# WeChatCV/WeDetect

Measured on AMD Instinct MI355X. Metric: images/s at 640x640 (WeDetect-Base image tower + 80-class similarity + top-k/NMS), higher is better.
Workload: dtype f32-equivalent: fp32 operands carried as fp16 hi+lo pairs, 3 fp16-MFMA passes per product, fp32 accumulate (fp16x3); similarity GEMM, dwconv, LN, post-process native f32

## Files before the change

__graft_entry__.py:

```python
import os
import sys

ROOT = os.path.dirname(os.path.abspath(__file__))
if ROOT not in sys.path:
    sys.path.insert(0, ROOT)


def build() -> None:
    from wedetect_amd import build as wb
    wb.build()
    import wedetect_amd.lib as lib
    import wedetect_amd.feed
    import wedetect_amd.tile
    import wedetect_amd.views
    import wedetect_amd.detector
    import oracle.postprocess
    import oracle.ref_cpu
    print("built and loaded", lib.LIB_PATH)


def smoke() -> None:
    import numpy as np
    import torch
    from oracle import postprocess as opp
    from oracle import ref_cpu as orc
    from wedetect_amd import weights as W
    from wedetect_amd.arch import get_arch
    from wedetect_amd.engine import ImageTower
    from wedetect_amd.pack import pack

    assert torch.cuda.is_available(), "smoke() needs a HIP device"
    torch.cuda.set_device(0)
    arch, b, hw, npr = "tiny", 2, 128, 64
    sd_np = W.make_state_dict(arch, num_prompts=npr)
    tower = ImageTower(arch, pack(sd_np, arch), b, hw, hw)
    imgs = W.make_images(b, hw, hw)
    embed, boxes = tower.features(torch.from_numpy(imgs).cuda())
    scores = tower.similarity(tower.P["prompts"], normalize=False)
    res = tower.postprocess(scores, 0.0, tower.identity_meta(), nms="torchvision")
    torch.cuda.synchronize()
    sd = orc.to_torch(sd_np)
    with torch.no_grad():
        _, p = orc.forward_features(sd, get_arch(arch), imgs)
        flat = orc.head_flat(sd, p, sd["embeddings"], normalize_text=False)
    e_err = float((embed.cpu() - flat["embed"]).abs().max())
    s_err = float((scores.cpu() - flat["scores"]).abs().max())
    b_err = float((boxes.cpu() - flat["boxes"]).abs().max())
    assert e_err < 1e-3 and s_err < 1e-3 and b_err < 1e-2, (e_err, s_err, b_err)
    lvl = np.concatenate([np.full(n, l) for l, n in enumerate(tower.nl)])
    for i in range(b):
        o = opp.uni_predict_image(boxes[i].cpu().numpy(), embed[i].cpu().numpy(), scores[i].cpu().numpy(), lvl,
                                  np.asarray(tower.lvl_logit_scale, np.float32), np.asarray(tower.lvl_bias, np.float32))
        n = int(res["count"][i])
        assert n == o["scores"].shape[0]
        assert np.array_equal(res["anchors"][i, :n].cpu().numpy(), o["anchors"])
        assert np.array_equal(res["labels"][i, :n].cpu().numpy(), o["labels"])
    print(f"smoke OK: max|d| embeddings {e_err:.2e} scores {s_err:.2e} boxes {b_err:.2e}; kept indices exact")


if __name__ == "__main__":
    build()
    if "--smoke" in sys.argv:
        smoke()
```

wedetect_amd/build.py:

```python
from __future__ import annotations

import os
import subprocess
import sys

HERE = os.path.dirname(os.path.abspath(__file__))
ROOT = os.path.dirname(HERE)
CSRC = os.path.join(HERE, "csrc")
LIB = os.path.join(HERE, "libwedetect_hip.so")
SOURCES = ["abi.hip", "conv_gemm.hip", "similarity_grouped.hip", "split_gemm.hip", "split_gemm_pre.hip", "split_gemm_p8.hip", "split_gemm_p4.hip", "split_gemm_conv.hip", "split_gemm_conv3.hip", "split_gemm_mlp.hip", "split_gemm_mlpw.hip", "probe.hip", "stem.hip", "elementwise.hip", "preprocess.hip", "text.hip", "bricks.hip", "evaluate.hip", "det_eval.hip", "postprocess.hip", "feed.hip", "tile.hip", "views.hip"]
PUBLIC_HEADERS = ["wedetect_hip.h", "wedetect_hip_feed.h", "wedetect_hip_tile.h", "wedetect_hip_views.h"]
HIPCC = os.environ.get("HIPCC", "/opt/rocm/bin/hipcc")
FLAGS = ["--offload-arch=gfx950", "-O3", "-std=c++17", "-fPIC", "-Wall", "-Wno-unused-function", "-Wno-inline-asm",
         "-I", os.path.join(ROOT, "include"), "-I", CSRC]
for _d in os.environ.get("WD_EXTRA_DEFINES", "").split():
    FLAGS.append("-D" + _d)
if os.environ.get("WD_DEBUG_ABLATIONS") == "1":
    FLAGS.append("-DWD_DEBUG_ABLATIONS")


def _headers():
    return [os.path.join(CSRC, f) for f in os.listdir(CSRC) if f.endswith(".h")] + [os.path.join(ROOT, "include", h) for h in PUBLIC_HEADERS]


def source_hash() -> str:
    import hashlib
    h = hashlib.sha256()
    files = sorted(os.path.join(CSRC, f) for f in os.listdir(CSRC) if f.endswith((".hip", ".h")))
    for f in files + [os.path.join(ROOT, "include", h) for h in PUBLIC_HEADERS]:
        h.update(os.path.basename(f).encode())
        h.update(open(f, "rb").read())
    return h.hexdigest()


NO_SCRATCH = {"stem.hip": ["stem_fused_kernel"], "split_gemm_mlpw.hip": ["fused_mlp_wide_kernel"],
              "split_gemm_mlp.hip": ["fused_mlp128_kernel"], "split_gemm_p8.hip": ["split_gemm_p8_kernel"],
              "split_gemm_p4.hip": ["split_gemm_p4_kernel"], "split_gemm_conv.hip": ["split_conv_pp_kernel"],
              "split_gemm_conv3.hip": ["split_conv3_kernel", "split_conv3w_kernel"],
              "split_gemm_pre.hip": ["split_gemm_pingpong_kernel", "split_gemm_glds_kernel"],
              "elementwise.hip": ["dwconv7_dma_kernel", "dwconv7_ln_reg4_dma_kernel"],
              "similarity_grouped.hip": ["similarity_grouped_kernel"],
              "feed.hip": ["feed_resample_h_kernel", "feed_canvas_kernel"],
              "tile.hip": ["tile_cut_kernel", "merge_keys_kernel"],
              "views.hip": ["flip_u8_kernel", "views_sort_kernel"]}
ASM_VMEM_SOURCES = {"split_gemm_mlpw.hip": ["fused_mlp_wide_kernel"], "split_gemm_mlp.hip": [], "split_gemm_p8.hip": [],
                    "split_gemm_p4.hip": [], "split_gemm_pre.hip": [], "split_gemm_conv.hip": [], "split_gemm_conv3.hip": [], "stem.hip": [], "elementwise.hip": [], "similarity_grouped.hip": [],
                    "feed.hip": [], "tile.hip": [], "views.hip": []}


ASM_DS_READ_SOURCES = {"split_gemm_conv3.hip": ["split_conv3w_kernel"]}


def check_isa(src: str, verbose: bool = True) -> None:
    asm = _obj(src).replace(".o", ".s")
    cmd = [HIPCC, *[f for f in FLAGS if f != "-fPIC"], "-S", "--cuda-device-only", os.path.join(CSRC, src), "-o", asm]
    subprocess.check_call(cmd, stderr=subprocess.DEVNULL)
    scripts = os.path.join(ROOT, "scripts")
    r = subprocess.run([sys.executable, os.path.join(scripts, "check_sgpr_vmem_hazard.py"), asm], capture_output=True, text=True)
    if r.returncode != 0:
        raise RuntimeError(f"SGPR -> VMEM hazard in the ISA of {src}:\n{r.stdout[-2000:]}")
    syms = ASM_VMEM_SOURCES[src]
    if syms:
        r = subprocess.run([sys.executable, os.path.join(scripts, "check_asm_loads.py"), asm, *syms], capture_output=True, text=True)
        if r.returncode != 0:
            raise RuntimeError(f"pending asm load touched in the ISA of {src}:\n{r.stdout[-2000:]}")
    if src in ASM_DS_READ_SOURCES:
        r = subprocess.run([sys.executable, os.path.join(scripts, "check_asm_ds_reads.py"), asm, *ASM_DS_READ_SOURCES[src]], capture_output=True, text=True)
        if r.returncode != 0:
            raise RuntimeError(f"pending asm ds_read touched in the ISA of {src}:\n{r.stdout[-2000:]}")
    if src in NO_SCRATCH:
        import re
        meta = open(asm).read()
        meta = meta[meta.index("amdhsa.kernels"):] if "amdhsa.kernels" in meta else ""
        seen = set()
        for blk in meta.split("- .agpr_count")[1:]:
            name = re.search(r"\.name:\s+(\S+)", blk).group(1)
            scratch = int(re.search(r"\.private_segment_fixed_size:\s+(\d+)", blk).group(1))
            for k in NO_SCRATCH[src]:
                if k in name:
                    seen.add(k)
                    if scratch != 0:
                        raise RuntimeError(f"{src}: kernel {name} uses {scratch} bytes of scratch — its counted vmcnt waits assume none")
        missing = [k for k in NO_SCRATCH[src] if k not in seen]
        if missing:
            raise RuntimeError(f"{src}: NO_SCRATCH names no kernel of this source: {missing}")
    os.remove(asm)
    if verbose:
        print(f"ISA checks passed: {src}", flush=True)


def _obj(src: str) -> str:
    return os.path.join(CSRC, src.replace(".hip", ".o"))


def _obj_stale(src: str) -> bool:
    obj = _obj(src)
    if not os.path.exists(obj):
        return True
    t = os.path.getmtime(obj)
    return any(os.path.getmtime(d) > t for d in [os.path.join(CSRC, src)] + _headers())


def _stale() -> bool:
    if not os.path.exists(LIB):
        return True
    t = os.path.getmtime(LIB)
    return any(_obj_stale(s) or os.path.getmtime(_obj(s)) > t for s in SOURCES)


def build(force: bool = False, verbose: bool = True) -> str:
    if not force and not _stale():
        return LIB
    procs = []
    for src in SOURCES:
        if not force and not _obj_stale(src):
            continue
        cmd = [HIPCC, *FLAGS, "-c", os.path.join(CSRC, src), "-o", _obj(src)]
        if verbose:
            print(" ".join(cmd), flush=True)
        procs.append((src, subprocess.Popen(cmd)))
    import concurrent.futures as cf
    with cf.ThreadPoolExecutor(max_workers=4) as ex:
        checks = [ex.submit(check_isa, src, verbose) for src, _ in procs if src in ASM_VMEM_SOURCES]
        for src, p in procs:
            if p.wait() != 0:
                raise RuntimeError(f"hipcc failed on {src}")
        for c in checks:
            c.result()
    cmd = [HIPCC, "--offload-arch=gfx950", "-shared", "-fPIC", *[_obj(s) for s in SOURCES], "-o", LIB]
    if verbose:
        print(" ".join(cmd), flush=True)
    subprocess.check_call(cmd)
    return LIB


if __name__ == "__main__":
    print(build(force="--force" in sys.argv))
```

wedetect_amd/csrc/split_epi_oct.h:

```cpp
#pragma once
#include "split_gemm_impl.h"

namespace {

template <int ACT, bool SPECIAL, bool CSPLIT>
__device__ __forceinline__ void epi_oct_core(const WdConvGemm& p, float unscale, int m, int n, const f32x4 v0, const f32x4 v1,
                                             const f32x4 b0, const f32x4 b1, const f32x4 r0, const f32x4 r1) {
  if (p.range_flag) {
    if (wd_any_nonfinite4(v0[0] + v0[1], v0[2] + v0[3], v1[0] + v1[1], v1[2] + v1[3])) *p.range_flag = 1u;
  }
  const EpiRow er = epi_row<SPECIAL>(p, m);
  f32x4 o0, o1;
#pragma unroll
  for (int r = 0; r < 4; ++r) {
    float x0 = sact<ACT>(fmaf(v0[r], unscale, b0[r]));
    float x1 = sact<ACT>(fmaf(v1[r], unscale, b1[r]));
    if (SPECIAL) {
      x0 = fmaf(x0, er.oscale, er.obias);
      x1 = fmaf(x1, er.oscale, er.obias);
      if (p.sigmoid) { x0 = wd_sigmoid_fast(x0); x1 = wd_sigmoid_fast(x1); }
    }
    o0[r] = x0;
    o1[r] = x1;
  }
  if (p.res != nullptr) {
#pragma unroll
    for (int r = 0; r < 4; ++r) {
      o0[r] = fmaf(p.res_alpha, r0[r], o0[r]);
      o1[r] = fmaf(p.res_alpha, r1[r], o1[r]);
    }
  }
  if (p.c2 != nullptr) {
    float* qp = p.c2 + (SPECIAL && p.c_batch_stride > 0 ? er.crow : (size_t)m) * p.ldc2 + n;
    *reinterpret_cast<f32x4*>(qp) = o0;
    *reinterpret_cast<f32x4*>(qp + 4) = o1;
  }
  float* rowp;
  int col = n;
  if (SPECIAL && p.out_mode == WD_OUT_DECONV2X2) {
    const int ncq = p.n >> 2;
    const int tap = n / ncq;
    col = n - tap * ncq;
    rowp = p.c + (er.crow + (size_t)(tap >> 1) * er.hw2 + (tap & 1)) * p.ldc;
  } else {
    rowp = p.c + er.crow * p.ldc;
  }
  if (CSPLIT) {
    u32x2 h0, l0, h1, l1;
    f32x4 s0 = o0, s1 = o1;
    if (p.c_split_scale != 0.f && p.c_split_scale != 1.0f) {
      s0 = o0 * p.c_split_scale;
      s1 = o1 * p.c_split_scale;
    }
    split4(s0, h0, l0);
    split4(s1, h1, l1);
    unsigned char* cp = reinterpret_cast<unsigned char*>(rowp) + (size_t)(col >> 3) * 32;
    *reinterpret_cast<u32x4*>(cp) = u32x4{h0[0], h0[1], h1[0], h1[1]};
    *reinterpret_cast<u32x4*>(cp + 16) = u32x4{l0[0], l0[1], l1[0], l1[1]};
  } else {
    *reinterpret_cast<f32x4*>(rowp + col) = o0;
    *reinterpret_cast<f32x4*>(rowp + col + 4) = o1;
  }
}

template <int ACT, bool SPECIAL, bool CSPLIT>
__device__ __forceinline__ void epi_oct(const WdConvGemm& p, float unscale, int m, int n, const f32x4 v0, const f32x4 v1) {
  f32x4 b0 = {0.f, 0.f, 0.f, 0.f}, b1 = {0.f, 0.f, 0.f, 0.f}, r0 = b0, r1 = b0;
  if (p.bias) {
    b0 = *reinterpret_cast<const f32x4*>(p.bias + n);
    b1 = *reinterpret_cast<const f32x4*>(p.bias + n + 4);
  }
  if (p.res != nullptr) {
    const float* rp = p.res + (size_t)m * p.ldres + n;
    r0 = *reinterpret_cast<const f32x4*>(rp);
    r1 = *reinterpret_cast<const f32x4*>(rp + 4);
  }
  epi_oct_core<ACT, SPECIAL, CSPLIT>(p, unscale, m, n, v0, v1, b0, b1, r0, r1);
}

template <int TM, int TN, bool PRE = true>
struct EpiOctOperands {
  static constexpr int NB = PRE ? TN : 1, NR = PRE ? TM * TN * 2 : 1;
  f32x4 b0[NB], b1[NB], r0[NR], r1[NR];
  __device__ __forceinline__ void load(const WdConvGemm& p, int mw, int nw, int lane) {
    if (!PRE) return;
#pragma unroll
    for (int j = 0; j < TN; ++j) {
      const int n = nw + j * 32 + 8 * (lane & 3);
      b0[j] = b1[j] = f32x4{0.f, 0.f, 0.f, 0.f};
      if (p.bias && n < p.n) {
        b0[j] = *reinterpret_cast<const f32x4*>(p.bias + n);
        b1[j] = *reinterpret_cast<const f32x4*>(p.bias + n + 4);
      }
    }
#pragma unroll
    for (int ij = 0; ij < TM * TN; ++ij)
#pragma unroll
      for (int ps = 0; ps < 2; ++ps) {
        const int m = mw + (ij / TN) * 32 + ps * 16 + (lane >> 2), n = nw + (ij % TN) * 32 + 8 * (lane & 3);
        r0[ij * 2 + ps] = r1[ij * 2 + ps] = f32x4{0.f, 0.f, 0.f, 0.f};
        if (p.res != nullptr && m < p.m && n < p.n) {
          const float* rp = p.res + (size_t)m * p.ldres + n;
          r0[ij * 2 + ps] = *reinterpret_cast<const f32x4*>(rp);
          r1[ij * 2 + ps] = *reinterpret_cast<const f32x4*>(rp + 4);
        }
      }
  }
};

template <int IJ, int TM, int TN, int ACT, bool SPECIAL, bool CSPLIT, bool PRE = true>
struct EpiOctWalk {
  static __device__ __forceinline__ void run(const WdConvGemm& p, float unscale, int mw, int nw, int lane,
                                             const f32x16 (&acc)[TM][TN], float* patch, const EpiOctOperands<TM, TN, PRE>& ops) {
    constexpr int I = IJ / TN, J = IJ % TN;
#pragma unroll
    for (int g = 0; g < 4; ++g)
      *reinterpret_cast<f32x4*>(patch + (lane & 31) * EPI_LDT + 8 * g + 4 * (lane >> 5)) =
          f32x4{acc[I][J][4 * g], acc[I][J][4 * g + 1], acc[I][J][4 * g + 2], acc[I][J][4 * g + 3]};
    __builtin_amdgcn_fence(__ATOMIC_RELEASE, "wavefront");
    __builtin_amdgcn_wave_barrier();
    __builtin_amdgcn_fence(__ATOMIC_ACQUIRE, "wavefront");
#pragma unroll
    for (int ps = 0; ps < 2; ++ps) {
      const int row = ps * 16 + (lane >> 2);
      const int m = mw + I * 32 + row;
      const int n = nw + J * 32 + 8 * (lane & 3);
      const f32x4 v0 = *reinterpret_cast<const f32x4*>(patch + row * EPI_LDT + 8 * (lane & 3));
      const f32x4 v1 = *reinterpret_cast<const f32x4*>(patch + row * EPI_LDT + 8 * (lane & 3) + 4);
      if (m < p.m && n < p.n) {
        if (PRE)
          epi_oct_core<ACT, SPECIAL, CSPLIT>(p, unscale, m, n, v0, v1, ops.b0[PRE ? J : 0], ops.b1[PRE ? J : 0],
                                             ops.r0[PRE ? IJ * 2 + ps : 0], ops.r1[PRE ? IJ * 2 + ps : 0]);
        else
          epi_oct<ACT, SPECIAL, CSPLIT>(p, unscale, m, n, v0, v1);
      }
    }
    __builtin_amdgcn_fence(__ATOMIC_RELEASE, "wavefront");
    __builtin_amdgcn_wave_barrier();
    __builtin_amdgcn_fence(__ATOMIC_ACQUIRE, "wavefront");
    EpiOctWalk<IJ + 1, TM, TN, ACT, SPECIAL, CSPLIT, PRE>::run(p, unscale, mw, nw, lane, acc, patch, ops);
  }
};
template <int TM, int TN, int ACT, bool SPECIAL, bool CSPLIT, bool PRE>
struct EpiOctWalk<TM * TN, TM, TN, ACT, SPECIAL, CSPLIT, PRE> {
  static __device__ __forceinline__ void run(const WdConvGemm&, float, int, int, int, const f32x16 (&)[TM][TN], float*,
                                             const EpiOctOperands<TM, TN, PRE>&) {}
};

template <int TM, int TN, bool CSPLIT, bool PRE = true>
__device__ __forceinline__ void epi_oct_all(const WdConvGemm& p, float unscale, int mw, int nw, int lane,
                                            const f32x16 (&acc)[TM][TN], float* patch) {
  const bool special = p.out_mode != WD_OUT_ROWS || p.c_batch_stride > 0 || p.seg_rows > 0 || p.sigmoid ||
                       p.out_scale != 1.0f || p.out_bias != 0.0f;
  EpiOctOperands<TM, TN, PRE> ops;
  ops.load(p, mw, nw, lane);
#define WD_OCT(A, S) EpiOctWalk<0, TM, TN, A, S, CSPLIT, PRE>::run(p, unscale, mw, nw, lane, acc, patch, ops)
  if (special) {
    switch (p.act) {
      case WD_ACT_RELU: WD_OCT(WD_ACT_RELU, true); break;
      case WD_ACT_SILU: WD_OCT(WD_ACT_SILU, true); break;
      case WD_ACT_GELU: WD_OCT(WD_ACT_GELU, true); break;
      default: WD_OCT(WD_ACT_NONE, true); break;
    }
  } else {
    switch (p.act) {
      case WD_ACT_RELU: WD_OCT(WD_ACT_RELU, false); break;
      case WD_ACT_SILU: WD_OCT(WD_ACT_SILU, false); break;
      case WD_ACT_GELU: WD_OCT(WD_ACT_GELU, false); break;
      default: WD_OCT(WD_ACT_NONE, false); break;
    }
  }
#undef WD_OCT
}

}
```

wedetect_amd/csrc/split_gemm.hip:

```cpp
#include <stdlib.h>
#include "split_gemm_impl.h"

namespace {

__global__ void split_weights_kernel(const float* __restrict__ w, int n, int k, int k16, float scale,
                                     unsigned short* __restrict__ out, int n_out) {
  const long long idx = (long long)blockIdx.x * blockDim.x + threadIdx.x;
  if (idx >= (long long)n_out * k16) return;
  const int row = (int)(idx / k16), kk = (int)(idx % k16);
  const float x = (kk < k && row < n) ? w[(size_t)row * k + kk] * scale : 0.0f;
  const _Float16 hi = (_Float16)x;
  const _Float16 lo = (_Float16)(x - (float)hi);
  unsigned short* o = out + (size_t)row * 2 * k16 + (kk >> 3) * 16 + (kk & 7);
  o[0] = __builtin_bit_cast(unsigned short, hi);
  o[8] = __builtin_bit_cast(unsigned short, lo);
}

template <int ACT, bool SPECIAL>
__global__ void __launch_bounds__(256) splitk_reduce_kernel(const WdConvGemm p, const float* __restrict__ ws, int splits,
                                                            float unscale, int vec_c, int vec_res, int vec_bias) {
  const long long idx = (long long)blockIdx.x * blockDim.x + threadIdx.x;
  const int nq = p.n >> 2;
  if (idx >= (long long)p.m * nq) return;
  const int m = (int)(idx / nq), n = (int)(idx - (long long)m * nq) * 4;
  const size_t plane = (size_t)p.m * p.n;
  f32x4 v = *reinterpret_cast<const f32x4*>(ws + (size_t)m * p.n + n);
  for (int s = 1; s < splits; ++s) v += *reinterpret_cast<const f32x4*>(ws + s * plane + (size_t)m * p.n + n);
  const EpiVec ev{vec_c, vec_res, vec_bias, unscale};
  epi_quad<ACT, SPECIAL>(p, epi_row<SPECIAL>(p, m), ev, m, n, v);
}

template <bool SPECIAL>
int launch_reduce(const WdConvGemm& p, const float* ws, int splits, float unscale, hipStream_t st) {
  const long long total = (long long)p.m * (p.n >> 2);
  const dim3 grid((unsigned)((total + 255) / 256)), block(256);
  const int vec_c = (p.ldc % 4 == 0) && wd_aligned16(p.c) && (p.out_mode == WD_OUT_ROWS || (p.n % 16 == 0));
  const int vec_res = p.res ? ((p.ldres % 4 == 0) && wd_aligned16(p.res)) : 0;
  const int vec_bias = p.bias ? wd_aligned16(p.bias) : 0;
  switch (p.act) {
    case WD_ACT_RELU: hipLaunchKernelGGL((splitk_reduce_kernel<WD_ACT_RELU, SPECIAL>), grid, block, 0, st, p, ws, splits, unscale, vec_c, vec_res, vec_bias); break;
    case WD_ACT_SILU: hipLaunchKernelGGL((splitk_reduce_kernel<WD_ACT_SILU, SPECIAL>), grid, block, 0, st, p, ws, splits, unscale, vec_c, vec_res, vec_bias); break;
    case WD_ACT_GELU: hipLaunchKernelGGL((splitk_reduce_kernel<WD_ACT_GELU, SPECIAL>), grid, block, 0, st, p, ws, splits, unscale, vec_c, vec_res, vec_bias); break;
    default: hipLaunchKernelGGL((splitk_reduce_kernel<WD_ACT_NONE, SPECIAL>), grid, block, 0, st, p, ws, splits, unscale, vec_c, vec_res, vec_bias); break;
  }
  return wd_launch_status();
}

}

extern "C" int64_t wd_split_weights_bytes(int32_t n, int32_t k) {
  if (n <= 0 || k <= 0) return 0;
  return (int64_t)((n + 7) & ~7) * ((k + 15) / 16 * 16) * 4;
}

static int split_weights_launch(const float* w, int32_t n, int32_t k, float scale, void* out, void* stream, int n_out) {
  if (!w || !out || n <= 0 || k <= 0 || !(scale > 0.0f) || !wd_aligned16(out)) return WD_ERR_BAD_ARG;
  const int k16 = (k + 15) / 16 * 16;
  const long long total = (long long)n_out * k16;
  hipLaunchKernelGGL(split_weights_kernel, dim3((unsigned)((total + 255) / 256)), dim3(256), 0,
                     static_cast<hipStream_t>(stream), w, n, k, k16, scale, static_cast<unsigned short*>(out), n_out);
  return wd_launch_status();
}

extern "C" int wd_split_weights(const float* w, int32_t n, int32_t k, float scale, void* out, void* stream) {
  return split_weights_launch(w, n, k, scale, out, stream, n);
}

extern "C" int wd_split_weights_padded(const float* w, int32_t n, int32_t k, float scale, void* out, void* stream) {
  return split_weights_launch(w, n, k, scale, out, stream, (n + 7) & ~7);
}

static int pick_split_cfg(const WdConvGemm& p) {
  const int m = p.m, n = p.n;
  const long long pad128 = (long long)((n + 127) / 128) * 128, pad64 = (long long)((n + 63) / 64) * 64;
  if (pad64 < pad128) return m >= 65536 ? 52 : 53;
  const bool plain = p.kh == 1 && p.kw == 1 && p.stride == 1 && p.pad == 0;
  if (plain && p.k >= 1024) return 55;
  const long long tiles = (long long)((m + 127) / 128) * ((n + 127) / 128);
  return tiles < 1024 ? 50 : 51;
}

long long wd_p8_workspace_floats();
bool wd_p8_persist_ok(int m, int n);
bool wd_conv_pp_ok(const WdConvGemm& p, int flags);
int wd_launch_conv_pp(const WdConvGemm& p, const void* w, float unscale, int flags, hipStream_t st, int ksplits, float* ws,
                      long long ws_floats, int variant);
bool wd_conv3_ok(const WdConvGemm& p, int flags);
const char* wd_conv3_config_name(int m, int n);
int wd_launch_conv3(const WdConvGemm& p, const void* w, float unscale, int flags, hipStream_t st, int variant, int ksplits, float* ws,
                    long long ws_floats);

extern "C" int64_t wd_p8_workspace_bytes(void) { return 4 * wd_p8_workspace_floats(); }

static int pick_presplit_cfg(int m, int n, int k, bool park) {
  if (k % 32 == 0 && k >= 256 && m % 8 == 0 && n % 256 == 0) {
    const long long tiles = (long long)((m + 255) / 256) * (n / 256);
    static const int mink = [] { const char* e = getenv("WD_P8_PERSIST_MINK"); return e ? atoi(e) : 1024; }();
    if (park && k >= mink && wd_p8_persist_ok(m, n)) return 65;
    if (tiles >= 128) return 64;
  }
  if (k % 16 == 0 && n % 256 == 0 && m % 16 == 0 && m >= 131072) return 66;
  return m >= 131072 ? 63 : 60;
}

extern "C" const char* wd_conv_gemm_split_config(int32_t m, int32_t n, int32_t k, int32_t is_conv) {
  if (is_conv == 4) {
    const bool narrow = (n % 128) != 0 && ((n + 63) / 64) * 64 < ((n + 127) / 128) * 128;
    return narrow ? "fp16x3 256x64x16/8w/dma" : "fp16x3 256x128x16/8w/dma";
  }
  if (is_conv == 5) return wd_conv3_config_name(m, n);
  if ((is_conv == 2 || is_conv == 3) && k % 16 == 0) {
    switch (pick_presplit_cfg(m, n, k, is_conv == 3)) {
      case 65: return "fp16x3 256x256x32/8w/p8s";
      case 64: return "fp16x3 256x256x32/8w/p8";
      case 66: return "fp16x3 128x256x16/4w/p4";
      case 63: return "fp16x3 256x128x16/8w/pingpong";
      default: return "fp16x3 128x128x16/4w/glds";
    }
  }
  WdConvGemm q{};
  q.m = m; q.n = n; q.k = k; q.kh = q.kw = q.stride = 1;
  if (is_conv) q.kh = q.kw = 3;
  switch (pick_split_cfg(q)) {
    case 50: return "fp16x3 128x128x32/4w";
    case 51: return "fp16x3 128x128x16/4w";
    case 52: return "fp16x3 256x64x16/4w";
    case 55: return "fp16x3 128x128x32/4w/pf2";
    default: return "fp16x3 128x64x16/2w";
  }
}

static int pick_ksplits(const WdConvGemm& p, int cfg, int flags, long long ws_floats) {
  if (ws_floats <= 0 || (flags & WD_SPLIT_C) || (p.n & 3) || cfg == 55 || cfg == 63 || cfg >= 64) return 1;
  const int bm = 128, bn = (cfg == 52 || cfg == 53) ? 64 : 128, bk = (cfg == 50) ? 32 : 16;
  const long long tiles = (long long)((p.m + (cfg == 52 ? 255 : bm - 1)) / (cfg == 52 ? 256 : bm)) * ((p.n + bn - 1) / bn);
  const int nk = (p.k + bk - 1) / bk;
  if (tiles >= 128 || nk < 16) return 1;
  int s = (int)(512 / tiles);
  if (s > nk / 8) s = nk / 8;
  if (s > 16) s = 16;
  while (s > 1 && (long long)s * p.m * p.n > ws_floats) --s;
  return s < 2 ? 1 : s;
}

static int conv_gemm_split_impl(const WdConvGemm* pp, const void* w_split, float w_unscale, int32_t flags, int32_t cfg,
                                float* ws, int64_t ws_bytes, int32_t force_splits, hipStream_t st) {
  if (!pp) return WD_ERR_BAD_ARG;
  const WdConvGemm& p = *pp;
  const int rc = check_split_args(p, w_split, w_unscale);
  if (rc != WD_OK) return rc;
  if (flags & ~(WD_SPLIT_A | WD_SPLIT_C)) return WD_ERR_BAD_ARG;
  if (ws && !wd_aligned16(ws)) return WD_ERR_BAD_ARG;
  if (p.c2 && !(flags & WD_SPLIT_C)) return WD_ERR_BAD_ARG;
  const bool production = cfg < 0;
  if (cfg < 0) cfg = pick_split_cfg(p);
  const bool plain = p.kh == 1 && p.kw == 1 && p.stride == 1 && p.pad == 0;
  const bool special = p.out_mode != WD_OUT_ROWS || p.c_batch_stride > 0 || p.seg_rows > 0 || p.sigmoid ||
                       p.out_scale != 1.0f || p.out_bias != 0.0f;
  if (p.ln_stats || p.ln_u) {
    if (!p.ln_stats || !p.ln_u || flags != (WD_SPLIT_A | WD_SPLIT_C) || !plain || special || p.res || p.c2 || force_splits > 1 ||
        !wd_aligned16(p.ln_u) || (reinterpret_cast<uintptr_t>(p.ln_stats) & 7u))
      return WD_ERR_BAD_ARG;
    if (cfg == 70 || cfg == 73 || cfg == 74 || (cfg >= 75 && cfg <= 79) || (cfg >= 700 && cfg < 716)) return WD_ERR_UNSUPPORTED;
  }
  if (flags & WD_SPLIT_A) {
    const bool covered = plain && !special && !p.c2 && !((flags & WD_SPLIT_C) && p.res);
    const bool forced = cfg == 70 || cfg == 73 || cfg == 74 || (cfg >= 700 && cfg < 716);
    static const bool conv3_on = [] { const char* e = getenv("WEDETECT_CONV3"); return !(e && e[0] == '0'); }();
    if ((cfg >= 75 && cfg <= 79) || (production && conv3_on && !(force_splits == 0 && ws != nullptr))) {
      if (wd_conv3_ok(p, flags) && wd_conv_pp_ok(p, flags))
        return wd_launch_conv3(p, w_split, w_unscale, flags, st, cfg == 76 ? 2 : cfg == 77 ? 7 : cfg == 78 ? 8 : cfg == 79 ? 9 : 0, force_splits > 1 ? force_splits : 1, ws, ws ? ws_bytes / 4 : 0);
      if (cfg >= 75 && cfg <= 79) return WD_ERR_UNSUPPORTED;
    }
    if (forced || (production && !covered)) {
      if (!wd_conv_pp_ok(p, flags)) return forced || !covered ? WD_ERR_UNSUPPORTED : WD_ERR_BAD_ARG;
      const long long wsf = ws ? ws_bytes / 4 : 0;
      int splits = force_splits > 0 ? force_splits : 1;
      if (force_splits == 0 && wsf > 0 && !forced) {
        const long long tiles = (long long)((p.m + 255) / 256) * ((p.n + 127) / 128);
        const int nk = p.k / 16;
        if (tiles < 128 && nk >= 32) {
          int s2 = (int)(256 / tiles);
          if (s2 > nk / 16) s2 = nk / 16;
          if (s2 > 8) s2 = 8;
          while (s2 > 1 && (long long)s2 * p.m * p.n > wsf) --s2;
          if (s2 > 1) splits = s2;
        }
      }
      return wd_launch_conv_pp(p, w_split, w_unscale, flags, st, splits, ws, wsf,
                               cfg == 73 ? 3 : cfg == 74 ? 4 : cfg >= 700 ? cfg - 600 : 0);
    }
  }
  if (flags == WD_SPLIT_C) {
    if (!plain || special || p.res || p.c2 || p.n % 8 || p.ldc % 8 || (p.bias && !wd_aligned16(p.bias)) || !wd_aligned16(p.c))
      return WD_ERR_UNSUPPORTED;
    constexpr int VC = SVAR_XCD | SVAR_PIN | SVAR_LDSEPI | SVAR_CSPLIT;
    const long long tiles = (long long)((p.m + 127) / 128) * ((p.n + 127) / 128);
    return tiles < 1024 ? launch_split<2, 2, 2, 2, 32, VC, 1>(p, w_split, w_unscale, st)
                        : launch_split<2, 2, 2, 2, 16, VC, 1>(p, w_split, w_unscale, st);
  }
  if (flags != 0) {
    if (production && plain && !special && p.k % 16 == 0)
      cfg = pick_presplit_cfg(p.m, p.n, p.k, ws != nullptr && force_splits == 0 && ws_bytes / 4 >= wd_p8_workspace_floats() &&
                                                 p.lda % 8 == 0 && !(flags & ~(WD_SPLIT_A | WD_SPLIT_C)));
    if (cfg != 50 && cfg != 51 && cfg != 55 && cfg != 60 && cfg != 63 && cfg != 64 && cfg != 65 && cfg != 66 && !(cfg >= 640 && cfg < 768)) cfg = 51;
    if ((flags & WD_SPLIT_C) && cfg == 55) cfg = 50;
  }
  const long long ws_floats = ws ? ws_bytes / 4 : 0;
  int splits = force_splits > 0 ? force_splits : pick_ksplits(p, cfg, flags, ws_floats);
  {
    const int bk = (cfg == 50) ? 32 : 16, nk = (p.k + bk - 1) / bk;
    if (splits > nk) splits = nk;
  }
  if (splits > 1) {
    if ((flags & WD_SPLIT_C) || (p.n & 3) || cfg == 55 || cfg == 63 || cfg >= 64) return WD_ERR_UNSUPPORTED;
    if ((long long)splits * p.m * p.n > ws_floats) return WD_ERR_WORKSPACE;
  }
  int lrc;
  if (flags != 0) {
    lrc = wd_launch_presplit(p, w_split, w_unscale, cfg, flags, st, splits, ws, ws_floats);
  } else {
    switch (cfg) {
      case 41: lrc = launch_split<2, 2, 2, 4, 16, SVAR_XCD | SVAR_PIN | SVAR_LDSEPI>(p, w_split, w_unscale, st, splits, ws); break;
      case 50: lrc = launch_split<2, 2, 2, 2, 32, SVAR_XCD | SVAR_PIN | SVAR_LDSEPI>(p, w_split, w_unscale, st, splits, ws); break;
      case 51: lrc = launch_split<2, 2, 2, 2, 16, SVAR_XCD | SVAR_PIN | SVAR_LDSEPI>(p, w_split, w_unscale, st, splits, ws); break;
      case 52: lrc = launch_split<2, 2, 4, 1, 16, SVAR_XCD | SVAR_PIN | SVAR_LDSEPI>(p, w_split, w_unscale, st, splits, ws); break;
      case 53: lrc = launch_split<2, 2, 2, 1, 16, SVAR_XCD | SVAR_PIN | SVAR_LDSEPI>(p, w_split, w_unscale, st, splits, ws); break;
      case 55: lrc = launch_split<2, 2, 2, 2, 32, SVAR_XCD | SVAR_PF2 | SVAR_LDSEPI>(p, w_split, w_unscale, st); break;
      default: return WD_ERR_UNSUPPORTED;
    }
  }
  if (lrc != WD_OK || splits <= 1) return lrc;
  return special ? launch_reduce<true>(p, ws, splits, w_unscale, st) : launch_reduce<false>(p, ws, splits, w_unscale, st);
}

extern "C" int wd_conv_gemm_split(const WdConvGemm* pp, const void* w_split, float w_unscale, int32_t flags,
                                  int32_t cfg, void* stream) {
  return conv_gemm_split_impl(pp, w_split, w_unscale, flags, cfg, nullptr, 0, 0, static_cast<hipStream_t>(stream));
}

extern "C" int wd_conv_gemm_split_ws(const WdConvGemm* pp, const void* w_split, float w_unscale, int32_t flags,
                                     int32_t cfg, void* workspace, int64_t workspace_bytes, int32_t splits, void* stream) {
  if (splits < 0 || workspace_bytes < 0) return WD_ERR_BAD_ARG;
  return conv_gemm_split_impl(pp, w_split, w_unscale, flags, cfg, static_cast<float*>(workspace), workspace_bytes, splits,
                              static_cast<hipStream_t>(stream));
}
```

wedetect_amd/csrc/split_gemm_conv.hip:

```cpp
#include "split_epi_oct.h"

namespace {

constexpr int CV_BM = 256, CV_WROWS = 128, CV_ROWB = 64, CV_STAGE = (CV_BM + CV_WROWS) * CV_ROWB, CV_NI = 3;

__device__ __forceinline__ void cv_dma16(unsigned lds_addr, const unsigned char* src) {
  asm volatile("s_mov_b32 m0, %0\n\tglobal_load_lds_dwordx4 %1, off" ::"s"(lds_addr), "v"(src) : "memory", "m0");
}

__device__ __forceinline__ void cv_wait_groups(int groups) {
  if (groups <= 0) asm volatile("s_waitcnt vmcnt(0)" ::: "memory");
  else if (groups == 1) asm volatile("s_waitcnt vmcnt(3)" ::: "memory");
  else if (groups == 2) asm volatile("s_waitcnt vmcnt(6)" ::: "memory");
  else if (groups == 3) asm volatile("s_waitcnt vmcnt(9)" ::: "memory");
  else if (groups == 4) asm volatile("s_waitcnt vmcnt(12)" ::: "memory");
  else asm volatile("s_waitcnt vmcnt(15)" ::: "memory");
}

template <int NBUF, int TN, bool CSPLIT, int ABL = 0>
__global__ void __launch_bounds__(512, NBUF <= 3 ? 4 : 2)
split_conv_pp_kernel(const WdConvGemm p, const unsigned char* __restrict__ wsp, const float* __restrict__ zero, int k16,
                     float unscale, int nbn, int ksplits, float* __restrict__ ws) {
  constexpr int TM = 2, BM = CV_BM, BN = 64 * TN, ROWB = CV_ROWB, STAGE = CV_STAGE, NI = CV_NI, DIST = NBUF - 1;
  extern __shared__ __attribute__((aligned(16))) unsigned char smem_raw[];
  const int t = threadIdx.x, lane = t & 63, wave = t >> 6;
  const int group = wave >> 2, wm = (wave >> 1) & 1, wn = wave & 1;
  int tile = blockIdx.x;
  {
    const int nwg = gridDim.x, xcd = tile & 7, idx = tile >> 3;
    const int q = nwg >> 3, r = nwg & 7;
    tile = (xcd < r ? xcd * (q + 1) : r * (q + 1) + (xcd - r) * q) + idx;
  }
  const int ntiles = gridDim.x / ksplits;
  const int ks = tile / ntiles;
  tile -= ks * ntiles;
  const int bn = tile % nbn, bm = tile / nbn;
  const int m0 = bm * BM, n0 = bn * BN;
  const int nk_all = p.k >> 4;
  const int per_split = (nk_all + ksplits - 1) / ksplits;
  const int s_begin = ks * per_split;
  const int nk = (s_begin + per_split < nk_all ? s_begin + per_split : nk_all) - s_begin;

  const unsigned char* base[NI];
  unsigned mask[NI];
#pragma unroll
  for (int j = 0; j < NI; ++j) {
    const int row = (wave * NI + j) * 16 + (lane >> 2);
    const int logical = (lane & 3) ^ ((row >> 2) & 3);
    const int memchunk = ((logical & 1) << 1) | ((logical >> 1) & 1);
    if (row < BM) {
      const int m = m0 + row;
      const bool ok = m < p.m;
      const int mm = ok ? m : 0;
      const int wo = mm % p.wout;
      const int q = mm / p.wout;
      const int ho = q % p.hout;
      const int b = q / p.hout;
      const int hi0 = ho * p.stride - p.pad, wi0 = wo * p.stride - p.pad;
      const long long pix = ((long long)b * p.hin + hi0) * p.win + wi0;
      base[j] = reinterpret_cast<const unsigned char*>(p.a) + pix * p.lda * 4 + memchunk * 16;
      unsigned mk = 0, bit = 1u;
      for (int kh = 0; kh < p.kh; ++kh) {
        const bool hok = (unsigned)(hi0 + kh) < (unsigned)p.hin;
        for (int kw = 0; kw < p.kw; ++kw, bit <<= 1)
          mk |= (hok && (unsigned)(wi0 + kw) < (unsigned)p.win) ? bit : 0u;
      }
      mask[j] = ok ? mk : 0u;
    } else {
      const int n = n0 + row - BM;
      const bool ok = n < p.n;
      base[j] = wsp + (size_t)(ok ? n : 0) * k16 * 4 + memchunk * 16;
      mask[j] = ok ? 0xFFFFFFFFu : 0u;
    }
  }
  int i_tap, i_ci, i_kh, i_kw, i_w;
  {
    const int kofs = s_begin * 16;
    i_tap = kofs / p.cin;
    i_ci = kofs - i_tap * p.cin;
    i_kh = i_tap / p.kw;
    i_kw = i_tap - i_kh * p.kw;
    i_w = s_begin * ROWB;
  }
  const unsigned lds0 = (unsigned)(size_t)(__attribute__((address_space(3))) unsigned char*)smem_raw;
  const unsigned char* zp = reinterpret_cast<const unsigned char*>(zero);
  bool prologue = true;
  auto issue = [&](int buf) {
    if ((ABL & 1) && !prologue) return;
    const unsigned lbase = lds0 + buf * STAGE + wave * NI * 1024;
    const int a_off = ((i_kh * p.win + i_kw) * p.lda + i_ci) * 4;
#pragma unroll
    for (int j = 0; j < NI; ++j) {
      const bool is_a = (wave * NI + j) * 16 < BM;
      const int off = is_a ? a_off : i_w;
      const unsigned bit = is_a ? (mask[j] >> i_tap) & 1u : mask[j] & 1u;
      cv_dma16(__builtin_amdgcn_readfirstlane(lbase + j * 1024), bit ? base[j] + off : zp);
    }
    i_w += ROWB;
    i_ci += 16;
    if (i_ci == p.cin) {
      i_ci = 0;
      ++i_tap;
      if (++i_kw == p.kw) { i_kw = 0; ++i_kh; }
    }
  };

  f32x16 acc[TM][TN];
#pragma unroll
  for (int i = 0; i < TM; ++i)
#pragma unroll
    for (int j = 0; j < TN; ++j)
#pragma unroll
      for (int r = 0; r < 16; ++r) acc[i][j][r] = 0.0f;

  int aoff_h[TM], aoff_l[TM], boff_h[TN], boff_l[TN];
  const int hsel = lane >> 5;
#pragma unroll
  for (int i = 0; i < TM; ++i) {
    const int row = group * 128 + wm * 64 + i * 32 + (lane & 31), f = (row >> 2) & 3;
    aoff_h[i] = row * ROWB + ((hsel ^ f) << 4);
    aoff_l[i] = row * ROWB + (((2 + hsel) ^ f) << 4);
  }
#pragma unroll
  for (int j = 0; j < TN; ++j) {
    const int row = wn * 32 * TN + j * 32 + (lane & 31), f = (row >> 2) & 3;
    boff_h[j] = BM * ROWB + row * ROWB + ((hsel ^ f) << 4);
    boff_l[j] = BM * ROWB + row * ROWB + (((2 + hsel) ^ f) << 4);
  }
  h8 xh[TM], xl[TM], wh[TN], wl[TN];
  auto read = [&](int buf) {
    if ((ABL & 2) && !prologue) return;
    const unsigned char* sp = smem_raw + buf * STAGE;
#pragma unroll
    for (int i = 0; i < TM; ++i) {
      xh[i] = *reinterpret_cast<const h8*>(sp + aoff_h[i]);
      xl[i] = *reinterpret_cast<const h8*>(sp + aoff_l[i]);
    }
#pragma unroll
    for (int j = 0; j < TN; ++j) {
      wh[j] = *reinterpret_cast<const h8*>(sp + boff_h[j]);
      wl[j] = *reinterpret_cast<const h8*>(sp + boff_l[j]);
    }
  };
  auto mfma = [&]() {
    if (ABL & 4) return;
#pragma unroll
    for (int i = 0; i < TM; ++i)
#pragma unroll
      for (int j = 0; j < TN; ++j)
        acc[i][j] = __builtin_amdgcn_mfma_f32_32x32x16_f16(wl[j], xh[i], acc[i][j], 0, 0, 0);
#pragma unroll
    for (int i = 0; i < TM; ++i)
#pragma unroll
      for (int j = 0; j < TN; ++j)
        acc[i][j] = __builtin_amdgcn_mfma_f32_32x32x16_f16(wh[j], xl[i], acc[i][j], 0, 0, 0);
#pragma unroll
    for (int i = 0; i < TM; ++i)
#pragma unroll
      for (int j = 0; j < TN; ++j)
        acc[i][j] = __builtin_amdgcn_mfma_f32_32x32x16_f16(wh[j], xh[i], acc[i][j], 0, 0, 0);
  };

#pragma unroll
  for (int d = 0; d < DIST; ++d)
    if (d < nk) issue(d);
  asm volatile("s_waitcnt vmcnt(0)" ::: "memory");
  __syncthreads();
  if (ABL & 2) read(0);
  prologue = false;
  int bcur = 0, bfill = DIST % NBUF;
  for (int s = 0; s < nk; ++s) {
    read(bcur);
    if (s + DIST < nk) issue(bfill);
    __builtin_amdgcn_sched_barrier(0);
    mfma();
    __builtin_amdgcn_sched_barrier(0);
    {
      const int last = s + DIST < nk - 1 ? s + DIST : nk - 1;
      cv_wait_groups(last - (s + 1));
    }
    __builtin_amdgcn_sched_barrier(0);
    __syncthreads();
    __builtin_amdgcn_sched_barrier(0);
    bcur = bcur == NBUF - 1 ? 0 : bcur + 1;
    bfill = bfill == NBUF - 1 ? 0 : bfill + 1;
  }
  __syncthreads();

  if (ABL & 8) {
    float sacc = 0.f;
#pragma unroll
    for (int i = 0; i < TM; ++i)
#pragma unroll
      for (int j = 0; j < TN; ++j)
#pragma unroll
        for (int r = 0; r < 16; ++r) sacc += acc[i][j][r];
    if (m0 + (t & 255) < p.m) p.c[(size_t)(m0 + (t & 255)) * p.ldc + n0 + (t >> 8)] = sacc;
    return;
  }
  const int mw = m0 + group * 128 + wm * 64, nw = n0 + wn * 32 * TN;
  float* patch = reinterpret_cast<float*>(smem_raw) + wave * 32 * EPI_LDT;
  static_assert(2 * STAGE >= 8 * 32 * EPI_LDT * 4, "operand LDS must hold one patch per wave");
  if (ksplits > 1) {
    WdConvGemm pr = p;
    pr.bias = nullptr; pr.res = nullptr; pr.c2 = nullptr; pr.range_flag = nullptr;
    pr.c = ws + (size_t)ks * p.m * p.n; pr.ldc = p.n;
    pr.out_mode = WD_OUT_ROWS; pr.c_batch_stride = 0; pr.seg_rows = 0; pr.sigmoid = 0; pr.out_scale = 1.0f; pr.out_bias = 0.0f;
    pr.act = WD_ACT_NONE;
    EpiOctOperands<TM, TN, false> ops;
    ops.load(pr, mw, nw, lane);
    EpiOctWalk<0, TM, TN, WD_ACT_NONE, false, false, false>::run(pr, 1.0f, mw, nw, lane, acc, patch, ops);
    return;
  }
  epi_oct_all<TM, TN, CSPLIT, (NBUF == 4 || TN == 1)>(p, unscale, mw, nw, lane, acc, patch);
}

template <int ACT, bool SPECIAL, bool CSPLIT>
__global__ void __launch_bounds__(256) splitk_oct_reduce_kernel(const WdConvGemm p, const float* __restrict__ ws, int splits,
                                                                float unscale) {
  const long long idx = (long long)blockIdx.x * blockDim.x + threadIdx.x;
  const int no = p.n >> 3;
  if (idx >= (long long)p.m * no) return;
  const int m = (int)(idx / no), n = (int)(idx - (long long)m * no) * 8;
  const size_t plane = (size_t)p.m * p.n;
  const float* src = ws + (size_t)m * p.n + n;
  f32x4 v0 = *reinterpret_cast<const f32x4*>(src), v1 = *reinterpret_cast<const f32x4*>(src + 4);
  for (int s = 1; s < splits; ++s) {
    v0 += *reinterpret_cast<const f32x4*>(src + s * plane);
    v1 += *reinterpret_cast<const f32x4*>(src + s * plane + 4);
  }
  epi_oct<ACT, SPECIAL, CSPLIT>(p, unscale, m, n, v0, v1);
}

template <bool CSPLIT>
int launch_oct_reduce(const WdConvGemm& p, const float* ws, int splits, float unscale, hipStream_t st) {
  const long long total = (long long)p.m * (p.n >> 3);
  const dim3 grid((unsigned)((total + 255) / 256)), block(256);
  const bool special = p.out_mode != WD_OUT_ROWS || p.c_batch_stride > 0 || p.seg_rows > 0 || p.sigmoid ||
                       p.out_scale != 1.0f || p.out_bias != 0.0f;
#define WD_RED(A, S) hipLaunchKernelGGL((splitk_oct_reduce_kernel<A, S, CSPLIT>), grid, block, 0, st, p, ws, splits, unscale)
  if (special) {
    switch (p.act) {
      case WD_ACT_RELU: WD_RED(WD_ACT_RELU, true); break;
      case WD_ACT_SILU: WD_RED(WD_ACT_SILU, true); break;
      case WD_ACT_GELU: WD_RED(WD_ACT_GELU, true); break;
      default: WD_RED(WD_ACT_NONE, true); break;
    }
  } else {
    switch (p.act) {
      case WD_ACT_RELU: WD_RED(WD_ACT_RELU, false); break;
      case WD_ACT_SILU: WD_RED(WD_ACT_SILU, false); break;
      case WD_ACT_GELU: WD_RED(WD_ACT_GELU, false); break;
      default: WD_RED(WD_ACT_NONE, false); break;
    }
  }
#undef WD_RED
  return wd_launch_status();
}

template <int NBUF, int TN, bool CSPLIT, int ABL = 0>
int launch_conv_pp(const WdConvGemm& p, const void* wsp, float unscale, hipStream_t st, int ksplits, float* ws) {
  constexpr int BN = 64 * TN, LDS = NBUF * CV_STAGE;
  const int nbm = (p.m + CV_BM - 1) / CV_BM, nbn = (p.n + BN - 1) / BN;
  const long long nblk = (long long)nbm * nbn * ksplits;
  if (nblk <= 0 || nblk > 0x7fffffffLL) return WD_ERR_BAD_ARG;
  const int k16 = (p.k + 15) / 16 * 16;
  const float* zero = wd_zero_block();
  if (!zero) return WD_ERR_LAUNCH;
  auto k = split_conv_pp_kernel<NBUF, TN, CSPLIT, ABL>;
  static WdAttrOnce attr;
  if (wd_set_max_lds(attr, reinterpret_cast<const void*>(k), LDS) != WD_OK) return WD_ERR_LAUNCH;
  WD_LAUNCH_GEMM(k, dim3((unsigned)nblk), dim3(512), LDS, st, p, static_cast<const unsigned char*>(wsp), zero, k16, unscale,
                 nbn, ksplits, ws);
  return wd_launch_status();
}

}

int wd_launch_oct_reduce(const WdConvGemm& p, const float* ws, int splits, float unscale, bool csplit, hipStream_t st) {
  return csplit ? launch_oct_reduce<true>(p, ws, splits, unscale, st) : launch_oct_reduce<false>(p, ws, splits, unscale, st);
}

bool wd_conv_pp_ok(const WdConvGemm& p, int flags) {
  if (!(flags & WD_SPLIT_A)) return false;
  if (p.cin % 16 || p.k % 16 || p.lda % 8 || p.kh * p.kw > 16 || p.n % 8) return false;
  if (!wd_aligned16(p.a) || !wd_aligned16(p.c)) return false;
  if (p.bias && !wd_aligned16(p.bias)) return false;
  if (p.res && (!wd_aligned16(p.res) || p.ldres % 4)) return false;
  if (p.c2 && (!(flags & WD_SPLIT_C) || !wd_aligned16(p.c2) || p.ldc2 % 4 || p.ldc2 < p.n || p.out_mode != WD_OUT_ROWS))
    return false;
  if ((flags & WD_SPLIT_C) ? (p.ldc % 8 != 0) : (p.ldc % 4 != 0)) return false;
  if (p.out_mode == WD_OUT_DECONV2X2 && (p.n % 32)) return false;
  return true;
}

int wd_launch_conv_pp(const WdConvGemm& p, const void* w, float unscale, int flags, hipStream_t st, int ksplits, float* ws,
                      long long ws_floats, int variant) {
  if (!wd_conv_pp_ok(p, flags)) return WD_ERR_UNSUPPORTED;
  const bool csplit = (flags & WD_SPLIT_C) != 0;
  const bool narrow = (p.n % 128) != 0 && ((p.n + 63) / 64) * 64 < ((p.n + 127) / 128) * 128;
  const long long tiles = (long long)((p.m + CV_BM - 1) / CV_BM) * (narrow ? (p.n + 63) / 64 : (p.n + 127) / 128);
  if (ksplits < 1) ksplits = 1;
  if (ksplits > 1 && (!ws || (long long)ksplits * p.m * p.n > ws_floats)) return WD_ERR_WORKSPACE;
  if (ksplits > (p.k >> 4)) ksplits = p.k >> 4;
  int nbuf = (tiles * ksplits <= 256) ? 4 : 3;
  if (variant == 3 || variant == 4) nbuf = variant;
  int rc;
#ifdef WD_DEBUG_ABLATIONS
  if (variant >= 100 && variant < 116 && !narrow && csplit) {
    switch (variant - 100) {
      case 1: return launch_conv_pp<4, 2, true, 1>(p, w, unscale, st, 1, ws);
      case 2: return launch_conv_pp<4, 2, true, 2>(p, w, unscale, st, 1, ws);
      case 3: return launch_conv_pp<4, 2, true, 3>(p, w, unscale, st, 1, ws);
      case 4: return launch_conv_pp<4, 2, true, 4>(p, w, unscale, st, 1, ws);
      case 7: return launch_conv_pp<4, 2, true, 7>(p, w, unscale, st, 1, ws);
      case 8: return launch_conv_pp<4, 2, true, 8>(p, w, unscale, st, 1, ws);
      case 11: return launch_conv_pp<4, 2, true, 11>(p, w, unscale, st, 1, ws);
      case 15: return launch_conv_pp<4, 2, true, 15>(p, w, unscale, st, 1, ws);
      default: break;
    }
  }
#endif
#define WD_CPP(NB, TNN, CS) launch_conv_pp<NB, TNN, CS>(p, w, unscale, st, ksplits, ws)
  if (nbuf == 4) {
    if (narrow) rc = csplit ? WD_CPP(4, 1, true) : WD_CPP(4, 1, false);
    else rc = csplit ? WD_CPP(4, 2, true) : WD_CPP(4, 2, false);
  } else {
    if (narrow) rc = csplit ? WD_CPP(3, 1, true) : WD_CPP(3, 1, false);
    else rc = csplit ? WD_CPP(3, 2, true) : WD_CPP(3, 2, false);
  }
#undef WD_CPP
  if (rc != WD_OK || ksplits <= 1) return rc;
  return csplit ? launch_oct_reduce<true>(p, ws, ksplits, unscale, st) : launch_oct_reduce<false>(p, ws, ksplits, unscale, st);
}
```

wedetect_amd/engine.py:

```python
from __future__ import annotations

import contextlib
import copy
import math
import os
import weakref
from typing import Dict, List, Optional, Sequence, Tuple

import numpy as np
import torch

from . import lib as L
from .arch import ArchSpec, CLS_MID, EMBED_DIM, REG_MID, STRIDES, get_arch, level_sizes
from .pack import Packed


DEFAULT_PRECISION = "fp16x3"


def fold_layernorm_into_linear(w1: torch.Tensor, b1: torch.Tensor, gamma: torch.Tensor, beta: torch.Tensor):
    w64, g64 = w1.double(), gamma.double()
    w1g = (w64 * g64[None, :]).float().contiguous()
    u = w1g.double().sum(dim=1).float().contiguous()
    v = (w64 @ beta.double() + b1.double()).float().contiguous()
    return w1g, u, v


_DEVICE_STREAMS: Dict[str, Dict[str, list]] = {}


def device_streams(dev: torch.device, role: str, n: int = 1) -> List[torch.cuda.Stream]:
    pool = _DEVICE_STREAMS.setdefault(str(dev), {})
    if not pool:
        for r in ("post", "nh", "bb2"):
            pool[r] = [torch.cuda.Stream(device=dev)]
    lst = pool.setdefault(role, [])
    while len(lst) < n:
        lst.append(torch.cuda.Stream(device=dev))
    return lst[:n]


class ImageTower:
    PRECISIONS = ("fp32", "fp16x3")
    SPLIT_K_AUTO_PIXELS = 4 * 640 * 640
    SPLIT_K_MID_PIXELS = 8 * 640 * 640

    def __init__(self, arch, packed: Packed, batch: int, height: int, width: int, device="cuda",
                 max_classes: int = 256, nms_pre: int = 30000, max_out: int = 300,
                 precision: Optional[str] = None, split_k: Optional[bool] = None):
        self.a: ArchSpec = get_arch(arch) if isinstance(arch, str) else arch
        self.P = packed
        if precision is None:
            precision = os.environ.get("WEDETECT_PRECISION", DEFAULT_PRECISION)
        if precision not in self.PRECISIONS:
            raise ValueError(f"precision must be one of {self.PRECISIONS}")
        self.precision = precision
        self.Ws: Dict[str, tuple] = {}
        auto_class = split_k is None and os.environ.get("WEDETECT_SPLIT_K", "auto") == "auto"
        if split_k is None:
            env = os.environ.get("WEDETECT_SPLIT_K", "auto")
            split_k = env == "1" or (env == "auto" and batch * height * width <= self.SPLIT_K_MID_PIXELS)
        self._split_ref = 1
        if split_k and auto_class and batch * height * width > self.SPLIT_K_AUTO_PIXELS:
            self._split_ref = max(1, self.SPLIT_K_MID_PIXELS // (height * width))
        self.kws = (torch.empty(16 << 20, dtype=torch.float32, device=torch.device(device))
                    if precision == "fp16x3" and split_k else None)
        self._kws_lane: Dict[int, torch.Tensor] = {}
        self.fixed_splitk = precision == "fp16x3" and os.environ.get("WEDETECT_FIXED_SPLITK", "1") == "1"
        self.fws = (torch.empty(2 * batch * 400 * 256 + 64, dtype=torch.float32, device=torch.device(device))
                    if self.fixed_splitk else None)
        self.p8_mode = os.environ.get("WEDETECT_P8", "persist")
        self.post_stream, self._post_ready, self._post_done = None, None, None
        dag = os.environ.get("WEDETECT_DAG", "auto")
        self.dag = dag != "0"
        self._dag_forced = dag == "1"
        self._dag_in_capture = dag == "1" or batch * height * width >= 8 * 640 * 640
        self._side: List[torch.cuda.Stream] = []
        self._events: List[torch.cuda.Event] = []
        self._ev_i = 0
        self._ev_after_neck = 0
        self._lane_i = 0
        self._fws_lane: Dict[int, torch.Tensor] = {}
        self._head_evs: List[torch.cuda.Event] = []
        self.bb_chains = os.environ.get("WEDETECT_BB_CHAINS", "auto")
        self.bb_chain_order = os.environ.get("WEDETECT_BB_CHAIN_ORDER", "free")
        st = os.environ.get("WEDETECT_BB_CHAIN_STAGES", "0-3").split("-")
        self.bb_chain_stages = (max(0, int(st[0])), min(3, int(st[-1])))
        self._chain_streams: List[torch.cuda.Stream] = []
        self.pipe_neck = os.environ.get("WEDETECT_PIPE_NECK", "auto")
        self._nh_stream: Optional[torch.cuda.Stream] = None
        self._nh_issue = False
        self._x_sets: List[List[torch.Tensor]] = []
        self._x_par = 0
        self._x_free: List[Optional[torch.cuda.Event]] = [None]
        self._bb_done: List[torch.cuda.Event] = []
        self.bb_depth = os.environ.get("WEDETECT_BB_DEPTH", "auto")
        self._depth2_issue = False
        self.pipe_persist = os.environ.get("WEDETECT_PIPE_PERSIST", "0")
        self._pipe_issue = False
        self.force_tile_forms = os.environ.get("WEDETECT_FORCE_TILE", "0") == "1"
        self._bb_slot = 0
        self._slot1: Optional[dict] = None
        self._chain_parks: Dict[int, torch.Tensor] = {}
        self._chain_evs: List[torch.cuda.Event] = []
        self.s2d_down = os.environ.get("WEDETECT_S2D_DOWN", "1") != "0"
        self.park = None
        if precision == "fp16x3" and self.p8_mode == "persist" and L.p8_workspace_bytes() > 0:
            self.park = torch.zeros(L.p8_workspace_bytes() // 4, dtype=torch.float32, device=torch.device(device))
        self.conv3 = os.environ.get("WEDETECT_CONV3", "1") != "0"
        self._park_mlp = None
        self.B, self.H, self.W = batch, height, width
        self.fuse_stem = os.environ.get("WEDETECT_FUSE_STEM", "1") == "1"
        self.fuse_mlp = os.environ.get("WEDETECT_FUSE_MLP", "1") == "1"
        self.fuse_mlp_wide = tuple(int(v) for v in os.environ.get("WEDETECT_FUSE_MLP_WIDE", "256").split(",") if v.strip())
        self.Wf: Dict[str, tuple] = {}
        self.fuse_dwln = os.environ.get("WEDETECT_FUSE_DWLN", "auto")
        self.fuse_dwln_wide = tuple(int(v) for v in os.environ.get("WEDETECT_FUSE_DWLN_WIDE", "").split(",") if v.strip())
        self.ln_fold = os.environ.get("WEDETECT_LN_FOLD", "1") == "1"
        self.ln_fold_fused = os.environ.get("WEDETECT_LN_FOLD_FUSED", "1") == "1"
        self.ln_part = self.ln_stats = None
        self.sim_split = os.environ.get("WEDETECT_SIM_SPLIT", "auto")
        self.embed_s: Optional[torch.Tensor] = None
        self._embed_split_on = False
        self._embed_split_valid = False
        self._text_split: list = []
        self.overflowed = False
        self.fp16x3_trips = 0
        self.fp16x3_retries = 0
        self._clean_fp32_steps, self._retry_after = 0, self.FALLBACK_RETRY
        self.range_flags = torch.zeros(2, dtype=torch.int32, device=torch.device(device))
        self.range_flag = self.range_flags[0:1]
        self.range_flag2 = self.range_flags[1:2]
        self.neck_pin = precision != "fp16x3" or os.environ.get("WEDETECT_NECK_GUARD", "1") == "0"
        self.dev = torch.device(device)
        if height % 32 or width % 32:
            raise ValueError("input size must be a multiple of 32")
        a, B = self.a, batch
        f = lambda *shape: torch.empty(*shape, dtype=torch.float32, device=self.dev)
        self.hw = [(height // (4 << i), width // (4 << i)) for i in range(4)]
        self.M = [B * h * w for h, w in self.hw]
        self.patches = f(self.M[0], 48)
        self.x = [f(self.M[i], a.dims[i]) for i in range(4)]
        self.tmp = f(max(self.M[i] * a.dims[i] for i in range(4)))
        self.hid = f(max(self.M[i] * 4 * a.dims[i] for i in range(4)))
        nc = a.neck_channels
        (h3, w3), (h4, w4), (h5, w5) = self.hw[1], self.hw[2], self.hw[3]
        M2, M3, M4, M5 = self.M
        self.cat_n4 = f(M5, nc["d1"] + nc["p5r"])
        self.cat_b0 = f(M4, 3 * nc["p5r"])
        self.b0_t = f(M3, nc["p5r"])
        self.f0 = f(M4, nc["p5r"])
        self.f_out0 = f(M4, nc["p5r"])
        self.cat_n3 = f(M4, nc["d2"] + nc["p4r"])
        self.cat_b1 = f(M3, 3 * nc["p4r"])
        self.b1_t = f(M2, nc["p4r"])
        self.f1 = f(M3, nc["p4r"])
        self.p3 = f(M3, nc["p4r"])
        self.p4 = f(M4, nc["n3"])
        self.p5 = f(M5, nc["n4"])
        self._bep = {}
        for name, m, cout in (("Rep_p4", M4, nc["p5r"]), ("Rep_p3", M3, nc["p4r"]),
                              ("Rep_n3", M4, nc["n3"]), ("Rep_n4", M5, nc["n4"])):
            c_ = cout // 2
            self._bep[name] = dict(cat=f(m, 2 * c_), u0=f(m, c_), u1=f(m, c_), t=f(m, c_), u0s=f(m, c_), u1s=f(m, c_), c_=c_)
        self.presplit_neck = (precision == "fp16x3" and os.environ.get("WEDETECT_NECK_PRESPLIT", "1") != "0"
                              and all(v % 32 == 0 for v in nc.values()) and CLS_MID % 16 == 0 and REG_MID % 16 == 0)
        self.lv = level_sizes(height, width)
        self.nl = [h * w for h, w in self.lv]
        self.ntot = sum(self.nl)
        self.off = [0, self.nl[0], self.nl[0] + self.nl[1]]
        self.embed = f(B, self.ntot, EMBED_DIM)
        self.boxes = f(B, self.ntot, 4)
        self.hc = [(f(B * n, CLS_MID), f(B * n, CLS_MID)) for n in self.nl]
        self.hr = [(f(B * n, REG_MID), f(B * n, REG_MID), f(B * n, 4 * 16)) for n in self.nl]
        self.nms_pre, self.max_out = nms_pre, max_out
        self.cap = L.topk_capacity(nms_pre)
        self.generation = 0
        self.sscale: Dict[str, float] = {}
        self._calib: Optional[Dict[str, torch.Tensor]] = None
        self._ln_scaled: Dict[tuple, tuple] = {}
        self.calibrated = False
        self.calibration_runs = 0
        self._alloc_post(max_classes)
        self.nms_ws = torch.zeros(max(1, L.nms_workspace_bytes(B) // 4), dtype=torch.int32, device=self.dev)
        self.cand_idx = torch.empty(B, self.cap, dtype=torch.int32, device=self.dev)
        self.cand_score = f(B, self.cap)
        self.cand_count = torch.empty(B, dtype=torch.int32, device=self.dev)
        self.out_boxes = f(B, max_out, 4)
        self.out_scores = f(B, max_out)
        self.out_labels = torch.empty(B, max_out, dtype=torch.int32, device=self.dev)
        self.out_anchors = torch.empty(B, max_out, dtype=torch.int32, device=self.dev)
        self.out_count = torch.empty(B, dtype=torch.int32, device=self.dev)
        self.out_embed = f(B, max_out, EMBED_DIM)
        self.text_norm = f(max_classes, EMBED_DIM)
        self.text_norm_pi: Optional[torch.Tensor] = None
        self.lvl_scale = [float(np.exp(np.float32(self.P.s[f"head{l}.logit_scale"]))) for l in range(3)]
        self.lvl_bias = [float(np.float32(self.P.s[f"head{l}.bias"])) for l in range(3)]
        self.lvl_logit_scale = [float(np.float32(self.P.s[f"head{l}.logit_scale"])) for l in range(3)]
        self._prepare_fold()

    def _alloc_post(self, k: int) -> None:
        self.max_classes = k
        self.generation += 1
        self.scores = torch.empty(self.B, self.ntot, k, dtype=torch.float32, device=self.dev)
        nbytes = L.topk_workspace_bytes(self.B, self.ntot * k, self.nms_pre)
        self.topk_ws = torch.empty(nbytes + 256, dtype=torch.uint8, device=self.dev)
        off = (-self.topk_ws.data_ptr()) % 256
        self.topk_ws = self.topk_ws[off:off + nbytes]

    def _record(self, key: Optional[str], t: torch.Tensor) -> None:
        if self._calib is None or key is None or t.numel() == 0:
            return
        m = t.abs().max()
        self._calib[key] = torch.maximum(self._calib[key], m) if key in self._calib else m

    def _ln_params(self, wname: str, bname: str, key: Optional[str]):
        sc = self.sscale.get(key, 1.0) if key else 1.0
        if sc == 1.0 or self.precision != "fp16x3":
            return self.P[wname], self.P[bname]
        ck = (wname, sc)
        if ck not in self._ln_scaled:
            self._ln_scaled[ck] = (self.P[wname] * sc, self.P[bname] * sc)
        return self._ln_scaled[ck]

    def _gemm(self, a, w: str, b: Optional[str], c, *, fp32: bool = False, a_key: Optional[str] = None,
              c_key: Optional[str] = None, **kw):
        ws = None
        guarded = fp32 and self.precision == "fp16x3" and not self.neck_pin
        if self.precision == "fp16x3" and (not fp32 or guarded):
            ws = self.Ws.get(w)
            if ws is None:
                wt = self.P[w]
                ws = self.Ws[w] = L.split_weights(wt.view(wt.shape[0], -1))
        work = None
        if ws is not None and self.kws is not None:
            ks = self._latency_splits(kw)
            if ks > 1:
                kh_, st_, pd_ = kw.get("kh", 1), kw.get("stride", 1), kw.get("pad", 0)
                m_ = self.B * ((kw["hin"] + 2 * pd_ - kh_) // st_ + 1) * ((kw["win"] + 2 * pd_ - kh_) // st_ + 1)
                work, kw = self._lane_kws(ks * m_ * kw["n"] + 64), dict(kw, k_splits=ks)
        if (ws is not None and self.fixed_splitk and self.kws is None and kw.get("kh", 1) == 3 and kw.get("stride", 1) == 1
                and kw["hin"] * kw["win"] <= 400 and 9 * kw["cin"] >= 2304 and kw["n"] % 4 == 0
                and 2 * self.B * kw["hin"] * kw["win"] * kw["n"] <= self.fws.numel()):
            work, kw = self._lane_fws(), dict(kw, k_splits=2)
        if (ws is not None and (kw.get("split_flags", 0) & L.SPLIT_A) and not self.conv3 and kw.get("kh", 1) == 3
                and kw.get("stride", 1) == 1 and "split_cfg" not in kw):
            kw = dict(kw, split_cfg=70)
        if ws is not None and (kw.get("split_flags", 0) & L.SPLIT_A):
            plain = kw.get("kh", 1) == 1 and kw.get("kw", 1) == 1 and kw.get("stride", 1) == 1 and kw.get("pad", 0) == 0
            m = self.B * kw["hin"] * kw["win"]
            if plain and self.park is not None and self._lane_i == 0 and not self._nh_issue and self._persist_ok("p8") and L.gemm_config(m, kw["n"], kw["cin"], split=True, presplit=True,
                                                                                       park=True).endswith("/p8s"):
                work = self.park
            elif plain and self.p8_mode == "0" and kw["cin"] % 16 == 0:
                flags_ = kw.get("split_flags", 0)
                special = (kw.get("out_mode", 0) != 0 or kw.get("c_batch_stride", 0) > 0 or kw.get("seg") is not None
                           or kw.get("sigmoid") or kw.get("c2") is not None or ((flags_ & L.SPLIT_C) and kw.get("res") is not None))
                if not special:
                    kw = dict(kw, split_cfg=63 if m >= 131072 else 60)
        if ws is not None:
            flags = kw.get("split_flags", 0)
            sa = self.sscale.get(a_key, 1.0) if a_key else 1.0
            if sa != 1.0:
                ws = (ws[0], ws[1] / sa)
                if not (flags & L.SPLIT_A):
                    kw = dict(kw, a_scale=sa)
            sc = self.sscale.get(c_key, 1.0) if (c_key and (flags & L.SPLIT_C)) else 1.0
            if sc != 1.0:
                kw = dict(kw, c_split_scale=sc)
        L.conv_gemm(a, None if ws is not None else self.P[w], self.P[b] if b else None, c, batch=self.B,
                    w_split=ws, workspace=work,
                    range_flag=(self.range_flag2 if guarded else self.range_flag) if ws is not None else None, **kw)
        if self._calib is not None:
            if fp32 and a_key:
                self._record(a_key, a[..., : kw["cin"]])
            if c_key:
                n, kh_, st_, pd_ = kw["n"], kw.get("kh", 1), kw.get("stride", 1), kw.get("pad", 0)
                m = self.B * ((kw["hin"] + 2 * pd_ - kh_) // st_ + 1) * ((kw["win"] + 2 * pd_ - kh_) // st_ + 1)
                if c.dim() == 1:
                    self._record(c_key, c[: m * kw["ldc"]])
                else:
                    self._record(c_key, c[..., : n // 4] if kw.get("out_mode", 0) == L.OUT_DECONV2X2 else c[..., :n])

    def _latency_splits(self, kw) -> int:
        flags = kw.get("split_flags", 0)
        kh, st, pd = kw.get("kh", 1), kw.get("stride", 1), kw.get("pad", 0)
        n, k = kw["n"], kh * kh * kw["cin"]
        if n % 4 or kw.get("ln_stats") is not None or "k_splits" in kw:
            return 1
        m1 = ((kw["hin"] + 2 * pd - kh) // st + 1) * ((kw["win"] + 2 * pd - kh) // st + 1) * self._split_ref
        plain = kh == 1 and st == 1 and pd == 0
        special = (kw.get("out_mode", 0) != 0 or kw.get("c_batch_stride", 0) > 0 or kw.get("seg") is not None or kw.get("sigmoid")
                   or kw.get("out_scale", 1.0) != 1.0 or kw.get("out_bias", 0.0) != 0.0)
        covered = plain and not special and kw.get("c2") is None and not ((flags & L.SPLIT_C) and kw.get("res") is not None)
        if (flags & L.SPLIT_A) and not covered:
            if kw["cin"] % 16 or k % 16 or n % 8:
                return 1
            tiles, nk = -(-m1 // 256) * -(-n // 128), k // 16
            if tiles >= 128 or nk < 32:
                return 1
            return max(1, min(256 // tiles, nk // 16, 8))
        if flags & L.SPLIT_C:
            return 1
        if (flags & L.SPLIT_A) and not L.gemm_config((self.B if self._split_ref == 1 else 1) * m1, n, k, split=True, presplit=True).endswith("/glds"):
            return 1
        tiles, nk = -(-m1 // 128) * -(-n // 128), -(-k // 16)
        if tiles >= 128 or nk < 16:
            return 1
        return max(1, min(512 // tiles, nk // 8, 16))

    def _persist_ok(self, family: str) -> bool:
        return not (self._pipe_issue or self.force_tile_forms) or self.pipe_persist in ("1", family)

    def _fold_weights(self, q: str) -> None:
        if q + "w1g" in self.P.t:
            return
        self.P.t[q + "w1g"], self.P.t[q + "u"], self.P.t[q + "v"] = fold_layernorm_into_linear(
            self.P[q + "w1"], self.P[q + "b1"], self.P[q + "ln_w"], self.P[q + "ln_b"])

    def _prepare_fold(self) -> None:
        a = self.a
        stages = [i for i in range(4)
                  if self._fold_ok(i, self.precision == "fp16x3" and a.dims[i] % 8 == 0 and (i == 0 or a.dims[i - 1] % 8 == 0))]
        if not stages:
            return
        if self.ln_stats is None:
            rows = max(self.M[k] for k in range(4))
            blk = max(self.M[k] * (a.dims[k] // 32) for k in range(4) if a.dims[k] % 32 == 0)
            self.ln_part = torch.empty(2 * blk, dtype=torch.float32, device=self.dev)
            self.ln_stats = torch.empty(2 * rows, dtype=torch.float32, device=self.dev)
        if not torch.cuda.is_current_stream_capturing():
            for i in stages:
                for j in range(a.depths[i]):
                    self._fold_weights(f"s{i}.{j}.")

    def _fold_ok(self, i: int, pre: bool) -> bool:
        c = self.a.dims[i]
        if not (self.ln_fold and pre and self.precision == "fp16x3" and c % 32 == 0):
            return False
        if self.fuse_dwln == "1" or (self.fuse_dwln == "auto" and (c <= 128 or c in self.fuse_dwln_wide)):
            return False
        if self.fuse_mlp and L.mlp_fused_supported(self.M[i], c, 4 * c):
            return False
        if c in self.fuse_mlp_wide and L.mlp_wide_supported(self.M[i], c, 4 * c):
            return self.ln_fold_fused and c in L.MLP_WIDE_FOLD_WIDTHS
        return True

    def _mlp_fused_fold(self, q: str, i: int) -> None:
        c = self.a.dims[i]
        self._fold_weights(q)
        ws = []
        for name, (n_, k_) in ((q + "w1g", (4 * c, c)), (q + "w2", (c, 4 * c))):
            f_ = self.Wf.get(name)
            if f_ is None:
                s_ = self.Ws.get(name)
                if s_ is None:
                    wt = self.P[name]
                    s_ = self.Ws[name] = L.split_weights(wt.view(wt.shape[0], -1))
                f_ = self.Wf[name] = (L.mlp_wide_pack(s_[0], n_, k_), s_[1])
            ws.append(f_)
        sa, sh = self.sscale.get(q + "dw", 1.0), self.sscale.get(q + "hid", 1.0)
        if self._park_mlp is None:
            self._park_mlp = self.park if self.park is not None else torch.zeros(
                max(1, L.p8_workspace_bytes() // 4), dtype=torch.float32, device=self.dev)
        L.mlp_fused_wide_ln(self.tmp, self.M[i], c, 4 * c, (ws[0][0], ws[0][1] / sa), self.P[q + "v"], self.P[q + "u"], self.ln_stats,
                            (ws[1][0], ws[1][1] / sh), self.P[q + "b2"], self.x[i], hid_scale=sh, range_flag=self.range_flag,
                            workspace=self._park_mlp if self._persist_ok("mlp") else None)

    def _mlp_fused(self, q: str, i: int, wide: bool = False) -> None:
        c = self.a.dims[i]
        ws = []
        for name in (q + "w1", q + "w2"):
            s_ = self.Ws.get(name)
            if s_ is None:
                wt = self.P[name]
                s_ = self.Ws[name] = L.split_weights(wt.view(wt.shape[0], -1))
            if wide:
                f_ = self.Wf.get(name)
                if f_ is None:
                    n_, k_ = (4 * c, c) if name.endswith("w1") else (c, 4 * c)
                    f_ = self.Wf[name] = (L.mlp_wide_pack(s_[0], n_, k_), s_[1])
                s_ = f_
            ws.append(s_)
        sa, sh = self.sscale.get(q + "ln", 1.0), self.sscale.get(q + "hid", 1.0)
        kw = {}
        if wide:
            if self._park_mlp is None:
                self._park_mlp = self.park if self.park is not None else torch.zeros(
                    max(1, L.p8_workspace_bytes() // 4), dtype=torch.float32, device=self.dev)
            kw["workspace"] = self._park_mlp if self._persist_ok("mlp") else None
        fn = L.mlp_fused_wide if wide else L.mlp_fused
        fn(self.tmp, self.M[i], c, 4 * c, (ws[0][0], ws[0][1] / sa), self.P[q + "b1"], (ws[1][0], ws[1][1] / sh),
           self.P[q + "b2"], self.x[i], hid_scale=sh, range_flag=self.range_flag, **kw)

    def _neck_split(self) -> bool:
        return self.presplit_neck and self.precision == "fp16x3" and not self.neck_pin

    @staticmethod
    def unsplit(t: torch.Tensor, scale: float = 1.0) -> torch.Tensor:
        rows, c = t.shape
        h = t.contiguous().view(torch.float16).view(rows, c // 8, 2, 8)
        v = (h[:, :, 0].float() + h[:, :, 1].float()).reshape(rows, c)
        return v if scale == 1.0 else v / scale

    def pyramid(self) -> List[torch.Tensor]:
        ps = [self.p3, self.p4, self.p5]
        if not self._neck_split():
            return ps
        return [self.unsplit(p, self.sscale.get(k, 1.0)) for p, k in zip(ps, ("p3", "p4", "p5"))]

    def _conv(self, a, w, b, c, *, hin, win, cin, lda, n, ldc, k=1, stride=1, act=L.ACT_NONE, res=None, ldres=0,
              res_alpha=1.0, **kw):
        self._gemm(a, w, b, c, hin=hin, win=win, cin=cin, lda=lda, kh=k, kw=k, stride=stride,
                   pad=(k // 2 if k == 3 else 0), n=n, ldc=ldc, act=act, res=res, ldres=ldres, res_alpha=res_alpha, **kw)

    N_LANES = 4

    def _dag_on(self) -> bool:
        if self._nh_issue and not self._dag_forced:
            return False
        return (self.dag and self._calib is None
                and (self._dag_in_capture or not torch.cuda.is_current_stream_capturing()))

    def _lane_kws(self, need: int = 0) -> Optional[torch.Tensor]:
        if self.kws is None:
            return None
        li = self._lane_i + (16 if self._nh_issue else 0)
        w = self.kws if li == 0 else self._kws_lane.get(li)
        if w is None or w.numel() < need:
            if torch.cuda.is_current_stream_capturing():
                raise L.WedetectHipError("split-K workspace must be grown before stream capture (run the step eagerly once)")
            w = torch.empty(max(need, self.kws.numel()), dtype=torch.float32, device=self.dev)
            if li == 0:
                self.kws = w
                self.generation += 1
            else:
                self._kws_lane[li] = w
        return w

    def _lane_fws(self) -> torch.Tensor:
        if self._lane_i == 0:
            return self.fws
        w = self._fws_lane.get(self._lane_i)
        if w is None:
            w = self._fws_lane[self._lane_i] = torch.empty_like(self.fws)
        return w

    class _Lane:
        def __init__(self, tower, i):
            self.t, self.i, self.ctx = tower, i, None

        def __enter__(self):
            t = self.t
            self.prev = t._lane_i
            t._lane_i = self.i
            if self.i > 0:
                self.ctx = torch.cuda.stream(t._side[self.i - 1])
                self.ctx.__enter__()
            return self

        def __exit__(self, *a):
            if self.ctx is not None:
                self.ctx.__exit__(*a)
            self.t._lane_i = self.prev

    def _lane(self, i: int) -> "ImageTower._Lane":
        if len(self._side) < self.N_LANES - 1:
            self._side = device_streams(self.dev, "lanes", self.N_LANES - 1)
        return ImageTower._Lane(self, i)

    def _mark(self) -> torch.cuda.Event:
        if self._ev_i == len(self._events):
            self._events.append(torch.cuda.Event())
        ev = self._events[self._ev_i]
        self._ev_i += 1
        ev.record(torch.cuda.current_stream())
        return ev

    @staticmethod
    def _after(*evs) -> None:
        st = torch.cuda.current_stream()
        for ev in evs:
            if ev is not None:
                st.wait_event(ev)

    BB_CHAINS_MIN_PIXELS = 32 * 640 * 640
    PIPE_NECK_MIN_PIXELS = 0

    def _n_chains(self) -> int:
        if self.bb_chains == "1" or self._calib is not None or self.kws is not None:
            return 1
        if torch.cuda.is_current_stream_capturing() and not self._dag_in_capture:
            return 1
        n = 2 if self.bb_chains == "auto" else int(self.bb_chains)
        if self.bb_chains == "auto" and self._depth2_issue:
            return 1
        if self.bb_chains == "auto" and not (self.BB_CHAINS_MIN_PIXELS <= self.B * self.H * self.W < 2 * self.BB_CHAINS_MIN_PIXELS):
            return 1
        while n > 1 and (self.B % n or any(t.numel() % (64 * n) for t in (self.tmp, self.hid, self.ln_part, self.ln_stats) if t is not None)):
            n -= 1
        return max(1, n)

    def _chain_views(self, n: int) -> List["ImageTower"]:
        if self._park_mlp is None:
            self._park_mlp = self.park if self.park is not None else torch.zeros(
                max(1, L.p8_workspace_bytes() // 4), dtype=torch.float32, device=self.dev)
        part = lambda t, h: None if t is None else t[h * (t.numel() // n): (h + 1) * (t.numel() // n)]
        views = []
        for h in range(n):
            v = copy.copy(self)
            v.B = self.B // n
            v.M = [m // n for m in self.M]
            v.x = [t[h * (m // n): (h + 1) * (m // n)] for t, m in zip(self.x, self.M)]
            v.patches = self.patches[h * v.M[0]: (h + 1) * v.M[0]]
            v.tmp, v.hid, v.ln_part, v.ln_stats = part(self.tmp, h), part(self.hid, h), part(self.ln_part, h), part(self.ln_stats, h)
            v._lane_i = 0
            if h:
                if h not in self._chain_parks:
                    if torch.cuda.is_current_stream_capturing():
                        raise L.WedetectHipError("image-chain workspaces must exist before stream capture (run the step eagerly once)")
                    self._chain_parks[h] = torch.zeros(max(1, L.p8_workspace_bytes() // 4), dtype=torch.float32, device=self.dev)
                v.park = self._chain_parks[h] if self.park is not None else None
                v._park_mlp = self._chain_parks[h]
            views.append(v)
        return views

    def backbone(self, images_u8: torch.Tensor) -> List[torch.Tensor]:
        B = self.B
        if images_u8.dtype != torch.uint8 or tuple(images_u8.shape) != (B, self.H, self.W, 3):
            raise L.WedetectHipError(f"images must be uint8 [{B},{self.H},{self.W},3] (RGB, NHWC)")
        if not images_u8.is_contiguous():
            images_u8 = images_u8.contiguous()
        if self._x_sets and self._x_free[self._x_par] is not None and not torch.cuda.is_current_stream_capturing():
            torch.cuda.current_stream().wait_event(self._x_free[self._x_par])
        n = self._n_chains()
        first, last = self.bb_chain_stages if n > 1 else (0, 3)
        if n == 1 or first > 0:
            for _ in self._backbone_blocks(images_u8, 0, 3 if n == 1 else first - 1):
                pass
        if n > 1:
            self._backbone_chains(images_u8, n, first, last)
            if last < 3:
                for _ in self._backbone_blocks(None, last + 1, 3):
                    pass
        return self.x

    def _backbone_chains(self, images_u8: torch.Tensor, n: int, first: int, last: int) -> None:
        views = self._chain_views(n)
        if len(self._chain_streams) < n - 1:
            self._chain_streams = device_streams(self.dev, "chains", n - 1)
        while len(self._chain_evs) < 3 * n:
            self._chain_evs.append(torch.cuda.Event())
        done, ev_dw, ev_mlp = self._chain_evs[:n], self._chain_evs[n:2 * n], self._chain_evs[2 * n:3 * n]
        main = torch.cuda.current_stream()
        streams = [main] + self._chain_streams[: n - 1]
        done[0].record(main)
        gens, pending = [], []
        for h, v in enumerate(views):
            if h:
                streams[h].wait_event(done[0])
            gens.append(ImageTower._backbone_blocks(v, images_u8[h * v.B: (h + 1) * v.B], first, last))
            pending.append(next(gens[h]))
        order = self.bb_chain_order
        rec_dw, rec_mlp = [False] * n, [False] * n
        alive = list(range(n))
        while alive:
            for h in list(alive):
                tag, before = pending[h], (h - 1) % n
                with (torch.cuda.stream(streams[h]) if h else contextlib.nullcontext()):
                    if tag == "dw" and order in ("dw", "both") and rec_dw[before]:
                        streams[h].wait_event(ev_dw[before])
                    if tag == "mlp" and order in ("gemm", "both") and rec_mlp[before]:
                        streams[h].wait_event(ev_mlp[before])
                    try:
                        pending[h] = next(gens[h])
                    except StopIteration:
                        alive.remove(h)
                        if h:
                            done[h].record(streams[h])
                    if tag == "dw" and order in ("dw", "both"):
                        ev_dw[h].record(streams[h])
                        rec_dw[h] = True
                    if tag == "mlp" and order in ("gemm", "both"):
                        ev_mlp[h].record(streams[h])
                        rec_mlp[h] = True
        for h in range(1, n):
            main.wait_event(done[h])

    def _backbone_blocks(self, images_u8: Optional[torch.Tensor], first: int = 0, last: int = 3):
        a, B = self.a, self.B
        if first == 0:
            yield "stem"
            self._stem(images_u8)
        for i in range(first, last + 1):
            yield from self._stage(i)

    def _stem(self, images_u8: torch.Tensor) -> None:
        a = self.a
        if self.fuse_stem and a.dims[0] in L.STEM_FUSED_WIDTHS:
            L.stem_fused(images_u8, self.P["stem.w"], self.P["stem.b"], self.P["stem.ln_w"], self.P["stem.ln_b"], self.x[0])
        else:
            L.stem_patchify(images_u8, self.patches)
            h0, w0 = self.hw[0]
            self._conv(self.patches, "stem.w", "stem.b", self.x[0], hin=h0, win=w0, cin=48, lda=48, n=a.dims[0],
                       ldc=a.dims[0])
            L.layernorm_rows(self.x[0], self.x[0], self.P["stem.ln_w"], self.P["stem.ln_b"], self.M[0], a.dims[0])

    def _stage(self, i: int):
        a, B = self.a, self.B
        c = a.dims[i]
        h, w = self.hw[i]
        pre = self.precision == "fp16x3" and c % 8 == 0 and (i == 0 or a.dims[i - 1] % 8 == 0)
        fa = L.SPLIT_A if pre else 0
        if i > 0:
            yield "down"
            cp = a.dims[i - 1]
            hp, wp = self.hw[i - 1]
            if pre and hp % 2 == 0 and wp % 2 == 0 and self.s2d_down:
                g_, b_ = self._ln_params(f"down{i}.ln_w", f"down{i}.ln_b", f"down{i}.ln")
                L.layernorm_rows_split_s2d(self.x[i - 1], self.tmp, g_, b_, B, hp, wp, cp)
                self._gemm(self.tmp, f"down{i}.w", f"down{i}.b", self.x[i], hin=h, win=w, cin=4 * cp, lda=4 * cp, n=c,
                           ldc=c, split_flags=fa, a_key=f"down{i}.ln")
            else:
                g_, b_ = self._ln_params(f"down{i}.ln_w", f"down{i}.ln_b", f"down{i}.ln" if pre else None)
                L.layernorm_rows(self.x[i - 1], self.tmp, g_, b_, self.M[i - 1], cp, split=pre)
                self._record(f"down{i}.ln", self.tmp[: self.M[i - 1] * cp])
                self._gemm(self.tmp, f"down{i}.w", f"down{i}.b", self.x[i], hin=hp, win=wp, cin=cp, lda=cp, kh=2, kw=2,
                           stride=2, pad=0, n=c, ldc=c, split_flags=fa, a_key=f"down{i}.ln" if pre else None)
        for j in range(a.depths[i]):
            q = f"s{i}.{j}."
            yield "dw"
            if self._fold_ok(i, pre) and not self.sscale.get(q + "fold_off"):
                self._prepare_fold()
                self._fold_weights(q)
                L.dwconv7_stats(self.x[i], self.P[q + "dw_w"], self.P[q + "dw_b"], self.tmp, self.ln_part, B, h, w, c,
                                scale=self.sscale.get(q + "dw", 1.0))
                L.ln_stats_finalize(self.ln_part, self.ln_stats, self.M[i], c)
                yield "mlp"
                if c in self.fuse_mlp_wide and L.mlp_wide_supported(self.M[i], c, 4 * c):
                    self._mlp_fused_fold(q, i)
                    continue
                self._conv(self.tmp, q + "w1g", q + "v", self.hid, hin=h, win=w, cin=c, lda=c, n=4 * c, ldc=4 * c,
                           act=L.ACT_GELU, split_flags=L.SPLIT_A | L.SPLIT_C, a_key=q + "dw", c_key=q + "hid",
                           ln_stats=self.ln_stats, ln_u=self.P[q + "u"])
                self._conv(self.hid, q + "w2", q + "b2", self.x[i], hin=h, win=w, cin=4 * c, lda=4 * c, n=c, ldc=c,
                           res=self.x[i], ldres=c, split_flags=fa, a_key=q + "hid")
                continue
            g_, b_ = self._ln_params(q + "ln_w", q + "ln_b", q + "ln" if pre else None)
            if c % 32 == 0 and (self.fuse_dwln == "1" or (self.fuse_dwln == "auto" and (c <= 128 or c in self.fuse_dwln_wide))):
                L.dwconv7_ln(self.x[i], self.P[q + "dw_w"], self.P[q + "dw_b"], self.tmp, g_, b_, B, h, w, c, split=pre)
            else:
                L.dwconv7(self.x[i], self.P[q + "dw_w"], self.P[q + "dw_b"], self.tmp, B, h, w, c)
                if self._calib is not None and self.ln_fold:
                    self._record(q + "dw", self.tmp[: self.M[i] * c])
                    d = self.tmp[: self.M[i] * c].view(self.M[i], c)
                    self._calib[q + "dw.mr"] = (d.mean(dim=1).abs() / d.std(dim=1, unbiased=False).clamp_min(1e-30)).max()
                L.layernorm_rows(self.tmp, self.tmp, g_, b_, self.M[i], c, split=pre)
            self._record(q + "ln", self.tmp[: self.M[i] * c])
            yield "mlp"
            if pre and self.fuse_mlp and L.mlp_fused_supported(self.M[i], c, 4 * c):
                self._mlp_fused(q, i)
                continue
            if pre and c in self.fuse_mlp_wide and L.mlp_wide_supported(self.M[i], c, 4 * c):
                self._mlp_fused(q, i, wide=True)
                continue
            self._conv(self.tmp, q + "w1", q + "b1", self.hid, hin=h, win=w, cin=c, lda=c, n=4 * c, ldc=4 * c,
                       act=L.ACT_GELU, split_flags=(L.SPLIT_A | L.SPLIT_C) if pre else 0,
                       a_key=q + "ln" if pre else None, c_key=q + "hid")
            self._conv(self.hid, q + "w2", q + "b2", self.x[i], hin=h, win=w, cin=4 * c, lda=4 * c, n=c, ldc=c,
                       res=self.x[i], ldres=c, split_flags=fa, a_key=q + "hid" if pre else None)

    def _bepc3(self, name: str, x, ldx: int, cin: int, hw: Tuple[int, int], out, cout: int, xkey: str, okey: str):
        bf = self._bep[name]
        c_ = bf["c_"]
        h, w = hw
        nb = self.a.neck_repeats // 2
        cat = bf["cat"]
        S = self._neck_split()
        fl = (L.SPLIT_A | L.SPLIT_C) if S else 0
        sfx = "s" if S else ""
        D = self._dag_on()

        def cv2():
            self._conv(x, f"{name}.cv2.w", f"{name}.cv2.b", cat[:, c_:], hin=h, win=w, cin=cin, lda=ldx, n=c_,
                       ldc=2 * c_, act=L.ACT_SILU, split_flags=fl, a_key=xkey, c_key=name + ".cat")
        ev_cv2 = None
        if D:
            ev_in = self._mark()
            with self._lane(3):
                self._after(ev_in)
                cv2()
                ev_cv2 = self._mark()
        self._conv(x, f"{name}.cv1.w", f"{name}.cv1.b", bf["u0" + sfx], hin=h, win=w, cin=cin, lda=ldx, n=c_, ldc=c_,
                   act=L.ACT_SILU, split_flags=fl, c2=bf["u0"] if S else None, ldc2=c_ if S else 0, a_key=xkey, c_key=name + ".u0")
        cur, nxt = "u0", "u1"
        for j in range(nb):
            s = f"{name}.m{j}"
            self._conv(bf[cur + sfx], s + ".c1.w", s + ".c1.b", bf["t"], hin=h, win=w, cin=c_, lda=c_, n=c_, ldc=c_, k=3,
                       act=L.ACT_SILU, split_flags=fl, a_key=f"{name}.{cur}", c_key=name + ".t")
            last = j == nb - 1
            dst, ldd = (cat, 2 * c_) if last else (bf[nxt + sfx], c_)
            self._conv(bf["t"], s + ".c2.w", s + ".c2.b", dst, hin=h, win=w, cin=c_, lda=c_, n=c_, ldc=ldd, k=3,
                       act=L.ACT_SILU, res=bf[cur], ldres=c_, res_alpha=self.P.s[s + ".alpha"], split_flags=fl,
                       c2=bf[nxt] if (S and not last) else None, ldc2=c_ if (S and not last) else 0,
                       a_key=name + ".t", c_key=name + ".cat" if last else f"{name}.{nxt}")
            cur, nxt = nxt, cur
        if D:
            self._after(ev_cv2)
        else:
            cv2()
        self._conv(cat, f"{name}.cv3.w", f"{name}.cv3.b", out, hin=h, win=w, cin=2 * c_, lda=2 * c_, n=cout,
                   ldc=cout, act=L.ACT_SILU, split_flags=fl, a_key=name + ".cat", c_key=okey)

    def _bifusion_mid(self, name: str, mid, c_mid: int, hw_mid, cat, cout: int, midkey: str):
        hm, wm = hw_mid
        fc = L.SPLIT_C if self._neck_split() else 0
        self._conv(mid, name + ".cv1.w", name + ".cv1.b", cat[:, cout:], hin=hm, win=wm, cin=c_mid, lda=c_mid, n=cout,
                   ldc=3 * cout, act=L.ACT_RELU, fp32=True, split_flags=fc, a_key=midkey, c_key=name + ".cat")

    def _bifusion_low(self, name: str, low, c_low: int, hw_low, cat, tbuf, cout: int, lowkey: str):
        hl, wl = hw_low
        S = self._neck_split()
        fl = (L.SPLIT_A | L.SPLIT_C) if S else 0
        fc = L.SPLIT_C if S else 0
        self._conv(low, name + ".cv2.w", name + ".cv2.b", tbuf, hin=hl, win=wl, cin=c_low, lda=c_low, n=cout, ldc=cout,
                   act=L.ACT_RELU, fp32=True, split_flags=fc, a_key=lowkey, c_key=name + ".t")
        self._conv(tbuf, name + ".downsample.w", name + ".downsample.b", cat[:, 2 * cout:], hin=hl, win=wl, cin=cout,
                   lda=cout, n=cout, ldc=3 * cout, k=3, stride=2, act=L.ACT_RELU, split_flags=fl, a_key=name + ".t",
                   c_key=name + ".cat")

    def _bifusion(self, name: str, top, ld_top: int, hw_top, mid, c_mid: int, hw_mid, low, c_low: int, hw_low,
                  cat, tbuf, out, cout: int, topkey: str, midkey: str, lowkey: str, okey: str, pre=None):
        ht, wt = hw_top
        hm, wm = hw_mid
        fl = (L.SPLIT_A | L.SPLIT_C) if self._neck_split() else 0
        self._gemm(top, name + ".up.w", name + ".up.b", cat, hin=ht, win=wt, cin=cout, lda=ld_top, n=4 * cout,
                   ldc=3 * cout, out_mode=L.OUT_DECONV2X2, split_flags=fl, a_key=topkey, c_key=name + ".cat")
        if pre is None:
            self._bifusion_mid(name, mid, c_mid, hw_mid, cat, cout, midkey)
            self._bifusion_low(name, low, c_low, hw_low, cat, tbuf, cout, lowkey)
        else:
            self._after(*pre)
        self._conv(cat, name + ".cv3.w", name + ".cv3.b", out, hin=hm, win=wm, cin=3 * cout, lda=3 * cout, n=cout,
                   ldc=cout, act=L.ACT_RELU, split_flags=fl, a_key=name + ".cat", c_key=okey)

    def neck(self, _level_ready=None) -> List[torch.Tensor]:
        a = self.a
        nc = a.neck_channels
        c1, c2, c3, c4 = self.x
        hw2, hw3, hw4, hw5 = self.hw
        ld4 = nc["d1"] + nc["p5r"]
        ld3 = nc["d2"] + nc["p4r"]
        S = self._neck_split()
        fl = (L.SPLIT_A | L.SPLIT_C) if S else 0
        fpn_out0 = self.cat_n4[:, nc["d1"]:]
        fpn_out1 = self.cat_n3[:, nc["d2"]:]
        D = self._dag_on()
        self._ev_i = 0
        self._head_evs = []
        pre0 = pre1 = None
        if D:
            ev0 = self._mark()
            with self._lane(1):
                self._after(ev0)
                self._bifusion_mid("Bifusion0", c3, nc["c3"], hw4, self.cat_b0, nc["p5r"], "c3")
                e_m0 = self._mark()
                self._bifusion_mid("Bifusion1", c2, nc["c2"], hw3, self.cat_b1, nc["p4r"], "c2")
                e_m1 = self._mark()
            with self._lane(2):
                self._after(ev0)
                self._bifusion_low("Bifusion0", c2, nc["c2"], hw3, self.cat_b0, self.b0_t, nc["p5r"], "c2")
                e_l0 = self._mark()
                self._bifusion_low("Bifusion1", c1, nc["c1"], hw2, self.cat_b1, self.b1_t, nc["p4r"], "c1")
                e_l1 = self._mark()
            pre0, pre1 = (e_m0, e_l0), (e_m1, e_l1)
        self._conv(c4, "reduce_layer0.w", "reduce_layer0.b", fpn_out0, hin=hw5[0], win=hw5[1], cin=nc["c4"],
                   lda=nc["c4"], n=nc["p5r"], ldc=ld4, act=L.ACT_RELU, fp32=True, split_flags=L.SPLIT_C if S else 0,
                   a_key="c4", c_key="cat_n4")
        self._bifusion("Bifusion0", fpn_out0, ld4, hw5, c3, nc["c3"], hw4, c2, nc["c2"], hw3, self.cat_b0, self.b0_t,
                       self.f0, nc["p5r"], "cat_n4", "c3", "c2", "f0", pre=pre0)
        self._bepc3("Rep_p4", self.f0, nc["p5r"], nc["p5r"], hw4, self.f_out0, nc["p5r"], "f0", "f_out0")
        self._conv(self.f_out0, "reduce_layer1.w", "reduce_layer1.b", fpn_out1, hin=hw4[0], win=hw4[1], cin=nc["p5r"],
                   lda=nc["p5r"], n=nc["p4r"], ldc=ld3, act=L.ACT_RELU, split_flags=fl, a_key="f_out0", c_key="cat_n3")
        self._bifusion("Bifusion1", fpn_out1, ld3, hw4, c2, nc["c2"], hw3, c1, nc["c1"], hw2, self.cat_b1, self.b1_t,
                       self.f1, nc["p4r"], "cat_n3", "c2", "c1", "f1", pre=pre1)
        self._bepc3("Rep_p3", self.f1, nc["p4r"], nc["p4r"], hw3, self.p3, nc["p4r"], "f1", "p3")
        if _level_ready is not None:
            _level_ready(0)
        self._conv(self.p3, "downsample2.w", "downsample2.b", self.cat_n3, hin=hw3[0], win=hw3[1], cin=nc["p4r"],
                   lda=nc["p4r"], n=nc["d2"], ldc=ld3, k=3, stride=2, act=L.ACT_RELU, split_flags=fl, a_key="p3", c_key="cat_n3")
        self._bepc3("Rep_n3", self.cat_n3, ld3, ld3, hw4, self.p4, nc["n3"], "cat_n3", "p4")
        if _level_ready is not None:
            _level_ready(1)
        self._conv(self.p4, "downsample1.w", "downsample1.b", self.cat_n4, hin=hw4[0], win=hw4[1], cin=nc["n3"],
                   lda=nc["n3"], n=nc["d1"], ldc=ld4, k=3, stride=2, act=L.ACT_RELU, split_flags=fl, a_key="p4", c_key="cat_n4")
        self._bepc3("Rep_n4", self.cat_n4, ld4, ld4, hw5, self.p5, nc["n4"], "cat_n4", "p5")
        self._ev_after_neck = self._ev_i
        if _level_ready is not None:
            _level_ready(2)
        return [self.p3, self.p4, self.p5]

    def _head_level(self, l: int) -> None:
        feat, cin = (self.p3, self.p4, self.p5)[l], self.a.head_in[l]
        S = self._neck_split()
        fl = (L.SPLIT_A | L.SPLIT_C) if S else 0
        fa = L.SPLIT_A if S else 0
        h, w = self.lv[l]

        def cls_branch():
            c1, c2 = self.hc[l]
            self._conv(feat, f"head{l}.cls0.w", f"head{l}.cls0.b", c1, hin=h, win=w, cin=cin, lda=cin, n=CLS_MID,
                       ldc=CLS_MID, k=3, act=L.ACT_SILU, split_flags=fl, a_key=f"p{l + 3}", c_key=f"h{l}.c1")
            self._conv(c1, f"head{l}.cls1.w", f"head{l}.cls1.b", c2, hin=h, win=w, cin=CLS_MID, lda=CLS_MID, n=CLS_MID,
                       ldc=CLS_MID, k=3, act=L.ACT_SILU, split_flags=fl, a_key=f"h{l}.c1", c_key=f"h{l}.c2")
            dst = self.embed.view(-1, EMBED_DIM)[self.off[l]:]
            if self._embed_split_on and S:
                self._conv(c2, f"head{l}.embed.w", f"head{l}.embed.b", self.embed_s[self.off[l]:], hin=h, win=w, cin=CLS_MID,
                           lda=CLS_MID, n=EMBED_DIM, ldc=EMBED_DIM, c_batch_stride=self.ntot, split_flags=fl, a_key=f"h{l}.c2",
                           c_key="embed", c2=dst, ldc2=EMBED_DIM)
            else:
                self._conv(c2, f"head{l}.embed.w", f"head{l}.embed.b", dst, hin=h, win=w, cin=CLS_MID, lda=CLS_MID,
                           n=EMBED_DIM, ldc=EMBED_DIM, c_batch_stride=self.ntot, split_flags=fa, a_key=f"h{l}.c2")

        def reg_branch():
            r1, r2, dist = self.hr[l]
            self._conv(feat, f"head{l}.reg0.w", f"head{l}.reg0.b", r1, hin=h, win=w, cin=cin, lda=cin, n=REG_MID,
                       ldc=REG_MID, k=3, act=L.ACT_SILU, split_flags=fl, a_key=f"p{l + 3}", c_key=f"h{l}.r1")
            self._conv(r1, f"head{l}.reg1.w", f"head{l}.reg1.b", r2, hin=h, win=w, cin=REG_MID, lda=REG_MID, n=REG_MID,
                       ldc=REG_MID, k=3, act=L.ACT_SILU, split_flags=fl, a_key=f"h{l}.r1", c_key=f"h{l}.r2")
            self._conv(r2, f"head{l}.dist.w", f"head{l}.dist.b", dist, hin=h, win=w, cin=REG_MID, lda=REG_MID, n=64,
                       ldc=64, split_flags=fa, a_key=f"h{l}.r2")
            L.dfl_decode(dist, 64, self.boxes, self.B, h, w, STRIDES[l], self.off[l], self.ntot)
        if not self._dag_on():
            cls_branch()
            reg_branch()
            return
        ev = self._mark()
        with self._lane(2):
            self._after(ev)
            reg_branch()
            self._head_evs.append(self._mark())
        if l == 2:
            cls_branch()
        else:
            with self._lane(1):
                self._after(ev)
                cls_branch()
                self._head_evs.append(self._mark())

    def _head_join(self) -> None:
        self._after(*self._head_evs)
        self._head_evs = []

    SIM_SPLIT_MIN = 256
    FALLBACK_RETRY, FALLBACK_RETRY_MAX = 64, 4096
    FOLD_MAX_MEAN_OVER_STD = 64.0

    def want_sim_split(self, num_classes: Optional[int]) -> bool:
        if num_classes is None or self.precision != "fp16x3" or not self._neck_split() or self.sim_split == "0" or self._calib is not None:
            return False
        return self.sim_split == "1" or num_classes >= self.SIM_SPLIT_MIN

    def _begin_head(self, num_classes: Optional[int], standalone: bool = False) -> None:
        if standalone:
            self._ev_i = self._ev_after_neck
            self._head_evs = []
        self._embed_split_on = self.want_sim_split(num_classes)
        if self._embed_split_on and self.embed_s is None:
            rows = (self.B * self.ntot + 7) // 8 * 8
            self.embed_s = torch.empty(rows, EMBED_DIM, dtype=torch.float32, device=self.dev)
            self.generation += 1
        self._embed_split_valid = self._embed_split_on

    def head(self, num_classes: Optional[int] = None) -> Tuple[torch.Tensor, torch.Tensor]:
        self._begin_head(num_classes, standalone=True)
        for l in range(3):
            self._head_level(l)
        self._head_join()
        self._record("embed", self.embed)
        return self.embed, self.boxes

    def similarity(self, text: torch.Tensor, normalize: bool, sigmoid: bool = True,
                   text_counts: Optional[torch.Tensor] = None) -> torch.Tensor:
        if text.dim() == 3 or text_counts is not None:
            return self._similarity_per_image(text, normalize, sigmoid, text_counts)
        k = text.shape[0]
        if text.dtype != torch.float32 or text.shape[1] != EMBED_DIM or not text.is_cuda:
            raise L.WedetectHipError("text bank must be a device float32 [K, 768] tensor")
        if k > self.max_classes:
            self._alloc_post(k)
        if k > self.text_norm.shape[0]:
            self.text_norm = torch.empty(k, EMBED_DIM, dtype=torch.float32, device=self.dev)
            self.generation += 1
        t = text.contiguous()
        out = self.scores.view(-1)[: self.B * self.ntot * k].view(self.B, self.ntot, k)
        seg = (self.ntot, self.off[1], self.off[2], self.lvl_scale, self.lvl_bias)
        if self._embed_split_valid and self.precision == "fp16x3" and self.want_sim_split(k):
            ts = self._split_text(t, normalize)
            if ts is not None:
                L.similarity_split(self.embed_s, self.B * self.ntot, ts[0], ts[1] / self.sscale.get("embed", 1.0), out, k, EMBED_DIM, k,
                                   seg=seg, sigmoid=sigmoid, range_flag=self.range_flag)
                return out
        if normalize:
            L.l2norm_rows(t, self.text_norm[:k])
            t = self.text_norm[:k]
        L.conv_gemm(self.embed, t, None, out, batch=1, hin=1, win=self.B * self.ntot, cin=EMBED_DIM, lda=EMBED_DIM,
                    n=k, ldc=k, sigmoid=sigmoid, seg=seg)
        return out

    def _similarity_per_image(self, text: torch.Tensor, normalize: bool, sigmoid: bool,
                              text_counts: Optional[torch.Tensor]) -> torch.Tensor:
        if not isinstance(text, torch.Tensor) or text.dim() != 3 or text.dtype != torch.float32 or text.shape[2] != EMBED_DIM \
                or not text.is_cuda or text.device != self.embed.device or text.shape[1] < 1:
            raise L.WedetectHipError("per-image text banks must be one device float32 [B, k_max, 768] tensor on the tower's device")
        if text.shape[0] != self.B:
            raise L.WedetectHipError(f"per-image text banks: {text.shape[0]} banks for a tower of batch {self.B}")
        if text_counts is not None:
            if not isinstance(text_counts, torch.Tensor) or not text_counts.is_cuda or text_counts.device != self.embed.device:
                raise L.WedetectHipError("text_counts must be a DEVICE int32 [B] tensor (the kernel reads it; the step has no host read)")
            if text_counts.dtype != torch.int32 or tuple(text_counts.shape) != (self.B,):
                raise L.WedetectHipError(f"text_counts must be int32 of shape [{self.B}], got {text_counts.dtype} {tuple(text_counts.shape)}")
            text_counts = text_counts.contiguous()
        k = text.shape[1]
        if k > self.max_classes:
            self._alloc_post(k)
        t = text.contiguous()
        if normalize:
            if self.text_norm_pi is None or self.B * k > self.text_norm_pi.shape[0]:
                self.text_norm_pi = torch.empty(self.B * k, EMBED_DIM, dtype=torch.float32, device=self.dev)
                self.generation += 1
            tn = self.text_norm_pi[: self.B * k]
            L.l2norm_rows(t.view(self.B * k, EMBED_DIM), tn)
            t = tn.view(self.B, k, EMBED_DIM)
        out = self.scores.view(-1)[: self.B * self.ntot * k].view(self.B, self.ntot, k)
        seg = (self.ntot, self.off[1], self.off[2], self.lvl_scale, self.lvl_bias)
        L.similarity_grouped(self.embed, t, text_counts, out, self.B, self.ntot, k, EMBED_DIM, k, seg, sigmoid=sigmoid)
        return out

    def _split_text(self, t: torch.Tensor, normalize: bool):
        for ref, ver, norm, ts in self._text_split:
            if ref() is t and ver == t._version and norm == bool(normalize):
                return ts
        if torch.cuda.is_current_stream_capturing():
            return None
        k = t.shape[0]
        src = t
        if normalize:
            L.l2norm_rows(t, self.text_norm[:k])
            src = self.text_norm[:k]
        ts = L.split_weights(src)
        self._text_split = [e for e in self._text_split if e[0]() is not None][-1:]
        self._text_split.append((weakref.ref(t), t._version, bool(normalize), ts))
        return ts

    NMS_MODES = {"vanilla": L.NMS_VANILLA, "torchvision": L.NMS_TORCHVISION, "mmcv": L.NMS_MMCV}

    def postprocess(self, scores: torch.Tensor, score_thr: float, meta: torch.Tensor, iou_thr: float = 0.7,
                    with_embed: bool = True, nms: str = "vanilla", nms_param: Optional[int] = None,
                    nms_device: str = "cpu") -> Dict[str, torch.Tensor]:
        B, n, k = scores.shape
        mode = self.NMS_MODES[nms]
        if nms_param is None:
            nms_param = {L.NMS_VANILLA: 0, L.NMS_TORCHVISION: L.TV_TRICK_MAX_NUMEL[nms_device], L.NMS_MMCV: L.MMCV_SPLIT_THR}[mode]
        L.topk_candidates(scores, B, n * k, float(np.float32(score_thr)), self.nms_pre, self.cand_idx,
                          self.cand_score, self.cand_count, self.topk_ws)
        L.nms_gather(self.cand_idx, self.cand_score, self.cand_count, self.cap, self.boxes, n, k, meta,
                     L.nms_threshold(iou_thr, mode, nms_device), self.max_out, self.embed if with_embed else None, EMBED_DIM,
                     self.out_boxes, self.out_scores, self.out_labels, self.out_anchors, self.out_count,
                     self.out_embed if with_embed else None, B, nms_mode=mode, mode_param=int(nms_param),
                     workspace=self.nms_ws)
        res = dict(bboxes=self.out_boxes, scores=self.out_scores, labels=self.out_labels, anchors=self.out_anchors,
                   count=self.out_count)
        if with_embed:
            res["embeddings"] = self.out_embed
        return res

    SCALE_TARGET_LOG2 = 10

    def calibrate(self, images_u8: torch.Tensor, merge: bool = False) -> Dict[str, float]:
        self.calibrated = True
        if self.precision != "fp16x3":
            return {}
        self.calibration_runs += 1
        saved = self.precision
        self.precision, self._calib = "fp32", {}
        try:
            self.features(images_u8)
            keys = list(self._calib)
            vals = torch.stack([self._calib[k] for k in keys]).tolist() if keys else []
        finally:
            self.precision, self._calib = saved, None
        amax = dict(zip(keys, vals))
        new = {}
        for k, m in amax.items():
            if k.endswith(".mr"):
                if not (m <= self.FOLD_MAX_MEAN_OVER_STD):
                    new[k[: -len("dw.mr")] + "fold_off"] = 2.0
                continue
            if math.isfinite(m) and m > 0.0:
                sc = 2.0 ** (self.SCALE_TARGET_LOG2 - math.floor(math.log2(m)) - 1)
                if sc != 1.0:
                    new[k] = sc
        if merge:
            keys = set(new) | set(self.sscale)
            off = {k for k in keys if k.endswith("fold_off")}
            new = {k: (2.0 if k in off else min(new.get(k, 1.0), self.sscale.get(k, 1.0))) for k in keys}
            new = {k: v for k, v in new.items() if v != 1.0}
        self.adopt_scales(new)
        self.fold_mean_over_std = {k[: -len(".mr")]: v for k, v in amax.items() if k.endswith(".mr")}
        return {k: v for k, v in amax.items() if not k.endswith(".mr")}

    def adopt_scales(self, sscale: Dict[str, float]) -> None:
        self.calibrated = True
        if dict(sscale) != self.sscale:
            self.sscale = dict(sscale)
            self._ln_scaled.clear()
            self.generation += 1

    def identity_meta(self) -> torch.Tensor:
        m = torch.tensor([0.0, 0.0, 0.0, 1.0, 1.0, float(self.W), float(self.H), 0.0], dtype=torch.float32)
        return m.repeat(self.B, 1).to(self.dev)

    def level_of(self, anchors: torch.Tensor) -> torch.Tensor:
        a = anchors.clamp_min(0)
        return (a >= self.off[1]).to(torch.int64) + (a >= self.off[2]).to(torch.int64)

    def neck_head(self, num_classes: Optional[int] = None):
        if not self._dag_on():
            self.neck()
            return self.head(num_classes)
        self._begin_head(num_classes)
        self.neck(_level_ready=self._head_level)
        self._head_join()
        return self.embed, self.boxes

    def features(self, images_u8: torch.Tensor, num_classes: Optional[int] = None):
        self.wait_post()
        self.backbone(images_u8)
        return self.neck_head(num_classes)

    def detect(self, images_u8, text, meta, *, normalize_text: bool, score_thr: float, iou_thr: float = 0.7,
               with_embed: bool = False, nms: Optional[str] = None, nms_param: Optional[int] = None, nms_device: str = "cpu",
               overlap_post: bool = False, text_counts: Optional[torch.Tensor] = None):
        if nms is None:
            nms = "mmcv" if normalize_text else "torchvision"
        num_classes = None if (text.dim() == 3 or text_counts is not None) else text.shape[0]
        if not overlap_post:
            self.wait_post()
            self.features(images_u8, num_classes=num_classes)
            scores = self.similarity(text, normalize=normalize_text, text_counts=text_counts)
            return self.postprocess(scores, score_thr, meta, iou_thr, with_embed, nms, nms_param, nms_device)
        if self.post_stream is None:
            self.post_stream = device_streams(self.dev, "post")[0]
            self._post_ready = torch.cuda.Event()
        main = torch.cuda.current_stream()
        pipe = self._pipe_neck_on()
        depth = self._bb_depth() if pipe else 1
        bb_stream = main
        if pipe:
            if not self._x_sets:
                self._x_sets = [self.x]
                self._nh_stream = device_streams(self.dev, "nh")[0]
                self._bb_done = [torch.cuda.Event(), torch.cuda.Event()]
            while len(self._x_sets) < depth + 1:
                self._x_sets.append([torch.empty_like(t) for t in self.x])
                self._x_free.append(None)
            self._x_par = (self._x_par + 1) % len(self._x_sets)
            self.x = self._x_sets[self._x_par]
        self._pipe_issue = pipe
        try:
            self._issue_pipelined_backbone(images_u8, main, depth)
        finally:
            self._pipe_issue = False
        bb_stream = self._slot1["stream"] if (depth == 2 and self._bb_slot) else main
        if pipe:
            self._bb_done[self._bb_slot].record(bb_stream)
        nh = self._nh_stream if pipe else main
        with (torch.cuda.stream(nh) if pipe else contextlib.nullcontext()):
            if pipe:
                nh.wait_event(self._bb_done[self._bb_slot])
                self._nh_issue = True
            try:
                if self._dag_on():
                    self.wait_post()
                    self.neck_head(num_classes)
                else:
                    self.neck()
                    self.wait_post()
                    self.head(num_classes)
                scores = self.similarity(text, normalize=normalize_text, text_counts=text_counts)
            finally:
                self._nh_issue = False
            self._post_ready.record(nh)
            if pipe:
                if self._x_free[self._x_par] is None:
                    self._x_free[self._x_par] = torch.cuda.Event()
                self._x_free[self._x_par].record(nh)
        for t_ in (meta, text, text_counts):
            if isinstance(t_, torch.Tensor) and t_.is_cuda:
                t_.record_stream(self.post_stream)
                if pipe:
                    t_.record_stream(nh)
        with torch.cuda.stream(self.post_stream):
            self.post_stream.wait_event(self._post_ready)
            res = self.postprocess(scores, score_thr, meta, iou_thr, with_embed, nms, nms_param, nms_device)
            if self._post_done is None:
                self._post_done = torch.cuda.Event()
            self._post_done.record(self.post_stream)
        return res

    def _issue_pipelined_backbone(self, images_u8: torch.Tensor, main, depth: int) -> None:
        if depth == 2:
            self._bb_slot ^= 1
            self._depth2_issue = True
            try:
                if self._bb_slot:
                    self._slot1_backbone(images_u8, main)
                else:
                    self.backbone(images_u8)
            finally:
                self._depth2_issue = False
        else:
            self._bb_slot = 0
            self.backbone(images_u8)

    def _bb_depth(self) -> int:
        if self.bb_depth == "auto":
            return 2 if self.B * self.H * self.W >= 2 * 640 * 640 else 1
        return 2 if self.bb_depth == "2" else 1

    def _slot1_backbone(self, images_u8: torch.Tensor, main) -> torch.cuda.Stream:
        if self._slot1 is None:
            z = lambda t: None if t is None else torch.empty_like(t)
            self._slot1 = dict(stream=device_streams(self.dev, "bb2")[0], ready=torch.cuda.Event(), img=torch.empty_like(images_u8),
                               tmp=z(self.tmp), hid=z(self.hid), ln_part=z(self.ln_part), ln_stats=z(self.ln_stats), patches=z(self.patches),
                               park=torch.zeros(max(1, L.p8_workspace_bytes() // 4), dtype=torch.float32, device=self.dev))
        s1 = self._slot1
        main.wait_event(self._bb_done[1])
        s1["img"].copy_(images_u8, non_blocking=True)
        s1["ready"].record(main)
        v = copy.copy(self)
        v.tmp, v.hid, v.ln_part, v.ln_stats, v.patches = s1["tmp"], s1["hid"], s1["ln_part"], s1["ln_stats"], s1["patches"]
        v.park = s1["park"] if self.park is not None else None
        v._park_mlp = s1["park"]
        if v.bb_chains != "auto":
            v.bb_chains = "1"
        with torch.cuda.stream(s1["stream"]):
            s1["stream"].wait_event(s1["ready"])
            v.backbone(s1["img"])
        return s1["stream"]

    def _pipe_neck_on(self) -> bool:
        if self.pipe_neck == "0" or self._calib is not None or torch.cuda.is_current_stream_capturing():
            return False
        return self.pipe_neck == "1" or self.B * self.H * self.W >= self.PIPE_NECK_MIN_PIXELS

    def wait_post(self) -> None:
        if self._post_done is not None and not torch.cuda.is_current_stream_capturing():
            torch.cuda.current_stream().wait_event(self._post_done)

    def checked_counts(self, res: Dict[str, torch.Tensor], rerun, recalibrate=None) -> List[int]:
        self.wait_post()
        counts = res["count"].tolist()
        if self.overflowed and self.precision == "fp32" and min(counts, default=0) >= 0:
            self._clean_fp32_steps += 1
            if self._clean_fp32_steps >= self._retry_after and recalibrate is not None:
                self.precision = "fp16x3"
                recalibrate()
                self.overflowed, self._clean_fp32_steps = False, 0
                self.range_flags.zero_()
                self.fp16x3_retries += 1
            return counts
        flags = self.range_flags.tolist() if self.precision == "fp16x3" else [0, 0]
        if flags[1] and not self.neck_pin:
            import warnings
            warnings.warn("wedetect_amd: a backbone residual stream left the fp16 range in a neck input layer; those layers now "
                          "run the fp32 MFMA kernel")
            self.neck_pin = True
            self.range_flags.zero_()
            return self.checked_counts(rerun(), rerun, recalibrate)
        tripped = flags[0] != 0
        if min(counts, default=0) >= 0 and not tripped:
            return counts
        self.range_flags.zero_()
        if self.precision == "fp16x3":
            self.fp16x3_trips += 1
        if self.precision == "fp16x3" and recalibrate is not None:
            before = dict(self.sscale)
            recalibrate()
            if self.sscale != before:
                import warnings
                warnings.warn("wedetect_amd: an activation left the fp16 range under the split scales of an earlier batch; "
                              "re-calibrated on this batch")
                return self.checked_counts(rerun(), rerun, None)
        if self.precision == "fp32":
            raise L.WedetectHipError("non-finite scores in fp32 mode: the checkpoint or the inputs produce inf / NaN")
        import warnings
        warnings.warn("wedetect_amd: an activation left the fp16 range (|x| >= 65504) in an fp16x3 layer; this tower now runs "
                      "the fp32 MFMA kernels (ImageTower(precision='fp32') avoids the detour)")
        self.precision = "fp32"
        self.overflowed = True
        self._clean_fp32_steps = 0
        self._retry_after = min(self.FALLBACK_RETRY_MAX, self.FALLBACK_RETRY if self.fp16x3_retries == 0 else 2 * self._retry_after)
        counts = rerun()["count"].tolist()
        if min(counts, default=0) < 0:
            raise L.WedetectHipError("non-finite scores in fp32 mode: the checkpoint or the inputs produce inf / NaN")
        return counts


class GraphedDetect:

    def __init__(self, tower: ImageTower, num_classes: int, *, normalize_text: bool, score_thr: float,
                 iou_thr: float = 0.7, with_embed: bool = True, warmup: int = 2, nms: Optional[str] = None,
                 nms_param: Optional[int] = None, nms_device: str = "cpu"):
        self.tower = tower
        dev = tower.dev
        self.images = torch.zeros(tower.B, tower.H, tower.W, 3, dtype=torch.uint8, device=dev)
        self.text = torch.zeros(num_classes, EMBED_DIM, dtype=torch.float32, device=dev)
        self.text[:, 0] = 1.0
        self.meta = tower.identity_meta()
        kw = dict(normalize_text=normalize_text, score_thr=score_thr, iou_thr=iou_thr, with_embed=with_embed, nms=nms,
                  nms_param=nms_param, nms_device=nms_device)
        side = torch.cuda.Stream(device=dev)
        side.wait_stream(torch.cuda.current_stream())
        with torch.cuda.stream(side):
            for _ in range(max(1, warmup)):
                tower.detect(self.images, self.text, self.meta, **kw)
        torch.cuda.current_stream().wait_stream(side)
        torch.cuda.synchronize()
        self.graph = torch.cuda.CUDAGraph()
        with torch.cuda.graph(self.graph):
            self.out = tower.detect(self.images, self.text, self.meta, **kw)
        self.generation = tower.generation

    def __call__(self, images_u8: torch.Tensor, text: torch.Tensor, meta: torch.Tensor):
        if self.generation != self.tower.generation:
            raise L.WedetectHipError("stale hipGraph: the tower re-allocated its similarity / top-k buffers (a larger class "
                                     "bank arrived) after this graph was captured; capture a new one")
        self.tower.wait_post()
        self.images.copy_(images_u8, non_blocking=True)
        self.text.copy_(text, non_blocking=True)
        self.meta.copy_(meta, non_blocking=True)
        self.graph.replay()
        return self.out
```

wedetect_amd/lib.py:

```python
from __future__ import annotations

import ctypes as C
import math
import os

import torch

_HERE = os.path.dirname(os.path.abspath(__file__))
LIB_PATH = os.environ.get("WEDETECT_LIB") or os.path.join(_HERE, "libwedetect_hip.so")

ACT_NONE, ACT_RELU, ACT_SILU, ACT_GELU = 0, 1, 2, 3
OUT_ROWS, OUT_DECONV2X2 = 0, 1
SPLIT_A, SPLIT_C = 1, 2
ABI_VERSION = 15
NMS_VANILLA, NMS_TORCHVISION, NMS_MMCV = 0, 1, 2
TV_TRICK_MAX_NUMEL = {"cpu": 4000, "cuda": 20000}
MMCV_SPLIT_THR = 10000

EXPORTS = (
    "wd_abi_version", "wd_strerror", "wd_sizeof_conv_gemm", "wd_conv_gemm", "wd_conv_gemm_tuned", "wd_conv_gemm_config", "wd_stem_patchify", "wd_dwconv7", "wd_dwconv7_variant",
    "wd_layernorm_rows", "wd_l2norm_rows", "wd_dfl_decode", "wd_topk_workspace_bytes", "wd_topk_capacity",
    "wd_topk_candidates", "wd_nms_workspace_bytes", "wd_nms_gather", "wd_retrieval_max",
    "wd_split_weights_bytes", "wd_split_weights", "wd_split_weights_padded", "wd_dwconv7_stats", "wd_ln_stats_finalize", "wd_conv_gemm_split", "wd_conv_gemm_split_ws", "wd_conv_gemm_split_config", "wd_layernorm_rows_split", "wd_layernorm_rows_split_s2d", "wd_letterbox_u8", "wd_retrieval_max_split", "wd_similarity_split", "wd_similarity_grouped", "wd_mlp_fused_wide_ln", "wd_text_embed", "wd_attention_small", "wd_recall_scratch_floats", "wd_recall_match",
    "wd_det_match_workspace_bytes", "wd_det_match_lds_bytes", "wd_det_match", "wd_det_sort", "wd_det_accumulate",
    "wd_max_sigmoid_attn", "wd_adaptive_maxpool_nhwc", "wd_cross_attention_small", "wd_time_next_gemm",
    "wd_cv_resize_paste_u8", "wd_chw_to_hwc_u8", "wd_p8_workspace_bytes", "wd_dwconv7_ln", "wd_probe_lds_dma", "wd_probe_issue", "wd_mlp_fused_split", "wd_mlp_fused_wide", "wd_stem_fused",
)


class WedetectHipMissing(ImportError):
    pass


class WedetectHipError(RuntimeError):
    pass


class ConvGemm(C.Structure):
    _fields_ = [
        ("a", C.c_void_p), ("w", C.c_void_p), ("bias", C.c_void_p), ("res", C.c_void_p), ("c", C.c_void_p),
        ("batch", C.c_int32), ("hin", C.c_int32), ("win", C.c_int32), ("cin", C.c_int32), ("lda", C.c_int32),
        ("kh", C.c_int32), ("kw", C.c_int32), ("stride", C.c_int32), ("pad", C.c_int32),
        ("hout", C.c_int32), ("wout", C.c_int32),
        ("m", C.c_int32), ("n", C.c_int32), ("k", C.c_int32),
        ("ldc", C.c_int32), ("ldres", C.c_int32),
        ("act", C.c_int32), ("out_mode", C.c_int32),
        ("res_alpha", C.c_float), ("out_scale", C.c_float), ("out_bias", C.c_float),
        ("sigmoid", C.c_int32),
        ("c_batch_stride", C.c_int32),
        ("seg_rows", C.c_int32), ("seg_end0", C.c_int32), ("seg_end1", C.c_int32),
        ("seg_scale", C.c_float * 3), ("seg_bias", C.c_float * 3),
        ("range_flag", C.c_void_p),
        ("c2", C.c_void_p), ("ldc2", C.c_int32),
        ("a_scale", C.c_float), ("c_split_scale", C.c_float),
        ("ln_stats", C.c_void_p), ("ln_u", C.c_void_p),
    ]


def _load():
    if not os.path.exists(LIB_PATH):
        raise WedetectHipMissing(
            f"{LIB_PATH} not found: build it with `python -m wedetect_amd.build` (hipcc, gfx950). "
            "wedetect_amd has no CPU or PyTorch fallback path.")
    lib = C.CDLL(LIB_PATH)
    for name in EXPORTS:
        if not hasattr(lib, name):
            raise WedetectHipMissing(f"{LIB_PATH} does not export {name}")
    vp, i32, i64, f32 = C.c_void_p, C.c_int32, C.c_int64, C.c_float
    lib.wd_abi_version.restype = C.c_int
    lib.wd_strerror.restype = C.c_char_p
    lib.wd_strerror.argtypes = [C.c_int]
    lib.wd_conv_gemm.argtypes = [C.POINTER(ConvGemm), vp]
    lib.wd_conv_gemm_tuned.argtypes = [C.POINTER(ConvGemm), i32, vp]
    lib.wd_conv_gemm_config.restype = C.c_char_p
    lib.wd_conv_gemm_config.argtypes = [i32, i32, i32]
    lib.wd_stem_patchify.argtypes = [vp, vp, i32, i32, i32, vp]
    lib.wd_dwconv7.argtypes = [vp, vp, vp, vp, i32, i32, i32, i32, vp]
    lib.wd_dwconv7_variant.argtypes = [vp, vp, vp, vp, i32, i32, i32, i32, i32, vp]
    lib.wd_layernorm_rows.argtypes = [vp, vp, vp, vp, i64, i32, i32, i32, f32, vp]
    lib.wd_l2norm_rows.argtypes = [vp, vp, i64, i32, vp]
    lib.wd_dfl_decode.argtypes = [vp, i32, vp, i32, i32, i32, i32, i32, i32, vp]
    lib.wd_topk_workspace_bytes.restype = i64
    lib.wd_topk_workspace_bytes.argtypes = [i32, i64, i32]
    lib.wd_topk_capacity.restype = i32
    lib.wd_topk_capacity.argtypes = [i32]
    lib.wd_topk_candidates.argtypes = [vp, i32, i64, f32, i32, vp, vp, vp, vp, i64, vp]
    lib.wd_nms_workspace_bytes.restype = i64
    lib.wd_nms_workspace_bytes.argtypes = [i32]
    lib.wd_nms_gather.argtypes = [vp, vp, vp, i32, vp, i32, i32, vp, f32, i32, i32, i32, vp, i32, vp, vp, vp, vp, vp, vp, i32, vp, i64, vp]
    lib.wd_retrieval_max.argtypes = [vp, vp, vp, vp, vp, vp, i32, i32, i32, i32, vp]
    lib.wd_split_weights_bytes.restype = i64
    lib.wd_split_weights_bytes.argtypes = [i32, i32]
    lib.wd_split_weights.argtypes = [vp, i32, i32, f32, vp, vp]
    lib.wd_split_weights_padded.argtypes = [vp, i32, i32, f32, vp, vp]
    lib.wd_dwconv7_stats.argtypes = [vp, vp, vp, vp, vp, i32, i32, i32, i32, f32, vp]
    lib.wd_similarity_split.argtypes = [vp, i64, vp, f32, vp, i32, i32, i32, i32, i32, i32, C.POINTER(C.c_float), C.POINTER(C.c_float), i32, vp, vp]
    lib.wd_similarity_grouped.argtypes = [vp, vp, vp, vp, i32, i32, i32, i32, i32, i32, i32, C.POINTER(C.c_float), C.POINTER(C.c_float), i32, vp]
    lib.wd_ln_stats_finalize.argtypes = [vp, vp, i64, i32, f32, vp]
    lib.wd_conv_gemm_split.argtypes = [C.POINTER(ConvGemm), vp, f32, i32, i32, vp]
    lib.wd_conv_gemm_split_ws.argtypes = [C.POINTER(ConvGemm), vp, f32, i32, i32, vp, i64, i32, vp]
    lib.wd_layernorm_rows_split.argtypes = [vp, vp, vp, vp, i64, i32, i32, i32, f32, vp]
    lib.wd_layernorm_rows_split_s2d.argtypes = [vp, vp, vp, vp, i32, i32, i32, i32, f32, vp]
    lib.wd_retrieval_max_split.argtypes = [vp, vp, f32, vp, vp, vp, vp, i32, i32, i32, i32, vp, vp]
    lib.wd_recall_scratch_floats.restype = i64
    lib.wd_recall_scratch_floats.argtypes = [i32, i32]
    lib.wd_recall_match.argtypes = [vp, vp, vp, vp, i32, vp, i32, vp, i64, vp, i32, i32, vp]
    lib.wd_det_match_workspace_bytes.restype = i64
    lib.wd_det_match_workspace_bytes.argtypes = [i32, i32]
    lib.wd_det_match_lds_bytes.restype = i32
    lib.wd_det_match_lds_bytes.argtypes = []
    lib.wd_det_match.argtypes = [vp, vp, vp, vp, vp, i32, vp, vp, vp, vp, vp, vp, vp, vp, i32, vp, vp, vp, vp, vp, i32, vp, vp, vp]
    lib.wd_det_sort.argtypes = [vp, i64, vp]
    lib.wd_det_accumulate.argtypes = [vp, i32, vp, vp, vp, vp, vp, vp, vp, vp, vp, i32, vp, vp, i32, vp, vp, vp, vp]
    lib.wd_text_embed.argtypes = [vp, vp, vp, vp, vp, vp, i64, i32, vp]
    lib.wd_attention_small.argtypes = [vp, vp, vp, i32, i32, i32, i32, i32, i32, vp]
    lib.wd_max_sigmoid_attn.argtypes = [vp, i32, vp, vp, vp, vp, i32, i32, i32, i32, i32, i32, i32, vp]
    lib.wd_adaptive_maxpool_nhwc.argtypes = [vp, i32, vp, i32, i64, i32, i32, i32, i32, i32, vp]
    lib.wd_cross_attention_small.argtypes = [vp, i32, vp, vp, i32, vp, i32, i32, i32, i32, i32, i32, vp]
    lib.wd_time_next_gemm.argtypes = [vp, vp]
    lib.wd_letterbox_u8.argtypes = [vp, i32, i32, vp, vp, i32, vp, vp, i32, vp, vp, i32, i32, i32, i32, i32, i32, i32, i32, i32, vp]
    lib.wd_cv_resize_paste_u8.argtypes = [vp, i32, i32, i32, vp, vp, vp, vp, vp, vp, i32, i32, f32, vp, i32, i32, i32, i32, i32, i32, i32, i32, vp]
    lib.wd_chw_to_hwc_u8.argtypes = [vp, i32, vp, i32, i32, i32, vp]
    lib.wd_dwconv7_ln.argtypes = [vp, vp, vp, vp, vp, vp, i32, i32, i32, i32, f32, i32, vp]
    lib.wd_mlp_fused_split.argtypes = [vp, i64, i32, i32, vp, f32, vp, vp, f32, vp, vp, f32, vp, vp]
    lib.wd_mlp_fused_wide.argtypes = [vp, i64, i32, i32, vp, f32, vp, vp, f32, vp, vp, f32, vp, vp, i64, vp]
    lib.wd_mlp_fused_wide_ln.argtypes = [vp, i64, i32, i32, vp, f32, vp, vp, vp, vp, f32, vp, vp, f32, vp, vp, i64, vp]
    lib.wd_stem_fused.argtypes = [vp, i32, i32, i32, vp, vp, vp, vp, i32, f32, vp, vp]
    lib.wd_probe_issue.argtypes = [i32, i32, i32, i32, i32, vp, vp, vp]
    lib.wd_probe_lds_dma.argtypes = [vp, i64, i32, i32, i32, i32, vp, vp]
    lib.wd_p8_workspace_bytes.restype = i64
    lib.wd_p8_workspace_bytes.argtypes = []
    lib.wd_conv_gemm_split_config.restype = C.c_char_p
    lib.wd_conv_gemm_split_config.argtypes = [i32, i32, i32, i32]
    if lib.wd_sizeof_conv_gemm() != C.sizeof(ConvGemm):
        raise WedetectHipMissing("struct WdConvGemm layout differs between the library and lib.ConvGemm; rebuild")
    if lib.wd_abi_version() != ABI_VERSION:
        raise WedetectHipMissing(f"ABI mismatch: library {lib.wd_abi_version()} vs binding {ABI_VERSION}; rebuild")
    return lib


LIB = _load()


def check(status: int, what: str) -> None:
    if status != 0:
        raise WedetectHipError(f"{what} failed: {LIB.wd_strerror(status).decode()} ({status})")


def stream_ptr() -> int:
    return torch.cuda.current_stream().cuda_stream


def _p(t) -> int:
    return 0 if t is None else t.data_ptr()


def _f32(t: torch.Tensor, name: str) -> torch.Tensor:
    if t.dtype != torch.float32 or not t.is_cuda:
        raise WedetectHipError(f"{name}: expected a CUDA/HIP float32 tensor, got {t.dtype} on {t.device}")
    return t


def conv_gemm(a, w, bias, c, *, batch, hin, win, cin, lda, kh=1, kw=1, stride=1, pad=0, hout=None, wout=None,
              n, ldc, act=ACT_NONE, res=None, ldres=0, res_alpha=1.0, out_mode=OUT_ROWS,
              out_scale=1.0, out_bias=0.0, sigmoid=False, c_batch_stride=0, seg=None, tuned_cfg=None,
              w_split=None, split_cfg=-1, split_flags=0, workspace=None, k_splits=0, range_flag=None, c2=None, ldc2=0, a_scale=1.0, c_split_scale=1.0,
              ln_stats=None, ln_u=None) -> None:
    hout = (hin + 2 * pad - kh) // stride + 1 if hout is None else hout
    wout = (win + 2 * pad - kw) // stride + 1 if wout is None else wout
    p = ConvGemm(a=_p(a), w=_p(w), bias=_p(bias), res=_p(res), c=_p(c), batch=batch, hin=hin, win=win, cin=cin,
                 lda=lda, kh=kh, kw=kw, stride=stride, pad=pad, hout=hout, wout=wout,
                 m=batch * hout * wout, n=n, k=kh * kw * cin, ldc=ldc, ldres=ldres, act=act, out_mode=out_mode,
                 res_alpha=res_alpha, out_scale=out_scale, out_bias=out_bias, sigmoid=int(bool(sigmoid)),
                 c_batch_stride=c_batch_stride, range_flag=_p(range_flag), c2=_p(c2), ldc2=ldc2, a_scale=a_scale, c_split_scale=c_split_scale,
                 ln_stats=_p(ln_stats), ln_u=_p(ln_u))
    if seg is not None:
        p.seg_rows, p.seg_end0, p.seg_end1 = int(seg[0]), int(seg[1]), int(seg[2])
        p.seg_scale = (C.c_float * 3)(*[float(v) for v in seg[3]])
        p.seg_bias = (C.c_float * 3)(*[float(v) for v in seg[4]])
    if w_split is not None:
        if workspace is not None:
            check(LIB.wd_conv_gemm_split_ws(C.byref(p), _p(w_split[0]), float(w_split[1]), int(split_flags), int(split_cfg),
                                            _p(workspace), workspace.numel() * workspace.element_size(), int(k_splits),
                                            stream_ptr()), f"wd_conv_gemm_split_ws[{split_cfg}]")
            return
        check(LIB.wd_conv_gemm_split(C.byref(p), _p(w_split[0]), float(w_split[1]), int(split_flags), int(split_cfg),
                                     stream_ptr()),
              f"wd_conv_gemm_split[{split_cfg}]")
        return
    if tuned_cfg is not None:
        check(LIB.wd_conv_gemm_tuned(C.byref(p), int(tuned_cfg), stream_ptr()), f"wd_conv_gemm_tuned[{tuned_cfg}]")
        return
    check(LIB.wd_conv_gemm(C.byref(p), stream_ptr()), "wd_conv_gemm")


def mlp_fused_supported(rows: int, c: int, hidden: int) -> bool:
    return c == 128 and hidden == 512 and rows > 0 and rows % 128 == 0


MLP_WIDE_WIDTHS = (256, 512)
MLP_WIDE_FOLD_WIDTHS = (256,)


def mlp_wide_supported(rows: int, c: int, hidden: int) -> bool:
    return c in MLP_WIDE_WIDTHS and hidden == 4 * c and rows > 0 and rows % 128 == 0


def mlp_wide_pack(w_split: torch.Tensor, n: int, k: int) -> torch.Tensor:
    if n % 32 or k % 16 or w_split.numel() != n * k * 4:
        raise WedetectHipError(f"mlp_wide_pack: [{n}][{k}] is not a whole number of 32 x 16 fragments")
    v = w_split.view(n // 32, 32, k // 16, 2, 2, 16)
    return v.permute(0, 2, 4, 3, 1, 5).contiguous().view(-1)


def mlp_fused_wide(a_split, rows, c, hidden, w1_frag, b1, w2_frag, b2, x, hid_scale=1.0, range_flag=None, workspace=None) -> None:
    ws_bytes = 0 if workspace is None else workspace.numel() * workspace.element_size()
    check(LIB.wd_mlp_fused_wide(_p(a_split), rows, c, hidden, _p(w1_frag[0]), float(w1_frag[1]), _p(b1), _p(w2_frag[0]),
                                float(w2_frag[1]), _p(b2), _p(x), float(hid_scale), _p(range_flag), _p(workspace), ws_bytes,
                                stream_ptr()),
          "wd_mlp_fused_wide")


def mlp_fused_wide_ln(d_split, rows, c, hidden, w1g_frag, v, u, ln_stats, w2_frag, b2, x, hid_scale=1.0, range_flag=None, workspace=None) -> None:
    ws_bytes = 0 if workspace is None else workspace.numel() * workspace.element_size()
    check(LIB.wd_mlp_fused_wide_ln(_p(d_split), rows, c, hidden, _p(w1g_frag[0]), float(w1g_frag[1]), _p(v), _p(u), _p(ln_stats),
                                   _p(w2_frag[0]), float(w2_frag[1]), _p(b2), _p(x), float(hid_scale), _p(range_flag), _p(workspace),
                                   ws_bytes, stream_ptr()), "wd_mlp_fused_wide_ln")


def mlp_fused(a_split, rows, c, hidden, w1_split, b1, w2_split, b2, x, hid_scale=1.0, range_flag=None) -> None:
    check(LIB.wd_mlp_fused_split(_p(a_split), rows, c, hidden, _p(w1_split[0]), float(w1_split[1]), _p(b1), _p(w2_split[0]),
                                 float(w2_split[1]), _p(b2), _p(x), float(hid_scale), _p(range_flag), stream_ptr()),
          "wd_mlp_fused_split")


def split_weights(w: torch.Tensor):
    _f32(w, "w")
    n, k = w.shape
    w = w.contiguous()
    amax = float(w.abs().max())
    scale = 1.0 if amax == 0.0 else 2.0 ** (13 - math.floor(math.log2(amax)))
    out = torch.empty(LIB.wd_split_weights_bytes(n, k), dtype=torch.uint8, device=w.device)
    check(LIB.wd_split_weights_padded(_p(w), n, k, scale, _p(out), stream_ptr()), "wd_split_weights_padded")
    return out, 1.0 / scale


def p8_workspace_bytes() -> int:
    return int(LIB.wd_p8_workspace_bytes())


def gemm_config(m: int, n: int, k: int, split: bool = False, conv: bool = False, presplit: bool = False,
                park: bool = False, dma: bool = False, conv3: bool = False) -> str:
    if split and dma and conv3:
        return LIB.wd_conv_gemm_split_config(m, n, k, 5).decode()
    if split and dma:
        return LIB.wd_conv_gemm_split_config(m, n, k, 4).decode()
    if split:
        return LIB.wd_conv_gemm_split_config(m, n, k, 1 if conv else ((3 if park else 2) if presplit else 0)).decode()
    return LIB.wd_conv_gemm_config(m, n, k).decode()


def stem_patchify(img_u8: torch.Tensor, out: torch.Tensor) -> None:
    b, h, w, _ = img_u8.shape
    check(LIB.wd_stem_patchify(_p(img_u8), _p(out), b, h, w, stream_ptr()), "wd_stem_patchify")


STEM_FUSED_WIDTHS = (64, 96, 128, 192)


def stem_fused(img_u8: torch.Tensor, wgt, bias, gamma, beta, out, eps=1e-6) -> None:
    b, h, w, _ = img_u8.shape
    check(LIB.wd_stem_fused(_p(img_u8), b, h, w, _p(wgt), _p(bias), _p(gamma), _p(beta), wgt.shape[0], eps, _p(out),
                            stream_ptr()), "wd_stem_fused")


def dwconv7(x, w7, bias, y, batch, h, w, c, variant: int = 0) -> None:
    if variant:
        check(LIB.wd_dwconv7_variant(_p(x), _p(w7), _p(bias), _p(y), batch, h, w, c, variant, stream_ptr()), "wd_dwconv7_variant")
        return
    check(LIB.wd_dwconv7(_p(x), _p(w7), _p(bias), _p(y), batch, h, w, c, stream_ptr()), "wd_dwconv7")


def dwconv7_stats(x, w7, bias, y_split, part, batch, h, w, c, scale=1.0) -> None:
    check(LIB.wd_dwconv7_stats(_p(x), _p(w7), _p(bias), _p(y_split), _p(part), batch, h, w, c, float(scale), stream_ptr()), "wd_dwconv7_stats")


def ln_stats_finalize(part, stats, rows, c, eps=1e-6) -> None:
    check(LIB.wd_ln_stats_finalize(_p(part), _p(stats), rows, c, float(eps), stream_ptr()), "wd_ln_stats_finalize")


def layernorm_rows(x, y, gamma, beta, rows, c, ldx=None, ldy=None, eps=1e-6, split=False) -> None:
    fn = LIB.wd_layernorm_rows_split if split else LIB.wd_layernorm_rows
    check(fn(_p(x), _p(y), _p(gamma), _p(beta), rows, c, ldx or c, ldy or c, eps, stream_ptr()),
          "wd_layernorm_rows_split" if split else "wd_layernorm_rows")


def layernorm_rows_split_s2d(x, y, gamma, beta, batch, h, w, c, eps=1e-6) -> None:
    check(LIB.wd_layernorm_rows_split_s2d(_p(x), _p(y), _p(gamma), _p(beta), batch, h, w, c, eps, stream_ptr()),
          "wd_layernorm_rows_split_s2d")


def letterbox_u8(src, h, w, bounds_h, kk_h, ksize_h, bounds_v, kk_v, ksize_v, tmp, dst, dst_h, dst_w, new_w, new_h,
                 left, top, fill) -> None:
    check(LIB.wd_letterbox_u8(_p(src), h, w, _p(bounds_h), _p(kk_h), ksize_h, _p(bounds_v), _p(kk_v), ksize_v, _p(tmp),
                              _p(dst), dst_h, dst_w, new_w, new_h, left, top, int(fill[0]), int(fill[1]), int(fill[2]),
                              stream_ptr()), "wd_letterbox_u8")


CVRESIZE_COPY, CVRESIZE_AREA_FAST, CVRESIZE_AREA, CVRESIZE_LINEAR = 0, 1, 2, 3


def cv_resize_paste_u8(src, sh, sw, mode, xa, xidx, xw, ya, yidx, yw, p0, p1, p2, dst, dst_h, dst_w, new_h, new_w, top, left,
                       fill=114, swap_rb=False) -> None:
    check(LIB.wd_cv_resize_paste_u8(_p(src), sh, sw, mode, _p(xa), _p(xidx), _p(xw), _p(ya), _p(yidx), _p(yw), int(p0), int(p1),
                                    float(p2), _p(dst), dst_h, dst_w, new_h, new_w, top, left, int(fill), int(bool(swap_rb)),
                                    stream_ptr()), "wd_cv_resize_paste_u8")


def chw_to_hwc_u8(src, dst) -> None:
    b, c, h, w = src.shape
    if c != 3 or tuple(dst.shape) != (b, h, w, 3) or dst.dtype != torch.uint8 or src.dtype not in (torch.uint8, torch.float32):
        raise WedetectHipError("chw_to_hwc_u8: src [B,3,H,W] uint8|float32, dst [B,H,W,3] uint8")
    if not src.is_contiguous() or not dst.is_contiguous():
        raise WedetectHipError("chw_to_hwc_u8: contiguous tensors only")
    check(LIB.wd_chw_to_hwc_u8(_p(src), int(src.dtype == torch.float32), _p(dst), b, h, w, stream_ptr()), "wd_chw_to_hwc_u8")


def dwconv7_ln(x, w7, bias, y, gamma, beta, batch, h, w, c, eps=1e-6, split=False) -> None:
    check(LIB.wd_dwconv7_ln(_p(x), _p(w7), _p(bias), _p(y), _p(gamma), _p(beta), batch, h, w, c, float(eps), int(bool(split)),
                            stream_ptr()), "wd_dwconv7_ln")


def l2norm_rows(x, y) -> None:
    rows, c = x.shape
    check(LIB.wd_l2norm_rows(_p(x), _p(y), rows, c, stream_ptr()), "wd_l2norm_rows")


def dfl_decode(dist, ld, boxes, batch, hl, wl, stride, anchor_off, anchors_total) -> None:
    check(LIB.wd_dfl_decode(_p(dist), ld, _p(boxes), batch, hl, wl, stride, anchor_off, anchors_total, stream_ptr()),
          "wd_dfl_decode")


def topk_capacity(nms_pre: int) -> int:
    return LIB.wd_topk_capacity(nms_pre)


def topk_workspace_bytes(batch: int, n: int, nms_pre: int) -> int:
    return LIB.wd_topk_workspace_bytes(batch, n, nms_pre)


def topk_candidates(scores, batch, n, thr, nms_pre, out_idx, out_score, out_count, workspace) -> None:
    check(LIB.wd_topk_candidates(_p(scores), batch, n, thr, nms_pre, _p(out_idx), _p(out_score), _p(out_count),
                                 _p(workspace), workspace.numel() * workspace.element_size(), stream_ptr()),
          "wd_topk_candidates")


def nms_workspace_bytes(batch: int) -> int:
    return LIB.wd_nms_workspace_bytes(batch)


def nms_threshold(iou_thr: float, nms_mode: int, device_kind: str = "cpu") -> float:
    import numpy as np
    if device_kind not in TV_TRICK_MAX_NUMEL:
        raise ValueError(f"device_kind must be one of {sorted(TV_TRICK_MAX_NUMEL)}, not {device_kind!r}")
    t = np.float32(iou_thr)
    if nms_mode == NMS_TORCHVISION and device_kind == "cpu" and float(t) > float(iou_thr):
        t = np.nextafter(t, np.float32(-np.inf), dtype=np.float32)
    return float(t)


def nms_gather(cand_idx, cand_score, cand_count, cand_stride, boxes, n_anchor, k, meta, iou_thr, max_out,
               embed, embed_dim, out_boxes, out_scores, out_labels, out_anchors, out_count, out_embed, batch,
               nms_mode: int = NMS_VANILLA, mode_param: int = 0, workspace=None) -> None:
    ws_bytes = 0 if workspace is None else workspace.numel() * workspace.element_size()
    check(LIB.wd_nms_gather(_p(cand_idx), _p(cand_score), _p(cand_count), cand_stride, _p(boxes), n_anchor, k,
                            _p(meta), iou_thr, max_out, nms_mode, mode_param, _p(embed), embed_dim, _p(out_boxes),
                            _p(out_scores), _p(out_labels), _p(out_anchors), _p(out_count), _p(out_embed), batch,
                            _p(workspace), ws_bytes, stream_ptr()),
          "wd_nms_gather")


def retrieval_max(e, t, scale, bias, count, out, n_img, rows_per_img, n_cls, dim) -> None:
    check(LIB.wd_retrieval_max(_p(e), _p(t), _p(scale), _p(bias), _p(count), _p(out), n_img, rows_per_img, n_cls, dim,
                               stream_ptr()), "wd_retrieval_max")


def retrieval_max_split(e, t_split, scale, bias, count, out, n_img, rows_per_img, n_cls, dim, range_flag=None) -> None:
    _f32(e, "e")
    rows = e.reshape(-1, dim).contiguous()
    es = torch.empty(LIB.wd_split_weights_bytes(rows.shape[0], dim), dtype=torch.uint8, device=e.device)
    check(LIB.wd_split_weights_padded(_p(rows), rows.shape[0], dim, 1.0, _p(es), stream_ptr()), "wd_split_weights_padded")
    check(LIB.wd_retrieval_max_split(_p(es), _p(t_split[0]), float(t_split[1]), _p(scale), _p(bias), _p(count), _p(out),
                                     n_img, rows_per_img, n_cls, dim, _p(range_flag), stream_ptr()), "wd_retrieval_max_split")


def similarity_split(e_split, rows, t_split, unscale, out, n_cls, dim, ldo, seg=None, sigmoid=True, range_flag=None) -> None:
    sr, e0, e1 = (int(seg[0]), int(seg[1]), int(seg[2])) if seg is not None else (0, 0, 0)
    sc = (C.c_float * 3)(*[float(v) for v in (seg[3] if seg is not None else (1, 1, 1))])
    sb = (C.c_float * 3)(*[float(v) for v in (seg[4] if seg is not None else (0, 0, 0))])
    check(LIB.wd_similarity_split(_p(e_split), int(rows), _p(t_split), float(unscale), _p(out), int(n_cls), int(dim), int(ldo),
                                  sr, e0, e1, sc, sb, int(bool(sigmoid)), _p(range_flag), stream_ptr()), "wd_similarity_split")


def similarity_grouped(embed, bank, count, out, n_img, rows_per_img, k_max, dim, ldo, seg, sigmoid=True) -> None:
    _f32(embed, "embed"), _f32(bank, "bank"), _f32(out, "out")
    if count is not None and (count.dtype != torch.int32 or not count.is_cuda or count.numel() < n_img or not count.is_contiguous()):
        raise WedetectHipError(f"count: expected a contiguous CUDA/HIP int32 [{n_img}] tensor, got {count.dtype} on {count.device}")
    if int(seg[0]) != int(rows_per_img):
        raise WedetectHipError("seg rows must equal rows_per_img")
    sc = (C.c_float * 3)(*[float(v) for v in seg[3]])
    sb = (C.c_float * 3)(*[float(v) for v in seg[4]])
    check(LIB.wd_similarity_grouped(_p(embed), _p(bank), _p(count), _p(out), int(n_img), int(rows_per_img), int(k_max), int(dim),
                                    int(ldo), int(seg[1]), int(seg[2]), sc, sb, int(bool(sigmoid)), stream_ptr()),
          "wd_similarity_grouped")


def text_embed(ids, pos_ids, word, pos, type0, out) -> None:
    check(LIB.wd_text_embed(_p(ids), _p(pos_ids), _p(word), _p(pos), _p(type0), _p(out), ids.numel(), word.shape[1],
                            stream_ptr()), "wd_text_embed")


def attention_small(qkv, mask, out, n_seq, seq_len, heads, head_dim) -> None:
    check(LIB.wd_attention_small(_p(qkv), _p(mask), _p(out), n_seq, seq_len, heads, head_dim, qkv.shape[1], out.shape[1],
                                 stream_ptr()), "wd_attention_small")


def max_sigmoid_attn(embed, guide, head_bias, head_scale, x, n_img, hw, n_guide, heads, head_channels, out_head_channels) -> None:
    check(LIB.wd_max_sigmoid_attn(_p(embed), embed.stride(0), _p(guide), _p(head_bias), _p(head_scale), _p(x), x.stride(0),
                                  n_img, hw, n_guide, heads, head_channels, out_head_channels, stream_ptr()),
          "wd_max_sigmoid_attn")


def adaptive_maxpool_nhwc(x, out, out_img_stride, n_img, h, w, channels, pool) -> None:
    check(LIB.wd_adaptive_maxpool_nhwc(_p(x), x.stride(0), _p(out), out.stride(0), out_img_stride, n_img, h, w, channels, pool,
                                       stream_ptr()), "wd_adaptive_maxpool_nhwc")


def cross_attention_small(q, k, v, out, n_img, n_q, n_k, heads, head_dim) -> None:
    if k.stride(0) != v.stride(0):
        raise WedetectHipError("k and v must share their row pitch")
    check(LIB.wd_cross_attention_small(_p(q), q.stride(0), _p(k), _p(v), k.stride(0), _p(out), out.stride(0), n_img, n_q, n_k,
                                       heads, head_dim, stream_ptr()), "wd_cross_attention_small")


def time_next_gemm(start: "torch.cuda.Event", stop: "torch.cuda.Event") -> None:
    check(LIB.wd_time_next_gemm(start.cuda_event, stop.cuda_event), "wd_time_next_gemm")
```

Measured before the change: 962.5.

## Fold text embeddings into head projection and recompute kept rows after NMS

Adds a fold path that multiplies the text class bank into the head's contrastive projection weights, so per-anchor similarity scores come straight from a split-fp16 conv GEMM over the c2 features. Embeddings and exact scores are then recomputed only for the rows kept after NMS, using new gather, select and reorder kernels. This avoids materializing the full per-anchor embedding and running the separate similarity GEMM. In exchange it adds folded-weight preparation per text bank, a device-side unscale, ragged-N epilogue stores, and extra post-NMS kernels, and it changes numerical ordering, which the reorder kernel re-sorts to keep.

```diff
diff --git a/__graft_entry__.py b/__graft_entry__.py
--- a/__graft_entry__.py
+++ b/__graft_entry__.py
@@ -13,6 +13,7 @@
     import wedetect_amd.feed
     import wedetect_amd.tile
     import wedetect_amd.views
+    import wedetect_amd.fold
     import wedetect_amd.detector
     import oracle.postprocess
     import oracle.ref_cpu
diff --git a/include/wedetect_hip_fold.h b/include/wedetect_hip_fold.h
--- /dev/null
+++ b/include/wedetect_hip_fold.h
@@ -0,0 +1,32 @@
+#ifndef WEDETECT_HIP_FOLD_H
+#define WEDETECT_HIP_FOLD_H
+
+#include <stdint.h>
+
+#include "wedetect_hip.h"
+
+#ifdef __cplusplus
+extern "C" {
+#endif
+
+int wd_fold_abi_version(void);
+
+int wd_fold_similarity(const WdConvGemm* p, const void* w_split, float w_unscale, const float* w_unscale_dev, void* stream);
+
+int wd_kept_rows_gather(const float* c2_0, const float* c2_1, const float* c2_2, int32_t rows0, int32_t rows1, int32_t rows2,
+                        int32_t row_floats, const int32_t* out_anchors, const int32_t* out_count, int32_t max_out,
+                        int32_t batch, float* gathered, void* stream);
+
+int wd_kept_rows_select(const float* level_embed, int32_t dim, int32_t off1, int32_t off2, const int32_t* out_anchors,
+                        const int32_t* out_count, const int32_t* perm, int32_t max_out, int32_t batch, float* out_embed,
+                        void* stream);
+
+int wd_kept_rows_reorder(const float* level_scores, int32_t k, int32_t n_anchor, int32_t off1, int32_t off2, float* out_boxes,
+                         float* out_scores, int32_t* out_labels, int32_t* out_anchors, const int32_t* out_count,
+                         int32_t max_out, int32_t batch, int32_t* perm, void* stream);
+
+#ifdef __cplusplus
+}
+#endif
+
+#endif
diff --git a/wedetect_amd/build.py b/wedetect_amd/build.py
--- a/wedetect_amd/build.py
+++ b/wedetect_amd/build.py
@@ -8,8 +8,8 @@
 ROOT = os.path.dirname(HERE)
 CSRC = os.path.join(HERE, "csrc")
 LIB = os.path.join(HERE, "libwedetect_hip.so")
-SOURCES = ["abi.hip", "conv_gemm.hip", "similarity_grouped.hip", "split_gemm.hip", "split_gemm_pre.hip", "split_gemm_p8.hip", "split_gemm_p4.hip", "split_gemm_conv.hip", "split_gemm_conv3.hip", "split_gemm_mlp.hip", "split_gemm_mlpw.hip", "probe.hip", "stem.hip", "elementwise.hip", "preprocess.hip", "text.hip", "bricks.hip", "evaluate.hip", "det_eval.hip", "postprocess.hip", "feed.hip", "tile.hip", "views.hip"]
-PUBLIC_HEADERS = ["wedetect_hip.h", "wedetect_hip_feed.h", "wedetect_hip_tile.h", "wedetect_hip_views.h"]
+SOURCES = ["abi.hip", "conv_gemm.hip", "similarity_grouped.hip", "split_gemm.hip", "split_gemm_pre.hip", "split_gemm_p8.hip", "split_gemm_p4.hip", "split_gemm_conv.hip", "split_gemm_conv3.hip", "split_gemm_mlp.hip", "split_gemm_mlpw.hip", "probe.hip", "stem.hip", "elementwise.hip", "preprocess.hip", "text.hip", "bricks.hip", "evaluate.hip", "det_eval.hip", "postprocess.hip", "feed.hip", "tile.hip", "views.hip", "fold.hip"]
+PUBLIC_HEADERS = ["wedetect_hip.h", "wedetect_hip_feed.h", "wedetect_hip_tile.h", "wedetect_hip_views.h", "wedetect_hip_fold.h"]
 HIPCC = os.environ.get("HIPCC", "/opt/rocm/bin/hipcc")
 FLAGS = ["--offload-arch=gfx950", "-O3", "-std=c++17", "-fPIC", "-Wall", "-Wno-unused-function", "-Wno-inline-asm",
          "-I", os.path.join(ROOT, "include"), "-I", CSRC]
diff --git a/wedetect_amd/csrc/fold.hip b/wedetect_amd/csrc/fold.hip
--- /dev/null
+++ b/wedetect_amd/csrc/fold.hip
@@ -0,0 +1,129 @@
+#include "common.h"
+#include "wedetect_hip_fold.h"
+
+namespace {
+
+__global__ void __launch_bounds__(64) kept_rows_gather_kernel(const float* __restrict__ c0, const float* __restrict__ c1,
+                                                              const float* __restrict__ c2, int rows0, int rows1, int rows2,
+                                                              int row_floats, const int* __restrict__ out_anchors,
+                                                              const int* __restrict__ out_count, int max_out, int batch,
+                                                              float* __restrict__ gathered) {
+  const int s = blockIdx.x, b = blockIdx.y, l = blockIdx.z, lane = threadIdx.x;
+  float* dst = gathered + (((size_t)l * batch + b) * max_out + s) * row_floats;
+  const int a = out_anchors[(size_t)b * max_out + s];
+  const int lvl = (a >= rows0) + (a >= rows0 + rows1);
+  const bool take = s < out_count[b] && a >= 0 && a < rows0 + rows1 + rows2 && lvl == l;
+  if (take) {
+    const float* base = l == 0 ? c0 : l == 1 ? c1 : c2;
+    const int rows = l == 0 ? rows0 : l == 1 ? rows1 : rows2;
+    const int pos = a - (l == 0 ? 0 : l == 1 ? rows0 : rows0 + rows1);
+    const float* src = base + ((size_t)b * rows + pos) * row_floats;
+    for (int i = lane * 4; i < row_floats; i += 256) *reinterpret_cast<f32x4*>(dst + i) = *reinterpret_cast<const f32x4*>(src + i);
+  } else {
+    for (int i = lane * 4; i < row_floats; i += 256) *reinterpret_cast<f32x4*>(dst + i) = f32x4{0.f, 0.f, 0.f, 0.f};
+  }
+}
+
+__global__ void __launch_bounds__(64) kept_rows_select_kernel(const float* __restrict__ level_embed, int dim, int off1, int off2,
+                                                              const int* __restrict__ out_anchors,
+                                                              const int* __restrict__ out_count, const int* __restrict__ perm,
+                                                              int max_out, int batch, float* __restrict__ out_embed) {
+  const int s = blockIdx.x, b = blockIdx.y, lane = threadIdx.x;
+  const size_t r = (size_t)b * max_out + s;
+  float* dst = out_embed + r * dim;
+  if (s < out_count[b]) {
+    const int a = out_anchors[r];
+    const int lvl = (a >= off1) + (a >= off2);
+    int from = perm ? perm[r] : s;
+    from = min(max(from, 0), max_out - 1);
+    const float* src = level_embed + (((size_t)lvl * batch + b) * max_out + from) * dim;
+    for (int i = lane * 4; i < dim; i += 256) *reinterpret_cast<f32x4*>(dst + i) = *reinterpret_cast<const f32x4*>(src + i);
+  } else {
+    for (int i = lane * 4; i < dim; i += 256) *reinterpret_cast<f32x4*>(dst + i) = f32x4{0.f, 0.f, 0.f, 0.f};
+  }
+}
+
+constexpr int KEPT_MAX = 1024;
+
+__global__ void __launch_bounds__(256) kept_rows_reorder_kernel(const float* __restrict__ level_scores, int k, int n_anchor,
+                                                                int off1, int off2, float* __restrict__ out_boxes,
+                                                                float* __restrict__ out_scores, int* __restrict__ out_labels,
+                                                                int* __restrict__ out_anchors,
+                                                                const int* __restrict__ out_count, int max_out, int batch,
+                                                                int* __restrict__ perm) {
+  __shared__ f32x4 s_box[KEPT_MAX];
+  __shared__ float s_score[KEPT_MAX];
+  __shared__ int s_label[KEPT_MAX], s_anchor[KEPT_MAX];
+  const int b = blockIdx.x, tid = threadIdx.x;
+  const size_t base = (size_t)b * max_out;
+  const int n = min(max(out_count[b], 0), max_out);
+  for (int s = tid; s < n; s += 256) {
+    const int a = out_anchors[base + s], c = out_labels[base + s];
+    float sc = out_scores[base + s];
+    if (a >= 0 && a < n_anchor && c >= 0 && c < k) {
+      const int lvl = (a >= off1) + (a >= off2);
+      sc = level_scores[(((size_t)lvl * batch + b) * max_out + s) * k + c];
+    }
+    s_score[s] = sc; s_label[s] = c; s_anchor[s] = a;
+    s_box[s] = *reinterpret_cast<const f32x4*>(out_boxes + (base + s) * 4);
+  }
+  __syncthreads();
+  for (int s = tid; s < n; s += 256) {
+    const float sc = s_score[s];
+    const long long idx = (long long)s_anchor[s] * k + s_label[s];
+    int rank = 0;
+    for (int j = 0; j < n; ++j) {
+      const float sj = s_score[j];
+      const long long ij = (long long)s_anchor[j] * k + s_label[j];
+      rank += (sj > sc || (sj == sc && (ij < idx || (ij == idx && j < s)))) ? 1 : 0;
+    }
+    *reinterpret_cast<f32x4*>(out_boxes + (base + rank) * 4) = s_box[s];
+    out_scores[base + rank] = sc;
+    out_labels[base + rank] = s_label[s];
+    out_anchors[base + rank] = s_anchor[s];
+    perm[base + rank] = s;
+  }
+  for (int s = n + tid; s < max_out; s += 256) perm[base + s] = s;
+}
+
+}
+
+extern "C" int wd_fold_abi_version(void) { return 1; }
+
+extern "C" int wd_kept_rows_gather(const float* c2_0, const float* c2_1, const float* c2_2, int32_t rows0, int32_t rows1,
+                                   int32_t rows2, int32_t row_floats, const int32_t* out_anchors, const int32_t* out_count,
+                                   int32_t max_out, int32_t batch, float* gathered, void* stream) {
+  if (!c2_0 || !c2_1 || !c2_2 || !out_anchors || !out_count || !gathered) return WD_ERR_BAD_ARG;
+  if (rows0 <= 0 || rows1 <= 0 || rows2 <= 0 || (long long)rows0 + rows1 + rows2 > 0x7fffffffLL) return WD_ERR_BAD_ARG;
+  if (row_floats < 4 || row_floats > 1024 || (row_floats & 3) || max_out <= 0 || max_out > 65535 || batch <= 0 || batch > 65535)
+    return WD_ERR_BAD_ARG;
+  if (!wd_aligned16(c2_0) || !wd_aligned16(c2_1) || !wd_aligned16(c2_2) || !wd_aligned16(gathered)) return WD_ERR_BAD_ARG;
+  hipLaunchKernelGGL(kept_rows_gather_kernel, dim3(max_out, batch, 3), dim3(64), 0, static_cast<hipStream_t>(stream), c2_0, c2_1,
+                     c2_2, rows0, rows1, rows2, row_floats, out_anchors, out_count, max_out, batch, gathered);
+  return wd_launch_status();
+}
+
+extern "C" int wd_kept_rows_select(const float* level_embed, int32_t dim, int32_t off1, int32_t off2, const int32_t* out_anchors,
+                                   const int32_t* out_count, const int32_t* perm, int32_t max_out, int32_t batch,
+                                   float* out_embed, void* stream) {
+  if (!level_embed || !out_anchors || !out_count || !out_embed) return WD_ERR_BAD_ARG;
+  if (dim <= 0 || (dim & 3) || off1 < 0 || off2 < off1 || max_out <= 0 || max_out > 65535 || batch <= 0 || batch > 65535)
+    return WD_ERR_BAD_ARG;
+  if (!wd_aligned16(level_embed) || !wd_aligned16(out_embed)) return WD_ERR_BAD_ARG;
+  hipLaunchKernelGGL(kept_rows_select_kernel, dim3(max_out, batch), dim3(64), 0, static_cast<hipStream_t>(stream), level_embed,
+                     dim, off1, off2, out_anchors, out_count, perm, max_out, batch, out_embed);
+  return wd_launch_status();
+}
+
+extern "C" int wd_kept_rows_reorder(const float* level_scores, int32_t k, int32_t n_anchor, int32_t off1, int32_t off2,
+                                    float* out_boxes, float* out_scores, int32_t* out_labels, int32_t* out_anchors,
+                                    const int32_t* out_count, int32_t max_out, int32_t batch, int32_t* perm, void* stream) {
+  if (!level_scores || !out_boxes || !out_scores || !out_labels || !out_anchors || !out_count || !perm) return WD_ERR_BAD_ARG;
+  if (k <= 0 || n_anchor <= 0 || off1 < 0 || off2 < off1 || off2 > n_anchor || max_out <= 0 || max_out > KEPT_MAX || batch <= 0 ||
+      batch > 65535)
+    return WD_ERR_BAD_ARG;
+  if (!wd_aligned16(out_boxes)) return WD_ERR_BAD_ARG;
+  hipLaunchKernelGGL(kept_rows_reorder_kernel, dim3(batch), dim3(256), 0, static_cast<hipStream_t>(stream), level_scores, k,
+                     n_anchor, off1, off2, out_boxes, out_scores, out_labels, out_anchors, out_count, max_out, batch, perm);
+  return wd_launch_status();
+}
diff --git a/wedetect_amd/csrc/split_epi_oct.h b/wedetect_amd/csrc/split_epi_oct.h
--- a/wedetect_amd/csrc/split_epi_oct.h
+++ b/wedetect_amd/csrc/split_epi_oct.h
@@ -58,8 +58,16 @@
     *reinterpret_cast<u32x4*>(cp) = u32x4{h0[0], h0[1], h1[0], h1[1]};
     *reinterpret_cast<u32x4*>(cp + 16) = u32x4{l0[0], l0[1], l1[0], l1[1]};
   } else {
-    *reinterpret_cast<f32x4*>(rowp + col) = o0;
-    *reinterpret_cast<f32x4*>(rowp + col + 4) = o1;
+    if (SPECIAL && (((p.n & 7) | (p.ldc & 3)) != 0 || (reinterpret_cast<uintptr_t>(p.c) & 15u) != 0)) {
+#pragma unroll
+      for (int r = 0; r < 4; ++r) {
+        if (col + r < p.n) rowp[col + r] = o0[r];
+        if (col + 4 + r < p.n) rowp[col + 4 + r] = o1[r];
+      }
+    } else {
+      *reinterpret_cast<f32x4*>(rowp + col) = o0;
+      *reinterpret_cast<f32x4*>(rowp + col + 4) = o1;
+    }
   }
 }
 
diff --git a/wedetect_amd/csrc/split_gemm.hip b/wedetect_amd/csrc/split_gemm.hip
--- a/wedetect_amd/csrc/split_gemm.hip
+++ b/wedetect_amd/csrc/split_gemm.hip
@@ -84,7 +84,7 @@
 bool wd_p8_persist_ok(int m, int n);
 bool wd_conv_pp_ok(const WdConvGemm& p, int flags);
 int wd_launch_conv_pp(const WdConvGemm& p, const void* w, float unscale, int flags, hipStream_t st, int ksplits, float* ws,
-                      long long ws_floats, int variant);
+                      long long ws_floats, int variant, const float* unscale_dev = nullptr);
 bool wd_conv3_ok(const WdConvGemm& p, int flags);
 const char* wd_conv3_config_name(int m, int n);
 int wd_launch_conv3(const WdConvGemm& p, const void* w, float unscale, int flags, hipStream_t st, int variant, int ksplits, float* ws,
@@ -245,3 +245,16 @@
   return conv_gemm_split_impl(pp, w_split, w_unscale, flags, cfg, static_cast<float*>(workspace), workspace_bytes, splits,
                               static_cast<hipStream_t>(stream));
 }
+
+extern "C" int wd_fold_similarity(const WdConvGemm* pp, const void* w_split, float w_unscale, const float* w_unscale_dev,
+                                  void* stream) {
+  if (!pp || !w_unscale_dev) return WD_ERR_BAD_ARG;
+  const WdConvGemm& p = *pp;
+  const int rc = check_split_args(p, w_split, w_unscale);
+  if (rc != WD_OK) return rc;
+  if (p.kh != 1 || p.kw != 1 || p.stride != 1 || p.pad != 0 || p.c_batch_stride <= 0 || p.res || p.c2 || p.ln_stats || p.ln_u ||
+      p.seg_rows > 0 || p.act != WD_ACT_NONE)
+    return WD_ERR_BAD_ARG;
+  if (!wd_conv_pp_ok(p, WD_SPLIT_A)) return WD_ERR_UNSUPPORTED;
+  return wd_launch_conv_pp(p, w_split, w_unscale, WD_SPLIT_A, static_cast<hipStream_t>(stream), 1, nullptr, 0, 0, w_unscale_dev);
+}
diff --git a/wedetect_amd/csrc/split_gemm_conv.hip b/wedetect_amd/csrc/split_gemm_conv.hip
--- a/wedetect_amd/csrc/split_gemm_conv.hip
+++ b/wedetect_amd/csrc/split_gemm_conv.hip
@@ -20,7 +20,7 @@
 template <int NBUF, int TN, bool CSPLIT, int ABL = 0>
 __global__ void __launch_bounds__(512, NBUF <= 3 ? 4 : 2)
 split_conv_pp_kernel(const WdConvGemm p, const unsigned char* __restrict__ wsp, const float* __restrict__ zero, int k16,
-                     float unscale, int nbn, int ksplits, float* __restrict__ ws) {
+                     float unscale, int nbn, int ksplits, float* __restrict__ ws, const float* __restrict__ unscale_dev) {
   constexpr int TM = 2, BM = CV_BM, BN = 64 * TN, ROWB = CV_ROWB, STAGE = CV_STAGE, NI = CV_NI, DIST = NBUF - 1;
   extern __shared__ __attribute__((aligned(16))) unsigned char smem_raw[];
   const int t = threadIdx.x, lane = t & 63, wave = t >> 6;
@@ -212,7 +212,8 @@
     EpiOctWalk<0, TM, TN, WD_ACT_NONE, false, false, false>::run(pr, 1.0f, mw, nw, lane, acc, patch, ops);
     return;
   }
-  epi_oct_all<TM, TN, CSPLIT, (NBUF == 4 || TN == 1)>(p, unscale, mw, nw, lane, acc, patch);
+  const float us = unscale_dev ? unscale * *unscale_dev : unscale;
+  epi_oct_all<TM, TN, CSPLIT, (NBUF == 4 || TN == 1)>(p, us, mw, nw, lane, acc, patch);
 }
 
 template <int ACT, bool SPECIAL, bool CSPLIT>
@@ -259,7 +260,8 @@
 }
 
 template <int NBUF, int TN, bool CSPLIT, int ABL = 0>
-int launch_conv_pp(const WdConvGemm& p, const void* wsp, float unscale, hipStream_t st, int ksplits, float* ws) {
+int launch_conv_pp(const WdConvGemm& p, const void* wsp, float unscale, hipStream_t st, int ksplits, float* ws,
+                   const float* unscale_dev) {
   constexpr int BN = 64 * TN, LDS = NBUF * CV_STAGE;
   const int nbm = (p.m + CV_BM - 1) / CV_BM, nbn = (p.n + BN - 1) / BN;
   const long long nblk = (long long)nbm * nbn * ksplits;
@@ -271,7 +273,7 @@
   static WdAttrOnce attr;
   if (wd_set_max_lds(attr, reinterpret_cast<const void*>(k), LDS) != WD_OK) return WD_ERR_LAUNCH;
   WD_LAUNCH_GEMM(k, dim3((unsigned)nblk), dim3(512), LDS, st, p, static_cast<const unsigned char*>(wsp), zero, k16, unscale,
-                 nbn, ksplits, ws);
+                 nbn, ksplits, ws, unscale_dev);
   return wd_launch_status();
 }
 
@@ -283,24 +285,28 @@
 
 bool wd_conv_pp_ok(const WdConvGemm& p, int flags) {
   if (!(flags & WD_SPLIT_A)) return false;
-  if (p.cin % 16 || p.k % 16 || p.lda % 8 || p.kh * p.kw > 16 || p.n % 8) return false;
-  if (!wd_aligned16(p.a) || !wd_aligned16(p.c)) return false;
+  const bool special = p.out_mode != WD_OUT_ROWS || p.c_batch_stride > 0 || p.seg_rows > 0 || p.sigmoid ||
+                       p.out_scale != 1.0f || p.out_bias != 0.0f;
+  const bool ragged_ok = special && !(flags & WD_SPLIT_C) && p.out_mode == WD_OUT_ROWS && !p.res && !p.c2;
+  if (p.cin % 16 || p.k % 16 || p.lda % 8 || p.kh * p.kw > 16 || (p.n % 8 && !ragged_ok)) return false;
+  if (!wd_aligned16(p.a) || (!wd_aligned16(p.c) && !ragged_ok)) return false;
   if (p.bias && !wd_aligned16(p.bias)) return false;
   if (p.res && (!wd_aligned16(p.res) || p.ldres % 4)) return false;
   if (p.c2 && (!(flags & WD_SPLIT_C) || !wd_aligned16(p.c2) || p.ldc2 % 4 || p.ldc2 < p.n || p.out_mode != WD_OUT_ROWS))
     return false;
-  if ((flags & WD_SPLIT_C) ? (p.ldc % 8 != 0) : (p.ldc % 4 != 0)) return false;
+  if ((flags & WD_SPLIT_C) ? (p.ldc % 8 != 0) : (p.ldc % 4 != 0 && !ragged_ok)) return false;
   if (p.out_mode == WD_OUT_DECONV2X2 && (p.n % 32)) return false;
   return true;
 }
 
 int wd_launch_conv_pp(const WdConvGemm& p, const void* w, float unscale, int flags, hipStream_t st, int ksplits, float* ws,
-                      long long ws_floats, int variant) {
+                      long long ws_floats, int variant, const float* unscale_dev) {
   if (!wd_conv_pp_ok(p, flags)) return WD_ERR_UNSUPPORTED;
   const bool csplit = (flags & WD_SPLIT_C) != 0;
   const bool narrow = (p.n % 128) != 0 && ((p.n + 63) / 64) * 64 < ((p.n + 127) / 128) * 128;
   const long long tiles = (long long)((p.m + CV_BM - 1) / CV_BM) * (narrow ? (p.n + 63) / 64 : (p.n + 127) / 128);
   if (ksplits < 1) ksplits = 1;
+  if (ksplits > 1 && (p.n % 8 || p.ldc % 4 || !wd_aligned16(p.c) || unscale_dev)) return WD_ERR_UNSUPPORTED;
   if (ksplits > 1 && (!ws || (long long)ksplits * p.m * p.n > ws_floats)) return WD_ERR_WORKSPACE;
   if (ksplits > (p.k >> 4)) ksplits = p.k >> 4;
   int nbuf = (tiles * ksplits <= 256) ? 4 : 3;
@@ -309,19 +315,19 @@
 #ifdef WD_DEBUG_ABLATIONS
   if (variant >= 100 && variant < 116 && !narrow && csplit) {
     switch (variant - 100) {
-      case 1: return launch_conv_pp<4, 2, true, 1>(p, w, unscale, st, 1, ws);
-      case 2: return launch_conv_pp<4, 2, true, 2>(p, w, unscale, st, 1, ws);
-      case 3: return launch_conv_pp<4, 2, true, 3>(p, w, unscale, st, 1, ws);
-      case 4: return launch_conv_pp<4, 2, true, 4>(p, w, unscale, st, 1, ws);
-      case 7: return launch_conv_pp<4, 2, true, 7>(p, w, unscale, st, 1, ws);
-      case 8: return launch_conv_pp<4, 2, true, 8>(p, w, unscale, st, 1, ws);
-      case 11: return launch_conv_pp<4, 2, true, 11>(p, w, unscale, st, 1, ws);
-      case 15: return launch_conv_pp<4, 2, true, 15>(p, w, unscale, st, 1, ws);
+      case 1: return launch_conv_pp<4, 2, true, 1>(p, w, unscale, st, 1, ws, nullptr);
+      case 2: return launch_conv_pp<4, 2, true, 2>(p, w, unscale, st, 1, ws, nullptr);
+      case 3: return launch_conv_pp<4, 2, true, 3>(p, w, unscale, st, 1, ws, nullptr);
+      case 4: return launch_conv_pp<4, 2, true, 4>(p, w, unscale, st, 1, ws, nullptr);
+      case 7: return launch_conv_pp<4, 2, true, 7>(p, w, unscale, st, 1, ws, nullptr);
+      case 8: return launch_conv_pp<4, 2, true, 8>(p, w, unscale, st, 1, ws, nullptr);
+      case 11: return launch_conv_pp<4, 2, true, 11>(p, w, unscale, st, 1, ws, nullptr);
+      case 15: return launch_conv_pp<4, 2, true, 15>(p, w, unscale, st, 1, ws, nullptr);
       default: break;
     }
   }
 #endif
-#define WD_CPP(NB, TNN, CS) launch_conv_pp<NB, TNN, CS>(p, w, unscale, st, ksplits, ws)
+#define WD_CPP(NB, TNN, CS) launch_conv_pp<NB, TNN, CS>(p, w, unscale, st, ksplits, ws, unscale_dev)
   if (nbuf == 4) {
     if (narrow) rc = csplit ? WD_CPP(4, 1, true) : WD_CPP(4, 1, false);
     else rc = csplit ? WD_CPP(4, 2, true) : WD_CPP(4, 2, false);
diff --git a/wedetect_amd/engine.py b/wedetect_amd/engine.py
--- a/wedetect_amd/engine.py
+++ b/wedetect_amd/engine.py
@@ -4,12 +4,14 @@
 import copy
 import math
 import os
+import warnings
 import weakref
 from typing import Dict, List, Optional, Sequence, Tuple
 
 import numpy as np
 import torch
 
+from . import fold as FD
 from . import lib as L
 from .arch import ArchSpec, CLS_MID, EMBED_DIM, REG_MID, STRIDES, get_arch, level_sizes
 from .pack import Packed
@@ -124,6 +126,21 @@
         self._embed_split_on = False
         self._embed_split_valid = False
         self._text_split: list = []
+        self.fold_text = os.environ.get("WEDETECT_FOLD_TEXT", "1") != "0"
+        self._text_fold: list = []
+        self.fold_launches = 0
+        self.embed_materialised = 0
+        self._per_image_seen = False
+        self.fold_declined_per_image = 0
+        self._fold_cur: Optional[dict] = None
+        self._embed_valid = True
+        self._c2_ready: Optional[torch.cuda.Event] = None
+        self._kept_g: Optional[torch.Tensor] = None
+        self._kept_t: Optional[torch.Tensor] = None
+        self._kept_es: Optional[torch.Tensor] = None
+        self._kept_s: Optional[torch.Tensor] = None
+        self._kept_perm: Optional[torch.Tensor] = None
+        self._scores_fold: Optional[tuple] = None
         self.overflowed = False
         self.fp16x3_trips = 0
         self.fp16x3_retries = 0
@@ -169,7 +186,7 @@
         self.nl = [h * w for h, w in self.lv]
         self.ntot = sum(self.nl)
         self.off = [0, self.nl[0], self.nl[0] + self.nl[1]]
-        self.embed = f(B, self.ntot, EMBED_DIM)
+        self._embed = f(B, self.ntot, EMBED_DIM)
         self.boxes = f(B, self.ntot, 4)
         self.hc = [(f(B * n, CLS_MID), f(B * n, CLS_MID)) for n in self.nl]
         self.hr = [(f(B * n, REG_MID), f(B * n, REG_MID), f(B * n, 4 * 16)) for n in self.nl]
@@ -199,9 +216,25 @@
         self.lvl_logit_scale = [float(np.float32(self.P.s[f"head{l}.logit_scale"])) for l in range(3)]
         self._prepare_fold()
 
+    @property
+    def embed(self) -> torch.Tensor:
+        if not self._embed_valid:
+            self._materialise_embed()
+        return self._embed
+
+    def _materialise_embed(self) -> None:
+        if torch.cuda.is_current_stream_capturing():
+            raise L.WedetectHipError("ImageTower.embed read under stream capture after a folded step")
+        self._after(self._c2_ready)
+        for l in range(3):
+            self._embed_conv(l, False)
+        self._embed_valid = True
+        self.embed_materialised += 1
+
     def _alloc_post(self, k: int) -> None:
         self.max_classes = k
         self.generation += 1
+        self._kept_s = None
         self.scores = torch.empty(self.B, self.ntot, k, dtype=torch.float32, device=self.dev)
         nbytes = L.topk_workspace_bytes(self.B, self.ntot * k, self.nms_pre)
         self.topk_ws = torch.empty(nbytes + 256, dtype=torch.uint8, device=self.dev)
@@ -813,14 +846,8 @@
                        ldc=CLS_MID, k=3, act=L.ACT_SILU, split_flags=fl, a_key=f"p{l + 3}", c_key=f"h{l}.c1")
             self._conv(c1, f"head{l}.cls1.w", f"head{l}.cls1.b", c2, hin=h, win=w, cin=CLS_MID, lda=CLS_MID, n=CLS_MID,
                        ldc=CLS_MID, k=3, act=L.ACT_SILU, split_flags=fl, a_key=f"h{l}.c1", c_key=f"h{l}.c2")
-            dst = self.embed.view(-1, EMBED_DIM)[self.off[l]:]
-            if self._embed_split_on and S:
-                self._conv(c2, f"head{l}.embed.w", f"head{l}.embed.b", self.embed_s[self.off[l]:], hin=h, win=w, cin=CLS_MID,
-                           lda=CLS_MID, n=EMBED_DIM, ldc=EMBED_DIM, c_batch_stride=self.ntot, split_flags=fl, a_key=f"h{l}.c2",
-                           c_key="embed", c2=dst, ldc2=EMBED_DIM)
-            else:
-                self._conv(c2, f"head{l}.embed.w", f"head{l}.embed.b", dst, hin=h, win=w, cin=CLS_MID, lda=CLS_MID,
-                           n=EMBED_DIM, ldc=EMBED_DIM, c_batch_stride=self.ntot, split_flags=fa, a_key=f"h{l}.c2")
+            if self._fold_cur is None:
+                self._embed_conv(l, self._embed_split_on and S)
 
         def reg_branch():
             r1, r2, dist = self.hr[l]
@@ -848,6 +875,18 @@
                 cls_branch()
                 self._head_evs.append(self._mark())
 
+    def _embed_conv(self, l: int, split: bool) -> None:
+        (h, w), c2 = self.lv[l], self.hc[l][1]
+        S = self._neck_split()
+        dst = self._embed.view(-1, EMBED_DIM)[self.off[l]:]
+        if split:
+            self._conv(c2, f"head{l}.embed.w", f"head{l}.embed.b", self.embed_s[self.off[l]:], hin=h, win=w, cin=CLS_MID,
+                       lda=CLS_MID, n=EMBED_DIM, ldc=EMBED_DIM, c_batch_stride=self.ntot, split_flags=L.SPLIT_A | L.SPLIT_C,
+                       a_key=f"h{l}.c2", c_key="embed", c2=dst, ldc2=EMBED_DIM)
+        else:
+            self._conv(c2, f"head{l}.embed.w", f"head{l}.embed.b", dst, hin=h, win=w, cin=CLS_MID, lda=CLS_MID,
+                       n=EMBED_DIM, ldc=EMBED_DIM, c_batch_stride=self.ntot, split_flags=L.SPLIT_A if S else 0, a_key=f"h{l}.c2")
+
     def _head_join(self) -> None:
         self._after(*self._head_evs)
         self._head_evs = []
@@ -861,27 +900,29 @@
             return False
         return self.sim_split == "1" or num_classes >= self.SIM_SPLIT_MIN
 
-    def _begin_head(self, num_classes: Optional[int], standalone: bool = False) -> None:
+    def _begin_head(self, num_classes: Optional[int], standalone: bool = False, fold: Optional[dict] = None) -> None:
         if standalone:
             self._ev_i = self._ev_after_neck
             self._head_evs = []
-        self._embed_split_on = self.want_sim_split(num_classes)
+        self._fold_cur = fold
+        self._embed_valid = fold is None
+        self._embed_split_on = fold is None and self.want_sim_split(num_classes)
         if self._embed_split_on and self.embed_s is None:
             rows = (self.B * self.ntot + 7) // 8 * 8
             self.embed_s = torch.empty(rows, EMBED_DIM, dtype=torch.float32, device=self.dev)
             self.generation += 1
         self._embed_split_valid = self._embed_split_on
 
-    def head(self, num_classes: Optional[int] = None) -> Tuple[torch.Tensor, torch.Tensor]:
-        self._begin_head(num_classes, standalone=True)
+    def head(self, num_classes: Optional[int] = None, _fold: Optional[dict] = None) -> Tuple[torch.Tensor, torch.Tensor]:
+        self._begin_head(num_classes, standalone=True, fold=_fold)
         for l in range(3):
             self._head_level(l)
         self._head_join()
-        self._record("embed", self.embed)
-        return self.embed, self.boxes
+        self._record("embed", self._embed)
+        return self._embed, self.boxes
 
     def similarity(self, text: torch.Tensor, normalize: bool, sigmoid: bool = True,
-                   text_counts: Optional[torch.Tensor] = None) -> torch.Tensor:
+                   text_counts: Optional[torch.Tensor] = None, _fold: Optional[dict] = None) -> torch.Tensor:
         if text.dim() == 3 or text_counts is not None:
             return self._similarity_per_image(text, normalize, sigmoid, text_counts)
         k = text.shape[0]
@@ -895,6 +936,11 @@
         t = text.contiguous()
         out = self.scores.view(-1)[: self.B * self.ntot * k].view(self.B, self.ntot, k)
         seg = (self.ntot, self.off[1], self.off[2], self.lvl_scale, self.lvl_bias)
+        self._scores_fold = None
+        if _fold is not None:
+            self._similarity_folded(_fold, out, k, sigmoid)
+            self._scores_fold = (_fold, bool(sigmoid))
+            return out
         if self._embed_split_valid and self.precision == "fp16x3" and self.want_sim_split(k):
             ts = self._split_text(t, normalize)
             if ts is not None:
@@ -904,19 +950,21 @@
         if normalize:
             L.l2norm_rows(t, self.text_norm[:k])
             t = self.text_norm[:k]
-        L.conv_gemm(self.embed, t, None, out, batch=1, hin=1, win=self.B * self.ntot, cin=EMBED_DIM, lda=EMBED_DIM,
+        L.conv_gemm(self._embed, t, None, out, batch=1, hin=1, win=self.B * self.ntot, cin=EMBED_DIM, lda=EMBED_DIM,
                     n=k, ldc=k, sigmoid=sigmoid, seg=seg)
         return out
 
     def _similarity_per_image(self, text: torch.Tensor, normalize: bool, sigmoid: bool,
                               text_counts: Optional[torch.Tensor]) -> torch.Tensor:
         if not isinstance(text, torch.Tensor) or text.dim() != 3 or text.dtype != torch.float32 or text.shape[2] != EMBED_DIM \
-                or not text.is_cuda or text.device != self.embed.device or text.shape[1] < 1:
+                or not text.is_cuda or text.device != self._embed.device or text.shape[1] < 1:
             raise L.WedetectHipError("per-image text banks must be one device float32 [B, k_max, 768] tensor on the tower's device")
         if text.shape[0] != self.B:
             raise L.WedetectHipError(f"per-image text banks: {text.shape[0]} banks for a tower of batch {self.B}")
+        self._per_image_seen = True
+        self._scores_fold = None
         if text_counts is not None:
-            if not isinstance(text_counts, torch.Tensor) or not text_counts.is_cuda or text_counts.device != self.embed.device:
+            if not isinstance(text_counts, torch.Tensor) or not text_counts.is_cuda or text_counts.device != self._embed.device:
                 raise L.WedetectHipError("text_counts must be a DEVICE int32 [B] tensor (the kernel reads it; the step has no host read)")
             if text_counts.dtype != torch.int32 or tuple(text_counts.shape) != (self.B,):
                 raise L.WedetectHipError(f"text_counts must be int32 of shape [{self.B}], got {text_counts.dtype} {tuple(text_counts.shape)}")
@@ -934,7 +982,7 @@
             t = tn.view(self.B, k, EMBED_DIM)
         out = self.scores.view(-1)[: self.B * self.ntot * k].view(self.B, self.ntot, k)
         seg = (self.ntot, self.off[1], self.off[2], self.lvl_scale, self.lvl_bias)
-        L.similarity_grouped(self.embed, t, text_counts, out, self.B, self.ntot, k, EMBED_DIM, k, seg, sigmoid=sigmoid)
+        L.similarity_grouped(self._embed, t, text_counts, out, self.B, self.ntot, k, EMBED_DIM, k, seg, sigmoid=sigmoid)
         return out
 
     def _split_text(self, t: torch.Tensor, normalize: bool):
@@ -953,6 +1001,109 @@
         self._text_split.append((weakref.ref(t), t._version, bool(normalize), ts))
         return ts
 
+    def _fold_for(self, text: torch.Tensor, text_counts, normalize: bool) -> Optional[dict]:
+        if self._per_image_seen:
+            if self.fold_text and text_counts is None and text.dim() == 2 and self.precision == "fp16x3":
+                self.fold_declined_per_image += 1
+            return None
+        if (not self.fold_text or text_counts is not None or text.dim() != 2 or self.precision != "fp16x3" or not self._neck_split()
+                or self._calib is not None or text.dtype != torch.float32 or text.shape[1] != EMBED_DIM or not text.is_cuda):
+            return None
+        if self.want_sim_split(text.shape[0]) and torch.cuda.is_current_stream_capturing():
+            return None
+        return self._fold_text(text.contiguous(), normalize)
+
+    def _fold_text(self, t: torch.Tensor, normalize: bool) -> Optional[dict]:
+        for ref, ver, norm, ent in self._text_fold:
+            if ref() is t and ver == t._version and norm == bool(normalize):
+                return ent
+        if torch.cuda.is_current_stream_capturing():
+            return None
+        ent = self._fold_compute(t, normalize, None)
+        self._text_fold = [e for e in self._text_fold if e[0]() is not None][-1:]
+        self._text_fold.append((weakref.ref(t), t._version, bool(normalize), ent))
+        return ent
+
+    def _fold_compute(self, t: torch.Tensor, normalize: bool, ent: Optional[dict]) -> dict:
+        k = t.shape[0]
+        k8 = (k + 7) // 8 * 8
+        if ent is None:
+            nbytes = int(L.LIB.wd_split_weights_bytes(k, CLS_MID))
+            ent = dict(k=k, w=[torch.empty(nbytes, dtype=torch.uint8, device=self.dev) for _ in range(3)],
+                       b=torch.zeros(3, k8, dtype=torch.float32, device=self.dev),
+                       u=torch.empty(3, dtype=torch.float32, device=self.dev),
+                       tn=torch.empty_like(t))
+        elif ent["k"] != k:
+            raise L.WedetectHipError(f"refold in place: a bank of {k} rows into a fold of {ent['k']}")
+        src = ent["tn"]
+        if normalize:
+            L.l2norm_rows(t, src)
+        else:
+            src.copy_(t)
+        if self.want_sim_split(k):
+            ent["ts"] = L.split_weights(src)
+        else:
+            ent.pop("ts", None)
+        t64 = src.double()
+        for l in range(3):
+            we = self.P[f"head{l}.embed.w"].view(EMBED_DIM, -1)
+            wf = (t64 @ we.double()).float()
+            ent["b"][l, :k].copy_((t64 @ self.P[f"head{l}.embed.b"].double()).float())
+            _, ex = torch.frexp(wf.abs().max())
+            one = torch.ones((), dtype=torch.float32, device=self.dev)
+            L.split_weights_scaled(wf * torch.ldexp(one, 14 - ex), ent["w"][l])
+            ent["u"][l].copy_(torch.ldexp(one, ex - 14))
+        self.fold_launches += 1
+        return ent
+
+    def _similarity_folded(self, ent: dict, out: torch.Tensor, k: int, sigmoid: bool) -> None:
+        if self._nh_issue:
+            for t_ in (*ent["w"], ent["b"], ent["u"]):
+                t_.record_stream(torch.cuda.current_stream())
+        flat = out.view(-1)
+        for l in range(3):
+            sa = self.sscale.get(f"h{l}.c2", 1.0)
+            FD.fold_similarity(self.hc[l][1], ent["w"][l], 1.0 / sa, ent["u"][l:l + 1], ent["b"][l], flat[self.off[l] * k:],
+                               batch=self.B, rows=self.nl[l], cin=CLS_MID, n=k, c_batch_stride=self.ntot,
+                               out_scale=self.lvl_scale[l], out_bias=self.lvl_bias[l], sigmoid=sigmoid, range_flag=self.range_flag)
+
+    def _kept_rows(self, ent: dict, sigmoid: bool, with_embed: bool) -> None:
+        rows, k = self.B * self.max_out, ent["k"]
+        if self._kept_g is None:
+            self._kept_g = torch.empty(3, rows, CLS_MID, dtype=torch.float32, device=self.dev)
+            self._kept_t = torch.empty(3, rows, EMBED_DIM, dtype=torch.float32, device=self.dev)
+            self._kept_perm = torch.empty(self.B, self.max_out, dtype=torch.int32, device=self.dev)
+        if self._kept_s is None:
+            self._kept_s = torch.empty(3 * rows * self.max_classes, dtype=torch.float32, device=self.dev)
+        if not torch.cuda.is_current_stream_capturing():
+            for t_ in (ent["tn"], *(ent["ts"][:1] if ent.get("ts") is not None else ())):
+                t_.record_stream(torch.cuda.current_stream())
+        ks = self._kept_s[: 3 * rows * k].view(3, rows, k)
+        ts = ent.get("ts") if self.want_sim_split(k) else None
+        if ts is not None and self._kept_es is None:
+            self._kept_es = torch.zeros(3, (rows + 7) // 8 * 8, EMBED_DIM, dtype=torch.float32, device=self.dev)
+        FD.kept_rows_gather([c[1] for c in self.hc], self.nl, CLS_MID, self.out_anchors, self.out_count, self.max_out, self.B,
+                            self._kept_g)
+        for l in range(3):
+            seg = (rows, rows if l == 0 else 0, rows if l < 2 else 0, self.lvl_scale, self.lvl_bias)
+            if ts is not None:
+                self._conv(self._kept_g[l], f"head{l}.embed.w", f"head{l}.embed.b", self._kept_es[l], hin=1, win=self.max_out,
+                           cin=CLS_MID, lda=CLS_MID, n=EMBED_DIM, ldc=EMBED_DIM, c_batch_stride=self.max_out,
+                           split_flags=L.SPLIT_A | L.SPLIT_C, a_key=f"h{l}.c2", c_key="embed", c2=self._kept_t[l], ldc2=EMBED_DIM)
+                L.similarity_split(self._kept_es[l], rows, ts[0], ts[1] / self.sscale.get("embed", 1.0), ks[l], k, EMBED_DIM, k,
+                                   seg=seg, sigmoid=sigmoid, range_flag=self.range_flag)
+                continue
+            self._conv(self._kept_g[l], f"head{l}.embed.w", f"head{l}.embed.b", self._kept_t[l], hin=1, win=self.max_out,
+                       cin=CLS_MID, lda=CLS_MID, n=EMBED_DIM, ldc=EMBED_DIM, c_batch_stride=self.max_out, split_flags=L.SPLIT_A,
+                       a_key=f"h{l}.c2")
+            L.conv_gemm(self._kept_t[l], ent["tn"], None, ks[l], batch=1, hin=1, win=rows, cin=EMBED_DIM, lda=EMBED_DIM,
+                        n=k, ldc=k, sigmoid=sigmoid, seg=seg)
+        FD.kept_rows_reorder(ks, k, self.ntot, self.off[1], self.off[2], self.out_boxes, self.out_scores, self.out_labels,
+                             self.out_anchors, self.out_count, self.max_out, self.B, self._kept_perm)
+        if with_embed:
+            FD.kept_rows_select(self._kept_t, EMBED_DIM, self.off[1], self.off[2], self.out_anchors, self.out_count, self.max_out,
+                                self.B, self.out_embed, self._kept_perm)
+
     NMS_MODES = {"vanilla": L.NMS_VANILLA, "torchvision": L.NMS_TORCHVISION, "mmcv": L.NMS_MMCV}
 
     def postprocess(self, scores: torch.Tensor, score_thr: float, meta: torch.Tensor, iou_thr: float = 0.7,
@@ -964,11 +1115,19 @@
             nms_param = {L.NMS_VANILLA: 0, L.NMS_TORCHVISION: L.TV_TRICK_MAX_NUMEL[nms_device], L.NMS_MMCV: L.MMCV_SPLIT_THR}[mode]
         L.topk_candidates(scores, B, n * k, float(np.float32(score_thr)), self.nms_pre, self.cand_idx,
                           self.cand_score, self.cand_count, self.topk_ws)
+        folded = self._scores_fold if scores.data_ptr() == self.scores.data_ptr() else None
+        if folded is not None and folded[0]["k"] != k:
+            folded = None
+        gather = with_embed and folded is None
+        if gather and not self._embed_valid:
+            self._materialise_embed()
         L.nms_gather(self.cand_idx, self.cand_score, self.cand_count, self.cap, self.boxes, n, k, meta,
-                     L.nms_threshold(iou_thr, mode, nms_device), self.max_out, self.embed if with_embed else None, EMBED_DIM,
+                     L.nms_threshold(iou_thr, mode, nms_device), self.max_out, self._embed if gather else None, EMBED_DIM,
                      self.out_boxes, self.out_scores, self.out_labels, self.out_anchors, self.out_count,
-                     self.out_embed if with_embed else None, B, nms_mode=mode, mode_param=int(nms_param),
+                     self.out_embed if gather else None, B, nms_mode=mode, mode_param=int(nms_param),
                      workspace=self.nms_ws)
+        if folded is not None:
+            self._kept_rows(folded[0], folded[1], with_embed)
         res = dict(bboxes=self.out_boxes, scores=self.out_scores, labels=self.out_labels, anchors=self.out_anchors,
                    count=self.out_count)
         if with_embed:
@@ -1025,19 +1184,19 @@
         a = anchors.clamp_min(0)
         return (a >= self.off[1]).to(torch.int64) + (a >= self.off[2]).to(torch.int64)
 
-    def neck_head(self, num_classes: Optional[int] = None):
+    def neck_head(self, num_classes: Optional[int] = None, _fold: Optional[dict] = None):
         if not self._dag_on():
             self.neck()
-            return self.head(num_classes)
-        self._begin_head(num_classes)
+            return self.head(num_classes, _fold)
+        self._begin_head(num_classes, fold=_fold)
         self.neck(_level_ready=self._head_level)
         self._head_join()
-        return self.embed, self.boxes
-
-    def features(self, images_u8: torch.Tensor, num_classes: Optional[int] = None):
+        return self._embed, self.boxes
+
+    def features(self, images_u8: torch.Tensor, num_classes: Optional[int] = None, _fold: Optional[dict] = None):
         self.wait_post()
         self.backbone(images_u8)
-        return self.neck_head(num_classes)
+        return self.neck_head(num_classes, _fold)
 
     def detect(self, images_u8, text, meta, *, normalize_text: bool, score_thr: float, iou_thr: float = 0.7,
                with_embed: bool = False, nms: Optional[str] = None, nms_param: Optional[int] = None, nms_device: str = "cpu",
@@ -1045,10 +1204,12 @@
         if nms is None:
             nms = "mmcv" if normalize_text else "torchvision"
         num_classes = None if (text.dim() == 3 or text_counts is not None) else text.shape[0]
+        fold = self._fold_for(text, text_counts, normalize_text)
         if not overlap_post:
             self.wait_post()
-            self.features(images_u8, num_classes=num_classes)
-            scores = self.similarity(text, normalize=normalize_text, text_counts=text_counts)
+            self.features(images_u8, num_classes=num_classes, _fold=fold)
+            scores = self.similarity(text, normalize=normalize_text, text_counts=text_counts, _fold=fold)
+            self._mark_c2(fold)
             return self.postprocess(scores, score_thr, meta, iou_thr, with_embed, nms, nms_param, nms_device)
         if self.post_stream is None:
             self.post_stream = device_streams(self.dev, "post")[0]
@@ -1083,12 +1244,13 @@
             try:
                 if self._dag_on():
                     self.wait_post()
-                    self.neck_head(num_classes)
+                    self.neck_head(num_classes, fold)
                 else:
                     self.neck()
                     self.wait_post()
-                    self.head(num_classes)
-                scores = self.similarity(text, normalize=normalize_text, text_counts=text_counts)
+                    self.head(num_classes, fold)
+                scores = self.similarity(text, normalize=normalize_text, text_counts=text_counts, _fold=fold)
+                self._mark_c2(fold)
             finally:
                 self._nh_issue = False
             self._post_ready.record(nh)
@@ -1108,6 +1270,13 @@
                 self._post_done = torch.cuda.Event()
             self._post_done.record(self.post_stream)
         return res
+
+    def _mark_c2(self, fold: Optional[dict]) -> None:
+        if fold is None or torch.cuda.is_current_stream_capturing():
+            return
+        if self._c2_ready is None:
+            self._c2_ready = torch.cuda.Event()
+        self._c2_ready.record(torch.cuda.current_stream())
 
     def _issue_pipelined_backbone(self, images_u8: torch.Tensor, main, depth: int) -> None:
         if depth == 2:
@@ -1232,6 +1401,9 @@
         with torch.cuda.graph(self.graph):
             self.out = tower.detect(self.images, self.text, self.meta, **kw)
         self.generation = tower.generation
+        self._fold = tower._fold_cur
+        self._normalize = normalize_text
+        self._src = None
 
     def __call__(self, images_u8: torch.Tensor, text: torch.Tensor, meta: torch.Tensor):
         if self.generation != self.tower.generation:
@@ -1240,6 +1412,11 @@
         self.tower.wait_post()
         self.images.copy_(images_u8, non_blocking=True)
         self.text.copy_(text, non_blocking=True)
+        if self._fold is not None and not (self._src is not None and self._src[0]() is text and self._src[1] == text._version):
+            self.tower._fold_compute(self.text, self._normalize, self._fold)
+            self._src = (weakref.ref(text), text._version)
         self.meta.copy_(meta, non_blocking=True)
         self.graph.replay()
+        if self._fold is not None:
+            self.tower._embed_valid = False
         return self.out
diff --git a/wedetect_amd/fold.py b/wedetect_amd/fold.py
--- /dev/null
+++ b/wedetect_amd/fold.py
@@ -0,0 +1,59 @@
+from __future__ import annotations
+
+import ctypes as C
+
+from . import lib as L
+
+FOLD_ABI_VERSION = 1
+
+EXPORTS = ("wd_fold_abi_version", "wd_fold_similarity", "wd_kept_rows_gather", "wd_kept_rows_select",
+           "wd_kept_rows_reorder")
+
+
+def _bind():
+    lib = L.LIB
+    for name in EXPORTS:
+        if not hasattr(lib, name):
+            raise L.WedetectHipMissing(f"{L.LIB_PATH} does not export {name}; rebuild (python -m wedetect_amd.build)")
+    vp, i32, f32 = C.c_void_p, C.c_int32, C.c_float
+    lib.wd_fold_abi_version.restype = C.c_int
+    lib.wd_fold_similarity.argtypes = [C.POINTER(L.ConvGemm), vp, f32, vp, vp]
+    lib.wd_kept_rows_gather.argtypes = [vp, vp, vp, i32, i32, i32, i32, vp, vp, i32, i32, vp, vp]
+    lib.wd_kept_rows_select.argtypes = [vp, i32, i32, i32, vp, vp, vp, i32, i32, vp, vp]
+    lib.wd_kept_rows_reorder.argtypes = [vp, i32, i32, i32, i32, vp, vp, vp, vp, vp, i32, i32, vp, vp]
+    if lib.wd_fold_abi_version() != FOLD_ABI_VERSION:
+        raise L.WedetectHipMissing(f"fold ABI mismatch: library {lib.wd_fold_abi_version()} vs binding {FOLD_ABI_VERSION}; rebuild")
+    return lib
+
+
+LIB = _bind()
+
+
+def fold_similarity(c2_split, w_split, unscale: float, unscale_dev, bias, out, *, batch: int, rows: int, cin: int, n: int,
+                    c_batch_stride: int, out_scale: float, out_bias: float, sigmoid: bool = True, range_flag=None) -> None:
+    p = L.ConvGemm(a=L._p(c2_split), w=0, bias=L._p(bias), res=0, c=L._p(out), batch=batch, hin=1, win=rows, cin=cin, lda=cin,
+                   kh=1, kw=1, stride=1, pad=0, hout=1, wout=rows, m=batch * rows, n=n, k=cin, ldc=n, ldres=0, act=L.ACT_NONE,
+                   out_mode=L.OUT_ROWS, res_alpha=1.0, out_scale=out_scale, out_bias=out_bias, sigmoid=int(bool(sigmoid)),
+                   c_batch_stride=c_batch_stride, range_flag=L._p(range_flag), c2=0, ldc2=0, a_scale=1.0, c_split_scale=1.0,
+                   ln_stats=0, ln_u=0)
+    L.check(LIB.wd_fold_similarity(C.byref(p), L._p(w_split), float(unscale), L._p(unscale_dev), L.stream_ptr()),
+            "wd_fold_similarity")
+
+
+def kept_rows_gather(c2, rows, row_floats: int, out_anchors, out_count, max_out: int, batch: int, gathered) -> None:
+    L.check(LIB.wd_kept_rows_gather(L._p(c2[0]), L._p(c2[1]), L._p(c2[2]), int(rows[0]), int(rows[1]), int(rows[2]),
+                                    int(row_floats), L._p(out_anchors), L._p(out_count), int(max_out), int(batch), L._p(gathered),
+                                    L.stream_ptr()), "wd_kept_rows_gather")
+
+
+def kept_rows_select(level_embed, dim: int, off1: int, off2: int, out_anchors, out_count, max_out: int, batch: int,
+                     out_embed, perm=None) -> None:
+    L.check(LIB.wd_kept_rows_select(L._p(level_embed), int(dim), int(off1), int(off2), L._p(out_anchors), L._p(out_count),
+                                    L._p(perm), int(max_out), int(batch), L._p(out_embed), L.stream_ptr()), "wd_kept_rows_select")
+
+
+def kept_rows_reorder(level_scores, k: int, n_anchor: int, off1: int, off2: int, out_boxes, out_scores, out_labels, out_anchors,
+                      out_count, max_out: int, batch: int, perm) -> None:
+    L.check(LIB.wd_kept_rows_reorder(L._p(level_scores), int(k), int(n_anchor), int(off1), int(off2), L._p(out_boxes),
+                                     L._p(out_scores), L._p(out_labels), L._p(out_anchors), L._p(out_count), int(max_out),
+                                     int(batch), L._p(perm), L.stream_ptr()), "wd_kept_rows_reorder")
diff --git a/wedetect_amd/lib.py b/wedetect_amd/lib.py
--- a/wedetect_amd/lib.py
+++ b/wedetect_amd/lib.py
@@ -245,6 +245,15 @@
     return out, 1.0 / scale
 
 
+def split_weights_scaled(w: torch.Tensor, out: torch.Tensor) -> None:
+    _f32(w, "w")
+    n, k = w.shape
+    w = w.contiguous()
+    if out.numel() * out.element_size() < LIB.wd_split_weights_bytes(n, k):
+        raise WedetectHipError("split_weights_scaled: output buffer too small")
+    check(LIB.wd_split_weights_padded(_p(w), n, k, 1.0, _p(out), stream_ptr()), "wd_split_weights_padded")
+
+
 def p8_workspace_bytes() -> int:
     return int(LIB.wd_p8_workspace_bytes())
 
```

Result: faster. 980.9, median of 6 (+1.9%).
